# HliasGit/navier_stokes_solver

Measured on AMD Instinct MI355X. Metric: DoF*iters/s (FGMRES+aSIMPLE, Re=100; first K=5 outer iterations), higher is better.
Workload: dtype f64

## Files before the change

### include/nsk.h

```cpp
#ifndef NSK_H
#define NSK_H

#include <stdint.h>

#ifdef __cplusplus
extern "C" {
#endif

typedef struct nsk_handle_s *nsk_handle;

enum {
  NSK_BLK_F = 0,
  NSK_BLK_BT = 1,
  NSK_BLK_B = 2,
  NSK_BLK_MP = 3,
  NSK_BLK_BT_GHOST = 4,
  NSK_BLK_S = 5
};
enum { NSK_SPACE_U = 0, NSK_SPACE_P = 1 };
enum { NSK_SOLVER_GMRES = 0, NSK_SOLVER_FGMRES = 1, NSK_SOLVER_BICGSTAB = 2 };
enum { NSK_PREC_BLOCK_DIAGONAL = 0, NSK_PREC_BLOCK_TRIANGULAR = 1, NSK_PREC_ASIMPLE = 2 };
enum { NSK_VARIANT_STATIONARY = 0, NSK_VARIANT_UNSTEADY = 1 };
enum { NSK_TRI_VELOCITY = 0, NSK_TRI_PRESSURE = 1 };

enum {
  NSK_OPT_TRI_ORDERING = 0,
  NSK_OPT_SUBDOMAINS = 1,
  NSK_OPT_FUSE_BLOCK_ROW = 2,
  NSK_OPT_STREAM_KERNELS = 3,
  NSK_OPT_INNER_FUSED_GS = 4,
  NSK_OPT_OUTER_FUSED_GS = 5,
  NSK_OPT_CG_SINGLE_REDUCTION = 11,
  NSK_OPT_BSR_VELOCITY = 7,
  NSK_OPT_TRI_SYNC_FREE = 9,
  NSK_OPT_VELOCITY_AMG = 10,
  NSK_OPT_TRI_LINE_GROUPS = 12,
  NSK_OPT_MASS_ORDERING = 13,
  NSK_OPT_SCHUR_SIGN = 14,
  NSK_OPT_BLAS1_PAIRS = 15,
  NSK_OPT_FACTOR_PRECISION = 16,
  NSK_OPT_INNER_MATRIX_PRECISION = 17,
  NSK_OPT_INNER_BASIS_PRECISION = 18,
  NSK_OPT_INNER_MATRIX_FREE_F = 19
};

typedef struct {
  double setup_ms, solve_ms;
  int64_t outer_iters, inner_u_its, inner_p_its, prec_applies, spmv_calls, tri_applies, reductions, host_syncs;
  double spmv_bytes, tri_bytes, blas1_bytes;
  int32_t n_colors_u, n_levels_u, n_colors_p, n_levels_p;
  int64_t nnz_s;
  int64_t sync_free_fallbacks;
  int64_t cur_outer_iters;
  double cur_residual;
  int64_t overlapped_spmvs;
  int64_t ring_applies;
  int64_t columns_skipped;
} nsk_stats;

int nsk_get_unique_id(void *out128);

int nsk_local_group_id(int nranks, void *out128);

nsk_handle nsk_create(int rank, int nranks, int device_id, const void *rccl_unique_id);
void nsk_destroy(nsk_handle h);
const char *nsk_last_error(nsk_handle h);

int nsk_set_partition(nsk_handle h, int space, int64_t owned_begin, int64_t owned_end, int n_ghost,
                      const int32_t *ghost_gids);
int nsk_set_support_points(nsk_handle h, int space, const double *xy);
int nsk_set_halo_plan(nsk_handle h, int space, int n_neighbors, const int32_t *peer_rank, const int32_t *send_ptr,
                      const int32_t *send_idx, const int32_t *recv_ptr);

int nsk_set_block_csr(nsk_handle h, int blk, int n_rows, int n_cols, const int32_t *rowptr, const int32_t *col,
                      const double *val);
int nsk_update_values(nsk_handle h, int blk, const double *val);

int nsk_set_option(nsk_handle h, int opt, double value);

int nsk_setup_preconditioner(nsk_handle h, int type, int variant, double alpha);

int nsk_solve(nsk_handle h, int solver, double tol_abs, int max_iter, const double *rhs_u, const double *rhs_p,
              double *x_u, double *x_p, int *iters, double *final_res);

int nsk_upload_system(nsk_handle h, const double *rhs_u, const double *rhs_p, const double *x_u, const double *x_p);
int nsk_solve_resident(nsk_handle h, int solver, double tol_abs, int max_iter, int *iters, double *final_res);
int nsk_download_solution(nsk_handle h, double *x_u, double *x_p);

int nsk_spmv(nsk_handle h, int blk, const double *x_owned, double *y, int add);
int nsk_jacobian_vmult(nsk_handle h, const double *x_u, const double *x_p, double *y_u, double *y_p);
int nsk_dot(nsk_handle h, int n, const double *x, const double *y, double *dot_out, double *norm_x_out);
int nsk_vec_op(nsk_handle h, int op, int n, double a, double c, const double *x, double *y, const double *z,
               const double *d, double *scalar_out);
int nsk_tri_apply(nsk_handle h, int which, const double *b, double *x);
int nsk_amg_info(nsk_handle h, int shard, int level, int64_t *rows, int64_t *nnz, double *lambda_max);
int nsk_tri_get_perm(nsk_handle h, int which, int32_t *perm);
int nsk_tri_get_value_bytes(nsk_handle h, int which, int32_t *bytes);
int nsk_inner_value_bytes(nsk_handle h, int blk, int32_t *bytes);
int nsk_inner_basis_bytes(nsk_handle h, int32_t *bytes);
int nsk_inner_spmv(nsk_handle h, int blk, const double *x_owned, double *y);
int nsk_inner_matrix_free(nsk_handle h, int32_t *on);
int nsk_matfree_f(nsk_handle h, const double *x_owned, double *y);
int nsk_precond_vmult(nsk_handle h, const double *src_u, const double *src_p, double *dst_u, double *dst_p,
                      int calls);
int64_t nsk_block_nnz(nsk_handle h, int blk);
int nsk_get_block(nsk_handle h, int blk, int32_t *rowptr, int32_t *col, double *val);
int nsk_debug_spmv_form(int blk_ok, int stream_ok, int inner32, int use_stream, int use_bsr, int mode, int inner);

int nsk_assembly_set_cells(nsk_handle h, int64_t n_cells, const int32_t *cell_u_nodes, const int32_t *cell_p_dofs,
                           const uint8_t *cell_flags, const double *tables944, int32_t cell_of_dof0);
int nsk_assembly_set_dirichlet(nsk_handle h, const uint8_t *dirichlet_u, const double *bc_u );
int nsk_assembly_set_simplex(nsk_handle h, int64_t n_cells, const int32_t *cell_u_nodes, const int32_t *cell_p_dofs,
                             const double *grad_lambda, const double *area, int64_t n_blocks, const int32_t *blk_ptr,
                             const int32_t *blk_ent, const int64_t *blk_pos0, const int64_t *blk_pos1,
                             const int32_t *node_ptr, const int32_t *node_ent, const int32_t *vert_ptr,
                             const int32_t *vert_ent, const double *outlet_w, int64_t pos00);
int nsk_state_set(nsk_handle h, const double *u_owned, const double *p_owned);
int nsk_state_get(nsk_handle h, double *u_owned, double *p_owned);
int nsk_state_save(nsk_handle h);
int nsk_state_update(nsk_handle h, double alpha);
int nsk_state_save_old(nsk_handle h);
int nsk_assemble(nsk_handle h, int stokes, double nu, double inv_dt, double p_out, int inhomogeneous_bc,
                 double *residual_norm);
int nsk_forces_set_faces(nsk_handle h, int64_t n_faces, const int32_t *face_cell, const uint8_t *face_side,
                         const double *tables672);
int nsk_forces_set_edges(nsk_handle h, int64_t n_edges, const int32_t *edge_cell, const uint8_t *edge_local,
                         const double *edge_nl);
int nsk_forces(nsk_handle h, double nu, double *drag_lift, double *local_drag_lift );
int nsk_state_get_patches(nsk_handle h, int64_t n, const int32_t *cells, double *vel ,
                          double *prs );
int nsk_record_set_cells(nsk_handle h, int64_t n_cells, const int32_t *cells, int subdivisions,
                         const double *w_u , const double *w_p );
int nsk_state_get_record(nsk_handle h, int64_t n_points, double *vel3 , double *prs );
int nsk_scale_values(nsk_handle h, int blk, double factor);
int nsk_download_rhs(nsk_handle h, double *rhs_u, double *rhs_p);
int nsk_time_assemble(nsk_handle h, double nu, double inv_dt, int reps, double *avg_ms);

int nsk_get_stats(nsk_handle h, nsk_stats *out);
int nsk_get_history(nsk_handle h, double *out, int cap);
int nsk_cancel(nsk_handle h);
int nsk_abort_group(nsk_handle h);
int nsk_reset_stats(nsk_handle h);

int nsk_time_op(nsk_handle h, int op, int reps, double *avg_ms, double *bytes);

int nsk_profile_begin(nsk_handle h, int op, int max_samples);
int nsk_profile_read(nsk_handle h, int op, double *avg_ms, int *n_samples, double *bytes_per_launch,
                     int64_t *n_calls, double *bytes_format);
int nsk_profile_end(nsk_handle h);

#ifdef __cplusplus
}
#endif
#endif
```

### navier_stokes_solver_amd/csrc/nsk_core.cpp

```cpp
#include "nsk_core.hpp"

#include <rccl/rccl.h>

#include <algorithm>
#include <condition_variable>
#include <cstdlib>
#include <map>
#include <memory>
#include <mutex>

namespace nsk {

#define NSK_NCCL(call)                                                                     \
  do {                                                                                     \
    ncclResult_t r__ = (call);                                                             \
    if (r__ != ncclSuccess)                                                                \
      throw ::nsk::Error(-20, std::string(#call) + ": " + ncclGetErrorString(r__));        \
  } while (0)

struct LocalGroup {
  int n = 0;
  std::mutex m;
  std::condition_variable cv;
  int waiting = 0;
// ... 485 lines not shown
    if (ns >= 0 && comm.active()) {
      comm.allreduce_sum(slot(ns), 1, stream);
      scalar_sqrt(stream, slot(ns), slot(ns) + 1);
    }
    if (ns >= 0) ++st.reductions;
    st.blas1_bytes += 4.0 * n * mc + 16.0 * n;
    ++gs_launches;
  }
}
void Ctx::multi_add(int n, double *x, double *const *z, const double *y, int m) {
  const int cap = gs_one_launch == 1 ? kMgsMaxVecs : gs_one_launch == 2 ? 16 : 1;
  for (int i0 = 0; i0 < m; i0 += cap) {
    const int mc = std::min(cap, m - i0);
    VecPackAll Z{};
    CoefPack Y{};
    for (int k = 0; k < mc; ++k) { Z.v[k] = z[i0 + k]; Y.y[k] = y[i0 + k]; }
    if (gs_one_launch && vec_multi_add(stream, n, x, Z, Y, mc)) {
      st.blas1_bytes += 8.0 * n * (mc + 2);
      ++gs_launches;
    } else {
      for (int k = 0; k < mc; ++k, ++gs_launches) vec_axpy(stream, n, sref(y[i0 + k]), z[i0 + k], x);
      st.blas1_bytes += 24.0 * n * mc;
    }
  }
}

bool Ctx::mgs_applicable(int n, int nv) const {
  if (!fused_mgs || comm.active() || nv < 1 || nv > kMgsMaxVecs) return false;
  const int G = std::min(n_cu, kMgsThreads);
  return (long)n <= (long)G * kMgsThreads * 12;
}

void Ctx::warn(const std::string &msg) {
  fprintf(stderr, "[nsk] warning: %s\n", msg.c_str());
  if (warn_text) *warn_text = "warning: " + msg;
}

void Ctx::mgs_timed_out() {
  fused_mgs = false;
  ++mgs_fallbacks;
  if (mgs_err.p) NSK_HIP(hipMemsetAsync(mgs_err.p, 0, sizeof(int), stream));
  warn("one-launch Gram-Schmidt sweep: a wait ran out of spins (workgroups not co-resident: another process on the "
       "GPU?); this column is redone link by link and the sweep stays off for this handle (slower, same results)");
}

bool Ctx::mgs_sweep(int n, double *w, double *const *v, int nv, int so) {
  if (!mgs_applicable(n, nv)) return false;
  const int G = std::min(n_cu, kMgsThreads);
  const size_t tab = (size_t)(kMgsMaxVecs + 1) * G;
  if (mgs_grid != G) {
    mgs_tables.alloc(2 * tab);
    vec_fill_sentinel(stream, (int)(2 * tab), mgs_tables.p);
    mgs_err.alloc(1);
    NSK_HIP(hipMemsetAsync(mgs_err.p, 0, sizeof(int), stream));
    mgs_grid = G;
    mgs_parity = 0;
  }
  MgsArgs A{};
  A.n = n;
  A.nv = nv;
  for (int k = 0; k < nv; ++k) A.v[k] = v[k];
  A.aux = w;
  A.table = mgs_tables.p + (size_t)mgs_parity * tab;
  A.rearm = mgs_tables.p + (size_t)(1 - mgs_parity) * tab;
  A.out = slot(so);
  A.err = mgs_err.p;
  A.fault = mgs_fault ? 1 : 0;
  NSK_HIP(hipMemsetAsync(slot(so + nv + 2), 0, sizeof(double), stream));
  mgs_tier = nsk::mgs_sweep(stream, A, G);
  if (!mgs_tier) return false;
  mgs_parity = 1 - mgs_parity;
  st.reductions += nv + 1;
  st.blas1_bytes += 8.0 * n * (nv + 2);
  return true;
}

int Csr::spmv_launch(hipStream_t s, SpmvForm f, const double *xo, const double *xg, double *y, int mode, const double *z,
                     int c0, int c1) const {
  if (f == SpmvForm::csr_vector) return nsk::spmv(s, view(), lpr, xo, xg, y, mode, z);
  if (c1 == kToPlanEnd) c1 = is_blk(f) ? blk_nblk : nblk;
  if (c1 <= c0) return 0;
  const int *cb = off16.p ? colbase.p + c0 : nullptr;
  switch (f) {
    case SpmvForm::blk_f32: nsk::spmv_blk_stream(s, blk_view32(), blk_rowblk.p + c0, c1 - c0, xo, xg, y); return 0;
    case SpmvForm::blk: nsk::spmv_blk_stream(s, blk_view(), blk_R, blk_C, blk_rowblk.p + c0, c1 - c0, xo, xg, y); return 0;
    case SpmvForm::stream_f32: return nsk::spmv_stream(s, view32(), rowblk.p + c0, c1 - c0, even_rows, xo, xg, y, off16.p, cb);
    default: return nsk::spmv_stream(s, view(), rowblk.p + c0, c1 - c0, even_rows, xo, xg, y, mode, z, off16.p, cb);
  }
}

void Ctx::spmv(Csr &A, Space &colspace, const DVec &x, double *y, int mode, const double *z) {
  comm.halo_exchange(colspace, x, stream);
  A.spmv_launch(stream, A.spmv_form(true, false, mode), x.own, x.ghost, y, mode, z);
  ++st.spmv_calls;
  st.spmv_bytes += (double)A.spmv_bytes() + (mode ? 8.0 * A.n_rows : 0.0);
}

bool build_rowblocks(const int *ra, const int *rb, int n_rows, int max_nnz, const std::vector<int> *cuts,
                     std::vector<int> &rowblk, const unsigned char *glue) {
  rowblk.clear();
  rowblk.push_back(0);
  size_t ci = 0;
  int r0 = 0;
  auto nnz_of = [&](int a, int b) { return (ra[b] - ra[a]) + (rb ? rb[b] - rb[a] : 0); };
  while (r0 < n_rows) {
    while (cuts && ci < cuts->size() && (*cuts)[ci] <= r0) ++ci;
    const int limit = (cuts && ci < cuts->size()) ? std::min(n_rows, (*cuts)[ci]) : n_rows;
    int r1 = r0 + 1;
    if (nnz_of(r0, r1) > max_nnz) return false;
    while (r1 < limit && r1 - r0 < kStreamRows && nnz_of(r0, r1 + 1) <= max_nnz) ++r1;
    if (glue) {
      while (r1 < limit && r1 > r0 && glue[r1]) --r1;
      if (r1 == r0) {
        r1 = r0 + 1;
        while (r1 < limit && glue[r1]) ++r1;
        if (r1 - r0 > kStreamRows || nnz_of(r0, r1) > max_nnz) return false;
      }
    }
    rowblk.push_back(r1);
    r0 = r1;
  }
  return true;
}

void Csr::find_interior() {
  int_r0 = int_r1 = 0;
  if (n_cols == n_own_cols) { int_r1 = n_rows; return; }
  std::vector<char> ghost((size_t)n_rows, 0);
#pragma omp parallel for schedule(static)
  for (int i = 0; i < n_rows; ++i) {
    char g = 0;
    for (int k = h_rowptr[i]; k < h_rowptr[i + 1]; ++k) g |= h_col[k] >= n_own_cols;
    ghost[i] = g;
  }
  int best0 = 0, best1 = 0, start = 0;
  for (int i = 0; i <= n_rows; ++i) {
    if (i == n_rows || ghost[i]) {
      if (i - start > best1 - best0) { best0 = start; best1 = i; }
      start = i + 1;
    }
  }
  int_r0 = best0;
  int_r1 = best1;
}

static void interior_runs(const std::vector<int> &rb, int r0, int r1, int &b0, int &b1) {
  b0 = b1 = 0;
  const int nb = (int)rb.size() - 1;
  for (int b = 0; b < nb; ++b)
    if (rb[b] >= r0 && rb[b + 1] <= r1) {
      if (b1 == b0) b0 = b;
      b1 = b + 1;
    }
}

void Csr::build_stream_plan(hipStream_t s) {
  std::vector<int> rb;
  find_interior();
  std::vector<int> cuts;
  if (int_r0 > 0) cuts.push_back(int_r0);
  if (int_r1 < n_rows && int_r1 > int_r0) cuts.push_back(int_r1);
  stream_ok = n_rows > 0 && build_rowblocks(h_rowptr.data(), nullptr, n_rows, kStreamNnz, cuts.empty() ? nullptr : &cuts, rb);
  if (!stream_ok) { nblk = 0; return; }
  nblk = (int)rb.size() - 1;
  interior_runs(rb, int_r0, int_r1, int_b0, int_b1);
  even_rows = true;
  for (int i = 0; i <= n_rows; ++i)
    if (h_rowptr[i] & 1) { even_rows = false; break; }
  rowblk.upload(rb, s);
  off16.release();
  colbase.release();
  idx16_wide = false;
}

void Csr::build_index16(hipStream_t s, bool want) {
  off16.release();
  colbase.release();
  idx16_wide = false;
  if (!want || !stream_ok || nblk <= 0) return;
  if (nnz <= 0) {
    colbase.alloc((size_t)nblk);
    off16.alloc(8);
    NSK_HIP(hipMemsetAsync(colbase.p, 0, sizeof(int) * (size_t)nblk, s));
    NSK_HIP(hipMemsetAsync(off16.p, 0, 8 * sizeof(unsigned short), s));
    return;
  }
  if (!col.p) return;
  DBuf<int> wide;
  wide.alloc(1);
  colbase.alloc((size_t)nblk);
  NSK_HIP(hipMemsetAsync(wide.p, 0, sizeof(int), s));
  nsk::setup_run_col_base(s, nblk, nullptr, rowblk.p, rowptr.p, col.p, colbase.p, wide.p);
  int w = 0;
  NSK_HIP(hipMemcpyAsync(&w, wide.p, sizeof(int), hipMemcpyDeviceToHost, s));
  NSK_HIP(hipStreamSynchronize(s));
  if (w) {
    idx16_wide = true;
    colbase.release();
    return;
  }
  off16.alloc((size_t)nnz + 8);
  NSK_HIP(hipMemsetAsync(off16.p + nnz, 0, 8 * sizeof(unsigned short), s));
  nsk::setup_run_col_offsets(s, nblk, nullptr, rowblk.p, rowptr.p, col.p, colbase.p, off16.p);
}

void Csr::build_blocked(int R, int C, hipStream_t s) {
  blk_ok = false;
  if (n_rows <= 0 || n_rows % R || n_own_cols % C || n_cols % C) return;
  const int nr = n_rows / R;
  std::vector<int> rp(nr + 1, 0);
  bool ok = true;
#pragma omp parallel for schedule(static) reduction(&& : ok)
  for (int r = 0; r < nr; ++r) {
    const int a0 = h_rowptr[R * r], len = h_rowptr[R * r + 1] - a0;
    bool good = len % C == 0;
    for (int q = 1; good && q < R; ++q) good = h_rowptr[R * r + q + 1] - h_rowptr[R * r + q] == len;
    for (int k = 0; good && k < len; k += C) {
      const int c = h_col[a0 + k];
      good = c % C == 0;
      for (int q = 0; good && q < R; ++q)
        for (int t = 0; good && t < C; ++t) good = h_col[h_rowptr[R * r + q] + k + t] == c + t;
    }
    rp[r + 1] = len / C;
    ok = ok && good;
  }
  if (!ok) return;
  for (int r = 0; r < nr; ++r) rp[r + 1] += rp[r];
  blk_count = rp[nr];
  UVec<int> bcol((size_t)blk_count), bsrc((size_t)blk_count * R * C);
  std::vector<int> rb;
#pragma omp parallel for schedule(static)
  for (int r = 0; r < nr; ++r)
    for (int k = 0; k < rp[r + 1] - rp[r]; ++k) {
      const size_t b = (size_t)rp[r] + k;
      bcol[b] = h_col[h_rowptr[R * r] + C * k] / C;
      for (int q = 0; q < R; ++q)
        for (int t = 0; t < C; ++t) bsrc[(b * R + q) * C + t] = h_rowptr[R * r + q] + C * k + t;
    }
  find_interior();
  const int ib0 = (int_r0 + R - 1) / R, ib1 = int_r1 / R;
  std::vector<int> cuts;
  if (ib0 > 0 && ib0 < nr) cuts.push_back(ib0);
  if (ib1 < nr && ib1 > ib0) cuts.push_back(ib1);
  if (!build_rowblocks(rp.data(), nullptr, nr, kBlkMax, cuts.empty() ? nullptr : &cuts, rb)) return;
  interior_runs(rb, ib0, ib1, blk_int_b0, blk_int_b1);
  blk_R = R;
  blk_C = C;
  blk_rows = nr;
  blk_nblk = (int)rb.size() - 1;
  h_blk_rowptr = rp;
  blk_rowptr.upload(rp, s);
  blk_col.upload(bcol, s);
  blk_src.upload(bsrc, s);
  blk_rowblk.upload(rb, s);
  blk_val.alloc((size_t)blk_count * R * C);
  NSK_HIP(hipStreamSynchronize(s));
  blk_ok = true;
  refresh_blocked(s);
}

void Csr::refresh_blocked(hipStream_t s) {
  if (blk_ok) vec_gather(s, (int)(blk_count * blk_R * blk_C), blk_src.p, val.p, blk_val.p);
}

void Csr::refresh_f32(hipStream_t s, bool count_overflow) {
  if (!inner32) return;
  if (count_overflow) {
    if (!f32_overflow.p) f32_overflow.alloc(1);
    NSK_HIP(hipMemsetAsync(f32_overflow.p, 0, sizeof(unsigned), s));
  }
  unsigned *ovf = count_overflow ? f32_overflow.p : nullptr;
  if (inner32 == 1) {
    const size_t n = (size_t)blk_count * blk_R * blk_C;
    if (blk_val32.n != n) blk_val32.alloc(n);
    vec_gather(s, (int)n, blk_src.p, val.p, blk_val32.p);
    if (ovf) vec_to_float(s, (int)nnz, val.p, nullptr, ovf);
  } else {
    if (val32.n != (size_t)nnz) val32.alloc((size_t)nnz);
    vec_to_float(s, (int)nnz, val.p, val32.p, ovf);
  }
  val32_version = values_version;
}

double *VecPool::get(bool zero) {
  double *p;
  if (!free_list.empty()) {
    p = free_list.back();
    free_list.pop_back();
  } else {
    NSK_HIP(hipMalloc((void **)&p, sizeof(double) * (((size_t)n + ng + 15) / 16 * 16 + 16)));
    all.push_back(p);
    zero = true;
  }
  if (zero) NSK_HIP(hipMemsetAsync(p, 0, sizeof(double) * ((size_t)n + ng), ctx->stream));
  return p;
}

void VecPool::destroy() {
  for (double *p : all) (void)hipFree(p);
  all.clear();
  free_list.clear();
}

float *BasisPool32::get(int j, int n_) {
  if (n_ != n) { destroy(); n = n_; }
  if ((size_t)j >= v.size()) v.resize((size_t)j + 1, nullptr);
  if (!v[j]) NSK_HIP(hipMalloc((void **)&v[j], sizeof(float) * (((size_t)n + 3) / 4 * 4 + 4)));
  return v[j];
}

void BasisPool32::destroy() {
  for (float *p : v) if (p) (void)hipFree(p);
  v.clear();
  n = 0;
}

}
```

### navier_stokes_solver_amd/csrc/nsk_core.hpp

```cpp
#pragma once
#include <hip/hip_runtime.h>

#include <cstdint>
#include <cstdio>
#include <cstring>
#include <memory>
#include <stdexcept>
#include <string>
#include <vector>

#include "nsk_kernels.h"

struct ncclComm;

namespace nsk {

struct Error : std::runtime_error {
  int code;
  Error(int c, const std::string &m) : std::runtime_error(m), code(c) {}
};

#define NSK_HIP(call)                                                                              \
  do {                                                                                             \
    hipError_t e__ = (call);                                                                       \
// ... 18 lines not shown
template <class T>
struct DBuf {
  T *p = nullptr;
  size_t n = 0;
  DBuf() = default;
  DBuf(const DBuf &) = delete;
  DBuf &operator=(const DBuf &) = delete;
  DBuf(DBuf &&o) noexcept : p(o.p), n(o.n) { o.p = nullptr; o.n = 0; }
  DBuf &operator=(DBuf &&o) noexcept {
    if (this != &o) { release(); p = o.p; n = o.n; o.p = nullptr; o.n = 0; }
    return *this;
  }
  ~DBuf() { release(); }
  void release() {
    if (p) (void)hipFree(p);
    p = nullptr;
    n = 0;
  }
  void alloc(size_t count) {
    release();
    n = count;
    if (count) NSK_HIP(hipMalloc((void **)&p, count * sizeof(T)));
  }
  void upload(const T *h, size_t count, hipStream_t s) {
    if (count != n) alloc(count);
    if (count) NSK_HIP(hipMemcpyAsync(p, h, count * sizeof(T), hipMemcpyHostToDevice, s));
  }
  template <class A>
  void upload(const std::vector<T, A> &h, hipStream_t s) { upload(h.data(), h.size(), s); }
};

struct LocalXchg {
  DBuf<double> buf[2];
  hipEvent_t ready[2] = {nullptr, nullptr}, done[2] = {nullptr, nullptr};
  long seq = 0;
  std::vector<const LocalXchg *> peer;
  ~LocalXchg() {
    for (int k = 0; k < 2; ++k) {
      if (ready[k]) (void)hipEventDestroy(ready[k]);
      if (done[k]) (void)hipEventDestroy(done[k]);
    }
  }
};

struct Space {
  int n = 0;
  int ng = 0;
  int64_t gbegin = 0, gend = 0;
  std::vector<int> ghost_gid;
  std::vector<int> peers, send_ptr, recv_ptr;
  DBuf<int> d_send_idx;
  DBuf<double> d_send_buf;
  int n_send = 0;
  std::unique_ptr<LocalXchg> lx;
};

struct DVec {
  double *own = nullptr;
  double *ghost = nullptr;
  int n = 0;
};

enum class SpmvForm { csr_vector, stream, stream_f32, blk, blk_f32 };
inline bool is_f32(SpmvForm f) { return f == SpmvForm::stream_f32 || f == SpmvForm::blk_f32; }
inline bool is_blk(SpmvForm f) { return f == SpmvForm::blk || f == SpmvForm::blk_f32; }
constexpr SpmvForm spmv_form(bool blk_ok, bool stream_ok, int inner32, bool use_stream, bool use_bsr, int mode, bool inner) {
  if (inner && mode == 0 && inner32 == 1 && use_stream && use_bsr && blk_ok) return SpmvForm::blk_f32;
  if (inner && mode == 0 && inner32 == 2 && use_stream && stream_ok && !(blk_ok && use_bsr)) return SpmvForm::stream_f32;
  if (blk_ok && use_stream && use_bsr && mode == 0) return SpmvForm::blk;
  if (stream_ok && use_stream) return SpmvForm::stream;
  return SpmvForm::csr_vector;
}

struct Csr {
  int n_rows = 0, n_cols = 0, n_own_cols = 0;
  int64_t nnz = 0;
  std::vector<int> h_rowptr;
  UVec<int> h_col;
  DBuf<int> rowptr, col;
  DBuf<double> val;
  int lpr = 16;
  bool present = false;
  DBuf<int> rowblk;
  int nblk = 0;
  bool stream_ok = false, even_rows = false;
  void build_stream_plan(hipStream_t s);
  DBuf<unsigned short> off16;
  DBuf<int> colbase;
  bool idx16_wide = false;
  void build_index16(hipStream_t s, bool want);
  int int_r0 = 0, int_r1 = 0, int_b0 = 0, int_b1 = 0, blk_int_b0 = 0, blk_int_b1 = 0;
  void find_interior();
  bool blk_ok = false;
  int blk_R = 1, blk_C = 1, blk_rows = 0, blk_nblk = 0;
  int64_t blk_count = 0;
  std::vector<int> h_blk_rowptr;
  DBuf<int> blk_rowptr, blk_col, blk_src, blk_rowblk;
  DBuf<double> blk_val;
  void build_blocked(int R, int C, hipStream_t s);
  void refresh_blocked(hipStream_t s);
  BlkView blk_view() const { return BlkView{blk_rows, n_own_cols / blk_C, blk_rowptr.p, blk_col.p, blk_val.p}; }
  CsrView view() const { return CsrView{n_rows, n_own_cols, rowptr.p, col.p, val.p}; }
  int inner32 = 0;
  DBuf<float> blk_val32, val32;
  long values_version = 0, val32_version = -1;
  DBuf<unsigned> f32_overflow;
  void release_f32() { inner32 = 0; blk_val32.release(); val32.release(); f32_overflow.release(); val32_version = -1; }
  void refresh_f32(hipStream_t s, bool count_overflow);
  BlkView32 blk_view32() const { return BlkView32{blk_rows, n_own_cols / blk_C, blk_rowptr.p, blk_col.p, blk_val32.p}; }
  CsrView32 view32() const { return CsrView32{n_rows, n_own_cols, rowptr.p, col.p, val32.p}; }
  static constexpr int kToPlanEnd = -1;
  SpmvForm spmv_form(bool use_stream, bool use_bsr, int mode = 0, bool inner = false) const {
    return nsk::spmv_form(blk_ok, stream_ok, inner32, use_stream, use_bsr, mode, inner);
  }
  int spmv_launch(hipStream_t s, SpmvForm f, const double *x_own, const double *x_ghost, double *y, int mode = 0,
                  const double *z = nullptr, int c0 = 0, int c1 = kToPlanEnd) const;
  double format_bytes(SpmvForm f) const {
    const double vb = is_f32(f) ? 4.0 : 8.0;
    if (is_blk(f)) return (double)blk_count * (4.0 + vb * blk_R * blk_C) + 4.0 * (blk_rows + 1.0) + 8.0 * n_rows + 8.0 * n_cols;
    const bool index16 = off16.p && f != SpmvForm::csr_vector;
    return (double)spmv_bytes() - (8.0 - vb) * (double)nnz - (index16 ? 2.0 * (double)nnz - 4.0 * nblk : 0.0);
  }
  size_t spmv_bytes() const {
    return (size_t)12 * nnz + 4 * ((size_t)n_rows + 1) + 8 * (size_t)n_rows + 8 * (size_t)n_cols;
  }
};

bool build_rowblocks(const int *rowptr_a, const int *rowptr_b, int n_rows, int max_nnz, const std::vector<int> *cuts,
                     std::vector<int> &rowblk, const unsigned char *glue = nullptr);

inline int pick_lpr(int64_t nnz, int n_rows) {
  const double mean = n_rows > 0 ? (double)nnz / n_rows : 0.0;
  if (mean <= 6) return 4;
  if (mean <= 20) return 8;
  if (mean <= 80) return 16;
  if (mean <= 200) return 32;
  return 64;
}

struct LocalGroup;
struct Comm {
  int rank = 0, nranks = 1;
  ncclComm *comm = nullptr;
  LocalGroup *local = nullptr;
  const double *pub_buf = nullptr;
  const std::vector<int> *pub_peers = nullptr, *pub_send_ptr = nullptr;
  double *h_tmp = nullptr;
  bool on_stream = false;
  int device = 0;
  struct Pub {
    const LocalXchg *x[2] = {nullptr, nullptr};
    const std::vector<int> *peers[2] = {nullptr, nullptr}, *send_ptr[2] = {nullptr, nullptr};
    int parity[2] = {0, 0};
  } pub[2];
  long coll_seq = 0, ar_seq = 0;
  DBuf<double> ar_stage[2];
  hipEvent_t ar_ready[2] = {nullptr, nullptr}, ar_done[2] = {nullptr, nullptr};
  void local_exchange_on_stream(Space *const *sps, const DVec *xs, int count, hipStream_t s);
  bool active() const { return nranks > 1 || comm != nullptr; }
  void init(int rank, int nranks, const void *unique_id, int device_id = 0);
  void destroy();
  void abort_group();
  void allreduce_sum(double *d, int count, hipStream_t s);
  void halo_exchange(Space &sp, const DVec &x, hipStream_t s);
  void halo_exchange2(Space &sa, const DVec &xa, Space &sb, const DVec &xb, hipStream_t s);
};

int make_local_group(int nranks, void *out128, int on_stream = 0);
int abort_local_group(const void *unique_id);

struct Stats {
  double setup_ms = 0, solve_ms = 0;
  long outer_iters = 0, inner_u_its = 0, inner_p_its = 0, prec_applies = 0, spmv_calls = 0, tri_applies = 0,
       reductions = 0, host_syncs = 0, ring_applies = 0,
       columns_skipped = 0;
  double spmv_bytes = 0, tri_bytes = 0, blas1_bytes = 0;
};

struct Ctx {
  hipStream_t stream = nullptr;
  hipStream_t stream2 = nullptr;
  hipEvent_t ev_fork = nullptr, ev_join = nullptr;
  void ensure_stream2();
  int device = 0;
  int n_cu = 256;
  Comm comm;
  ReduceWs ws{};
  DBuf<double> ws_partials;
  DBuf<unsigned> ws_ticket;
  static constexpr int kSlots = 4096;
  DBuf<double> d_scal;
  double *h_scal = nullptr;
  int slot_top = 0;
  Stats st;

  void init(int device_id);
  void destroy();
  int alloc_slots(int k) {
    if (slot_top + k > kSlots) throw Error(-11, "out of device scalar slots");
    const int s = slot_top;
    slot_top += k;
    return s;
  }
  double *slot(int i) { return d_scal.p + i; }
  const double *read_slots(int first, int count);
  void sync() { NSK_HIP(hipStreamSynchronize(stream)); }

  void dot(int n, const double *x, const double *y, int slot_out);
  void norm2(int n, const double *x, int slot_out);
  void axpy_dot(int n, SRef a, const double *x, double *y, const double *w, int slot_out);
  void axpy_norm2(int n, SRef a, const double *x, double *y, int slot_out);
  void multi_dot(int n, const double *w, double *const *v, int m, int slot_out, bool defer = false);
// ... 80 lines not shown
```

### navier_stokes_solver_amd/csrc/nsk_debug.cpp

```cpp
#include <algorithm>
#include <cstring>

#include "nsk_handle.hpp"
#include "nsk_internal.h"

namespace {
std::vector<int> shifted(const int32_t *p, size_t n, int64_t base) {
  std::vector<int> v(n);
  for (size_t i = 0; i < n; ++i) {
    const int64_t q = (int64_t)p[i] + base;
    if (q < 0 || q > INT32_MAX) throw Error(-62, "position beyond int32");
    v[i] = (int)q;
  }
  return v;
}
DBuf<int> on_device(const int *h, size_t n) {
  DBuf<int> d;
  d.upload(h, n, nullptr);
  return d;
}
DBuf<double> on_device(const double *h, size_t n) {
  DBuf<double> d;
  d.upload(h, n, nullptr);
  return d;
// ... 256 lines not shown
    case NSK_DBG_KRY_MULTI_DOT_ALL_F32: {
      const bool rider = par[0] != 0.0;
      c.multi_dot_all_f32(n, d[0], f.data() + 1, m, rider, so);
      c.allreduce_slots(so, m + (rider ? 1 : 0));
      break;
    }
    case NSK_DBG_KRY_MULTI_AXPY_ALL_F32:
      set_slots(m);
      c.multi_axpy_all_f32(n, d[0], f.data() + 1, m, so, par[m] != 0.0 ? so + m : -1);
      break;
    case NSK_DBG_KRY_GS_COLUMN_F32: {
      const int mode = (int)par[0];
      if (mode < 1 || mode > 2) throw Error(-61, "nsk_debug_krylov: fp32 basis: Gram-Schmidt mode 1 or 2");
      if (!c.f32_basis_applies(mode)) throw Error(-61, "nsk_debug_krylov: fp32 basis: the pair forms only");
      arnoldi_column(c, n, d[0], (double *const *)nullptr, m, so, mode, [] {}, f.data() + 1);
      break;
    }
    case NSK_DBG_KRY_EQU:
      set_slots(1);
      vec_equ(st, n, sref(1.0, nullptr, c.slot(so)), d[0], d[1]);
      break;
    case NSK_DBG_KRY_EQU_F32:
      set_slots(1);
      vec_equ_f32(st, n, sref(1.0, nullptr, c.slot(so)), d[0], f[1], d[2]);
      break;
  }
  int bad_guards = 0;
  for (int k = 0; k < n_vec; ++k) {
    if (is_float(k)) {
      hf.resize((size_t)len[k]);
      bad_guards += fv[k].fetch(hf.data(), c);
      for (int64_t i = 0; i < len[k]; ++i) vec[k][i] = (double)hf[(size_t)i];
    } else {
      bad_guards += dv[k].fetch(vec[k], c);
    }
  }
  memcpy(slots64, c.read_slots(so, 64), sizeof(double) * 64);
  info8[0] = (int32_t)c.red_paths;
  info8[1] = path;
  info8[2] = std::min(c.n_cu, kMgsThreads);
  info8[3] = bad_guards;
  info8[4] = (int32_t)(c.gs_launches - gs_launches);
  for (int k = 5; k < 8; ++k) info8[k] = 0;
  return 0;
  NSK_CATCH(h)
}


int nsk_debug_spmv(nsk_handle h, int form, int lpr, int mode, int misalign, int c0, int c1, const nsk_dbg_spmv_mat *Am,
                   const nsk_dbg_spmv_mat *Bm, double *y, const double *z, const double *d, const double *dinv,
                   int32_t *rowblk_out, int rowblk_cap, int32_t *info) {
  NSK_TRY_DEV(h)
  Ctx &c = h->ctx;
  hipStream_t st = h->s();
  for (int k = 0; k < 16; ++k) info[k] = 0;
  info[0] = -1;
  if (form < NSK_DBG_SPMV_CSRV || form > NSK_DBG_SPMV_STREAM_I16_F32) throw Error(-65, "nsk_debug_spmv: unknown form");
  const bool two = form == NSK_DBG_SPMV_STREAM2 || form == NSK_DBG_SPMV_BLK_FUSED;
  const bool modes = form == NSK_DBG_SPMV_CSRV || form == NSK_DBG_SPMV_STREAM || form == NSK_DBG_SPMV_STREAM_I16;
  const bool epi = form == NSK_DBG_SPMV_BLK21_EPI;
  if (!Am || !y || two != (Bm != nullptr)) throw Error(-61, "nsk_debug_spmv: matrices");
  if (mode < 0 || mode > 2 || (mode != 0 && !modes) || (mode == 2 && !z)) throw Error(-61, "nsk_debug_spmv: mode");
  if (epi && !(d && dinv)) throw Error(-61, "nsk_debug_spmv: the epilogue needs d and dinv");
  if ((two || form == NSK_DBG_SPMV_CSRV) && c0 >= 0) throw Error(-61, "nsk_debug_spmv: this form runs whole plans only");
  int R = 1, C = 1;
  if (form == NSK_DBG_SPMV_BLK22 || form == NSK_DBG_SPMV_BLK22_F32 || form == NSK_DBG_SPMV_BLK_FUSED) R = C = 2;
  if (form == NSK_DBG_SPMV_BLK21 || epi) R = 2;
  if (form == NSK_DBG_SPMV_BLK12) C = 2;
  const bool blocked = form >= NSK_DBG_SPMV_BLK22 && form != NSK_DBG_SPMV_STREAM2 && form != NSK_DBG_SPMV_STREAM_I16 && form != NSK_DBG_SPMV_STREAM_I16_F32;
  if ((misalign & 4) && R == 2) throw Error(-61, "nsk_debug_spmv: the R = 2 forms store pairs, y is 16-byte aligned");
  if (two && Bm->n_rows != Am->n_rows) throw Error(-61, "nsk_debug_spmv: both matrices over the same rows");

  Csr A, B;
  dbg_fill_csr(A, *Am, st);
  if (two) dbg_fill_csr(B, *Bm, st);
  info[2] = A.lpr;
  info[3] = R;
  info[4] = C;
  info[5] = A.stream_ok;
  info[6] = A.stream_ok && A.even_rows;

  std::vector<int> rb;
  const std::vector<int> *ea = &A.h_rowptr, *eb = nullptr;
  DBuf<int> fused_rb;
  const int *d_rb = nullptr;
  int ib0 = 0, ib1 = 0, refused = 0;
  auto download = [&](const DBuf<int> &src, int nblk) {
    rb.resize((size_t)nblk + 1);
    NSK_HIP(hipMemcpyAsync(rb.data(), src.p, sizeof(int) * rb.size(), hipMemcpyDeviceToHost, st));
    c.sync();
    d_rb = src.p;
  };
  const bool i16 = form == NSK_DBG_SPMV_STREAM_I16 || form == NSK_DBG_SPMV_STREAM_I16_F32;
  if (form == NSK_DBG_SPMV_STREAM || form == NSK_DBG_SPMV_STREAM_F32 || i16) {
    if (!A.stream_ok) refused = 1;
    else { download(A.rowblk, A.nblk); ib0 = A.int_b0; ib1 = A.int_b1; }
    if (!refused && i16) {
      A.build_index16(st, true);
      if (!A.off16.p) refused = 5;
    }
  } else if (form == NSK_DBG_SPMV_STREAM2) {
    if (!A.even_rows) refused = 3;
    else if (!fused_row_plan(A, B, rb)) refused = 4;
    else { eb = &B.h_rowptr; fused_rb.upload(rb, st); d_rb = fused_rb.p; ib1 = (int)rb.size() - 1; }
  } else if (blocked) {
    A.build_blocked(R, C, st);
    if (two) B.build_blocked(2, 1, st);
    info[7] = A.blk_ok && (!two || B.blk_ok);
    if (!info[7] || (two && A.blk_rows != B.blk_rows)) refused = 2;
    else if (two) {
      if (!fused_blk_plan(A, B, rb)) refused = 4;
      else { ea = &A.h_blk_rowptr; eb = &B.h_blk_rowptr; fused_rb.upload(rb, st); d_rb = fused_rb.p; ib1 = (int)rb.size() - 1; }
    } else { download(A.blk_rowblk, A.blk_nblk); ea = &A.h_blk_rowptr; ib0 = A.blk_int_b0; ib1 = A.blk_int_b1; }
  }
  info[15] = refused;
  if (refused) return 1;
  const int nblk = (int)rb.size() - 1;
  if (form != NSK_DBG_SPMV_CSRV) {
    info[8] = nblk;
    info[9] = ib0;
    info[10] = ib1;
    for (int b = 0; b < nblk; ++b) {
      const int e = (*ea)[rb[b + 1]] - (*ea)[rb[b]] + (eb ? (*eb)[rb[b + 1]] - (*eb)[rb[b]] : 0);
      info[11] = std::max(info[11], rb[b + 1] - rb[b]);
      info[12] = std::max(info[12], e);
    }
    if (rowblk_out) std::copy(rb.begin(), rb.begin() + std::min<size_t>(rb.size(), (size_t)std::max(0, rowblk_cap)), rowblk_out);
    if (c0 < 0) { c0 = 0; c1 = nblk; }
    if (c0 > c1 || c1 > nblk) throw Error(-61, "nsk_debug_spmv: run range");
  }

  const int og = misalign & 1, ob = (misalign >> 1) & 1, oy = (misalign >> 2) & 1;
  DbgVec<double> xa, xag, xb, xbg, yv, zv, dv, div;
  xa.put(Am->x_own, (size_t)A.n_own_cols, kDbgFront, kDbgBack, st);
  xag.put(Am->x_ghost, (size_t)(A.n_cols - A.n_own_cols), kDbgFront + og, kDbgBack, st);
  if (two) {
    xb.put(Bm->x_own, (size_t)B.n_own_cols, kDbgFront + ob, kDbgBack, st);
    xbg.put(Bm->x_ghost, (size_t)(B.n_cols - B.n_own_cols), kDbgFront + og, kDbgBack, st);
  }
  yv.put(y, (size_t)A.n_rows, kDbgFront + oy, kDbgBack, st);
  if (z) zv.put(z, (size_t)A.n_rows, kDbgFront + oy, kDbgBack, st);
  if (epi) { dv.put(d, (size_t)A.n_rows, kDbgFront, kDbgBack, st); div.put(dinv, (size_t)A.n_rows, kDbgFront, kDbgBack, st); }

  const int n_run = c1 - c0;
  switch (form) {
    case NSK_DBG_SPMV_CSRV:
      if (lpr == 0) lpr = A.lpr;
      if (lpr != 2 && lpr != 4 && lpr != 8 && lpr != 16 && lpr != 32 && lpr != 64) throw Error(-61, "nsk_debug_spmv: lpr");
      info[2] = nsk::spmv(st, A.view(), lpr, xa.p, xag.p, yv.p, mode, zv.p);
      break;
    case NSK_DBG_SPMV_STREAM: case NSK_DBG_SPMV_STREAM_I16:
      info[1] = A.spmv_launch(st, SpmvForm::stream, xa.p, xag.p, yv.p, mode, zv.p, c0, c1);
      break;
    case NSK_DBG_SPMV_STREAM_F32: case NSK_DBG_SPMV_STREAM_I16_F32:
      A.inner32 = 2;
      A.refresh_f32(st, false);
      info[1] = A.spmv_launch(st, SpmvForm::stream_f32, xa.p, xag.p, yv.p, 0, nullptr, c0, c1);
      break;
    case NSK_DBG_SPMV_BLK22: case NSK_DBG_SPMV_BLK21: case NSK_DBG_SPMV_BLK12: case NSK_DBG_SPMV_BLK11:
      A.spmv_launch(st, SpmvForm::blk, xa.p, xag.p, yv.p, 0, nullptr, c0, c1);
      break;
    case NSK_DBG_SPMV_BLK22_F32:
      A.inner32 = 1;
      A.refresh_f32(st, false);
      A.spmv_launch(st, SpmvForm::blk_f32, xa.p, xag.p, yv.p, 0, nullptr, c0, c1);
      break;
    case NSK_DBG_SPMV_BLK21_EPI:
      nsk::spmv_blk_stream(st, A.blk_view(), 2, 1, d_rb + c0, n_run, xa.p, xag.p, yv.p, dv.p, div.p);
      break;
    case NSK_DBG_SPMV_STREAM2:
      info[1] = nsk::spmv2_stream(st, A.view(), xa.p, xag.p, B.view(), xb.p, xbg.p, d_rb, nblk, yv.p);
      break;
    case NSK_DBG_SPMV_BLK_FUSED:
      nsk::spmv_blk_fused22_21(st, A.blk_view(), xa.p, xag.p, B.blk_view(), xb.p, xbg.p, d_rb, nblk, yv.p);
      break;
  }
  NSK_HIP(hipGetLastError());
  info[0] = form;
  info[14] = form == NSK_DBG_SPMV_CSRV ? 0 : n_run;
  int bad = yv.fetch(y, c);
  for (DbgVec<double> *v : {&xa, &xag, &xb, &xbg, &zv, &dv, &div}) bad += v->fetch(nullptr, c);
  info[13] = bad;
  return 0;
  NSK_CATCH(h)
}

int nsk_debug_tri(nsk_handle h, const nsk_dbg_tri_args *a, int32_t *info) {
  NSK_TRY_DEV(h)
  Ctx &c = h->ctx;
  hipStream_t st = h->s();
  for (int k = 0; k < 40; ++k) info[k] = 0;
  if (!a || a->n < 1 || !a->rowptr || !a->col || !a->val || a->rowptr[0] != 0 || a->n_apply < 1 || !a->b || !a->x ||
      !a->perm_out || !a->factor_out)
    throw Error(-61, "nsk_debug_tri: arguments");
  if (a->kind < 0 || a->kind > 1 || a->ordering < ORDER_NATURAL || a->ordering > ORDER_MULTICOLOR || a->group < 1)
    throw Error(-61, "nsk_debug_tri: kind, ordering or group");
  const int n = a->n;
  for (int i = 0; i < n; ++i)
    if (a->rowptr[i + 1] < a->rowptr[i]) throw Error(-58, "nsk_debug_tri: rowptr not monotone");
  const int64_t nnz = a->rowptr[n];
  for (int i = 0; i < n; ++i)
    for (int k = a->rowptr[i]; k < a->rowptr[i + 1]; ++k)
      if (a->col[k] < 0 || a->col[k] >= n || (k > a->rowptr[i] && a->col[k - 1] >= a->col[k]))
        throw Error(-59, "nsk_debug_tri: column ids out of range or not sorted");
  std::vector<int> sub;
  if (a->n_sub > 1) {
    if (!a->sub_off || a->sub_off[0] != 0 || a->sub_off[a->n_sub] != n) throw Error(-61, "nsk_debug_tri: sub-domain offsets");
    for (int k = 0; k < a->n_sub; ++k)
      if (a->sub_off[k + 1] < a->sub_off[k]) throw Error(-61, "nsk_debug_tri: sub-domain offsets");
    sub.assign(a->sub_off, a->sub_off + a->n_sub + 1);
  }
  if (a->x_layout != 0 && !(a->want_block2 && a->sync_free)) {
    info[16] = 1;
    return 1;
  }

  Csr A;
  A.n_rows = A.n_cols = A.n_own_cols = n;
  A.nnz = nnz;
  A.h_rowptr.assign(a->rowptr, a->rowptr + n + 1);
  A.h_col.assign(a->col, a->col + nnz);
  A.rowptr.upload(a->rowptr, (size_t)n + 1, st);
  A.col.upload(a->col, (size_t)nnz, st);
  A.val.upload(a->val, (size_t)nnz, st);
  A.present = true;

  TriSolve T;
  T.use_stream = a->use_stream != 0;
  T.sync_free = a->sync_free != 0;
  T.tiny_bytes = a->tiny_bytes;
  T.host_analysis = a->host_analysis != 0;
  T.want_index16 = a->want_index16 != 0;
  T.want_f32 = a->want_f32 != 0;
  T.x_layout = a->x_layout != 0 ? 1 : 0;
  T.analyze(&c, A, a->kind, a->ordering, sub, a->want_block2 != 0, a->xy, a->group);
  T.y.alloc((size_t)n + 1 + kDbgBack);
  NSK_HIP(hipMemsetAsync(T.y.p, 0xFF, sizeof(double) * T.y.n, st));
  if (T.x_layout) {
    T.xc.alloc((size_t)n + 1 + kDbgBack);
    NSK_HIP(hipMemsetAsync(T.xc.p, 0xFF, sizeof(double) * T.xc.n, st));
  }
  T.numeric(A.val.p);
  NSK_HIP(hipGetLastError());

  std::vector<DbgVec<double>> bv((size_t)a->n_apply), xv((size_t)a->n_apply);
  for (int k = 0; k < a->n_apply; ++k) {
    bv[k].put(a->b + (size_t)k * n, (size_t)n, kDbgFront, kDbgBack, st);
    xv[k].put(a->x + (size_t)k * n, (size_t)n, kDbgFront, kDbgBack, st);
  }
  for (int k = 0; k < a->n_apply; ++k) T.apply(bv[k].p, xv[k].p);
  NSK_HIP(hipGetLastError());
  int bad = 0;
  for (int k = 0; k < a->n_apply; ++k) {
    bad += xv[k].fetch(a->x + (size_t)k * n, c);
    bad += bv[k].fetch(nullptr, c);
  }
  for (const DBuf<double> *iv : {&T.y, &T.xc}) {
// ... 22 lines not shown
    memcpy(&nanv, &nan_bits, 8);
    for (int64_t k = 0; k < nnz; ++k) a->factor_out[k] = nanv;
    for (size_t k = 0; k < fv.size(); ++k) {
      if (sp[k] < 0 || sp[k] >= nnz) throw Error(-62, "nsk_debug_tri: a source position outside the matrix");
      a->factor_out[sp[k]] = fv[k];
    }
  }

  const int path = T.last_path;
  const bool scalar_halves = path == TRI_PATH_SF_SCALAR || path == TRI_PATH_COLOUR_SCALAR;
  const bool halves = scalar_halves || path == TRI_PATH_SF_BLOCKED || path == TRI_PATH_COLOUR_BLOCKED;
  info[0] = path;
  info[1] = halves && T.f32 ? 32 : 64;
  info[2] = !scalar_halves ? 0 : T.Loff16.p ? 16 : 32;
  info[3] = !scalar_halves ? 0 : T.Uoff16.p ? 16 : 32;
  info[4] = T.gmax;
  info[5] = T.n_colors;
  info[6] = T.n_levels_L;
  info[7] = T.n_levels_U;
  if (T.stream_ready || T.block2_ready) {
    for (int half = 0; half < 2; ++half) {
      const DBuf<int4> &D = half ? T.Udesc : T.Ldesc;
      std::vector<int4> d(D.n);
      if (D.n) NSK_HIP(hipMemcpyAsync(d.data(), D.p, sizeof(int4) * D.n, hipMemcpyDeviceToHost, st));
      c.sync();
      info[8 + 2 * half] = (int)D.n;
      info[9 + 2 * half] = (half ? T.n_Usf : T.n_Lsf) - (int)D.n;
      for (const int4 &r : d) {
        info[12] = std::max(info[12], r.y - r.x);
        info[13] = std::max(info[13], r.w - r.z);
      }
    }
  }
  if (T.sf_err.p) {
    int e = 0;
    NSK_HIP(hipMemcpy(&e, T.sf_err.p, sizeof(int), hipMemcpyDeviceToHost));
    info[14] = e != 0;
  }
  info[15] = bad;
  info[17] = (a->want_block2 && !T.block2_ready ? 1 : 0) | (a->want_index16 && !(scalar_halves && T.Loff16.p) ? 2 : 0) |
             (a->want_f32 && info[1] != 32 ? 4 : 0) |
             (a->ordering == ORDER_NATURAL && n >= 4096 && !T.ring_ready ? 8 : 0);
  info[18] = T.lpr;
  for (const TriSolve::Step &s : T.schedL) ++info[s.serial ? 20 : 19];
  for (const TriSolve::Step &s : T.schedU) ++info[s.serial ? 29 : 28];
  info[21] = T.last_tiny;
  info[22] = T.ring_ready ? T.ringL.n_pass : 0;
  if (a->kind == 0)
    for (const TriSolve::Step &s : T.schedN) ++info[s.serial ? 24 : 23];
  info[25] = T.stream_ready;
  info[26] = T.block2_ready;
  info[27] = T.dev_analysis;
  info[30] = T.max_row_nnz;
  info[31] = (int32_t)T.nnz;
  info[32] = path == TRI_PATH_SF_BLOCKED && T.x_layout != 0;
  return 0;
  NSK_CATCH(h)
}

int nsk_debug_amg(nsk_handle h, const nsk_dbg_amg_args *a, int32_t *info) {
  NSK_TRY_DEV(h)
  return debug_amg(&h->ctx, a, info);
  NSK_CATCH(h)
}

int nsk_debug_index_width(nsk_handle h, int b, int32_t *out3) {
  NSK_TRY(h)
  if (b != NSK_BLK_S && b != NSK_BLK_MP) throw Error(-62, "nsk_debug_index_width: S or M_p");
  if (h->prec_type < 0) throw Error(-46, "call nsk_setup_preconditioner first");
  const Csr &A = h->blk[b];
  const TriSolve &T = b == NSK_BLK_S ? h->tS : h->tMp;
  out3[0] = !A.present || h->form_of(A) != SpmvForm::stream ? 0 : A.off16.p ? 16 : 32;
  const bool halves = T.stream_ready && T.halves_in_use();
  out3[1] = !halves ? 0 : T.Loff16.p ? 16 : 32;
  out3[2] = !halves ? 0 : T.Uoff16.p ? 16 : 32;
  return 0;
  NSK_CATCH(h)
}

int nsk_debug_spmv_form(int blk_ok, int stream_ok, int inner32, int use_stream, int use_bsr, int mode, int inner) {
  return (int)spmv_form(blk_ok != 0, stream_ok != 0, inner32, use_stream != 0, use_bsr != 0, mode, inner != 0);
}

int nsk_debug_pool_counts(nsk_handle h, int32_t *out6) {
  int k = 0;
  for (const VecPool *p : {&h->pool_u, &h->pool_p, &h->pool_b}) {
    out6[k++] = (int32_t)p->all.size();
    out6[k++] = (int32_t)p->free_list.size();
  }
  return 0;
}

int64_t nsk_debug_asm(nsk_handle h, int what, void *out, int64_t cap) {
  NSK_TRY_DEV(h)
  const auto &A = h->asmd;
  if (!A.ready || A.simplex || !A.mf_valid) throw Error(-66, "nsk_debug_asm: no Q3/Q2 assembly on the handle (call nsk_assemble)");
  const void *src = nullptr;
  size_t bytes = 0;
  switch (what) {
    case NSK_DBG_ASM_CQ: src = A.cq.p; bytes = sizeof(double) * (size_t)A.n_cells * kAsmCellDoubles; break;
    case NSK_DBG_ASM_D0: src = A.d0.p; bytes = sizeof(double); break;
    case NSK_DBG_ASM_NODE_CELLS: src = A.node_cells.p; bytes = sizeof(int) * A.node_cells.n; break;
    case NSK_DBG_ASM_NODE_OFF: src = A.node_off.p; bytes = A.node_off.n; break;
    case NSK_DBG_ASM_NODE_SELF: src = A.node_self.p; bytes = sizeof(int) * A.node_self.n; break;
    case NSK_DBG_ASM_PDOF_CELLS: src = A.pdof_cells.p; bytes = sizeof(int) * A.pdof_cells.n; break;
    default: throw Error(-65, "nsk_debug_asm: unknown item");
  }
  if (!out || cap < (int64_t)bytes) throw Error(-61, "nsk_debug_asm: out is too small");
  if (bytes) NSK_HIP(hipMemcpyAsync(out, src, bytes, hipMemcpyDeviceToHost, h->s()));
  h->ctx.sync();
  return (int64_t)bytes;
  NSK_CATCH(h)
}

}
```

### navier_stokes_solver_amd/csrc/nsk_handle.hpp

```cpp
#pragma once
#include <chrono>
#include <exception>
#include <string>
#include <vector>

#include "../../include/nsk.h"
#include "nsk_solver.hpp"
#include "nsk_amg.hpp"
#include "nsk_assembly.hpp"
#include "nsk_tri.hpp"

using namespace nsk;

inline double wall_ms() {
  return std::chrono::duration<double, std::milli>(std::chrono::steady_clock::now().time_since_epoch()).count();
}
inline bool verbose() {
  static const bool v = getenv("NSK_VERBOSE") && atoi(getenv("NSK_VERBOSE")) > 0;
  return v;
}
struct Phase {
  const char *name;
  double t0;
  explicit Phase(const char *n) : name(n), t0(wall_ms()) {}
// ... 18 lines not shown
    S.used = 0;
    S.e0.resize(cap);
    S.e1.resize(cap);
    for (int i = 0; i < cap; ++i) { (void)hipEventCreate(&S.e0[i]); (void)hipEventCreate(&S.e1[i]); }
  }
  Slot *want(int o) {
    for (int k = 0; k < n; ++k)
      if (slots[k].op == o) {
        ++slots[k].seen;
        return slots[k].used < slots[k].cap ? &slots[k] : nullptr;
      }
    return nullptr;
  }
  Slot *find(int o) {
    for (int k = 0; k < n; ++k)
      if (slots[k].op == o) return &slots[k];
    return nullptr;
  }
  void release() {
    for (int k = 0; k < n; ++k) {
      for (size_t i = 0; i < slots[k].e0.size(); ++i) { (void)hipEventDestroy(slots[k].e0[i]); (void)hipEventDestroy(slots[k].e1[i]); }
      slots[k] = Slot{};
    }
    n = 0;
  }
};

struct Sampled {
  EventSampler::Slot *smp;
  hipStream_t s;
  Sampled(EventSampler &es, int op, hipStream_t st) : smp(es.want(op)), s(st) {
    if (smp) (void)hipEventRecord(smp->e0[smp->used], s);
  }
  Sampled(const Sampled &) = delete;
  ~Sampled() {
    if (smp) (void)hipEventRecord(smp->e1[smp->used++], s);
  }
};
struct Event {
  hipEvent_t e = nullptr;
  Event() { NSK_HIP(hipEventCreate(&e)); }
  Event(const Event &) = delete;
  ~Event() { (void)hipEventDestroy(e); }
  operator hipEvent_t() const { return e; }
};

inline bool fused_blk_plan(const Csr &F, const Csr &Bt, std::vector<int> &rb) {
  return build_rowblocks(F.h_blk_rowptr.data(), Bt.h_blk_rowptr.data(), F.blk_rows, kBlkMax, nullptr, rb);
}
inline bool fused_row_plan(const Csr &F, const Csr &Bt, std::vector<int> &rb) {
  return build_rowblocks(F.h_rowptr.data(), Bt.h_rowptr.data(), F.n_rows, kStreamNnz, nullptr, rb);
}

struct nsk_handle_s {
  Ctx ctx;
  EventSampler sampler;
  std::string err;
  Space sp[2];
  Csr blk[6];
  VecPool pool_u, pool_p, pool_b;
  bool pools_ready = false;
  int tri_ordering = ORDER_MULTICOLOR, subdomains = 1, fuse_block_row = 1, use_stream = 1;
  int inner_fused_gs = 1;
  bool outer_fused_gs = false, cg_fused = false;
  int use_bsr = 1;
  int sync_free_fallbacks = 0;
  std::vector<double> support[2];
  int line_groups = 2, group_u = 2, group_p = 3;
  int mp_ordering = -1;
  int mass_ordering(int type, int variant_) const {
    if (mp_ordering >= 0) return mp_ordering;
    return (type == 0 && variant_ == 1) ? (int)ORDER_NATURAL : tri_ordering;
  }
  static constexpr int kGroupRowsU = 4000000, kGroupRowsP = 1000000;
  const double *xy(int space) const {
    if (!line_groups || support[space].size() != 2 * (size_t)sp[space].n) return nullptr;
    if (sync_free_mode < (space == 0 ? 2 : 1)) return nullptr;
    if (line_groups == 2 && sp[space].n > (space == 0 ? kGroupRowsU : kGroupRowsP)) return nullptr;
    return support[space].data();
  }
  int x_layout_mode = 2;
  int sync_free_mode = 2;
  int fault_inject = 0;
  DBuf<int> jrow_blk, jblk_blk;
  int jrow_nblk = 0, jblk_nblk = 0;
  bool jrow_ok = false, jblk_ok = false;

  int prec_type = -1, variant = 0;
  double alpha = 0.5;
  TriSolve tF, tMp, tS;
  Amg amgF;
  int velocity_amg = 1;
  int schur_sign = 1;
  int blas1_pairs = -1;
  int factor_precision = 64;
  int inner_matrix_precision = 64;
  int inner_basis_precision = 64;
  bool basis32_wanted = false;
  BasisPool32 basis32_u;
  int inner_basis_width() const {
    if (!inner_solve_on(NSK_BLK_F)) return 0;
    return basis32_wanted && ctx.f32_basis_applies(inner_fused_gs) ? 4 : 8;
  }
  void inner_fgmres_options(SolverFGMRES &sv) {
    sv.fused_gs = inner_fused_gs;
    sv.skip_unused = inner_skip();
    sv.basis32 = basis32_wanted ? &basis32_u : nullptr;
  }
  long mp_values_version = 0, mp_factored_version = -1;
  int mp_factored_kind = -1;
  bool amg_active = false;
  int timeop_between = -1;
  bool amg_pending = false;
  void amg_ready() {
    if (!amg_pending) return;
    amg_pending = false;
    const double t0 = wall_ms();
    try {
      amgF.setup(&ctx, blk[NSK_BLK_F], sub_offsets(0));
    } catch (...) {
      amgF.clear();
      amg_pending = true;
      throw;
    }
    setup_ms += wall_ms() - t0;
    lazy_setup_ms += wall_ms() - t0;
  }
  double lazy_setup_ms = 0;
  bool tF_ok = false, tMp_ok = false, tS_ok = false, s_symbolic = false;
  int tF_key = -1, tMp_key = -1, tS_key = -1;
  TriSolve *tP = nullptr;
  int s_max_row = 0;
  double *D = nullptr, *Dinv = nullptr, *tmp_p = nullptr, *delta_p = nullptr, *tmp_u = nullptr, *tmp_b = nullptr;
  double *rhs_b = nullptr, *x_b = nullptr, *x_keep = nullptr;
  volatile long progress_step = 0;
  volatile double progress_value = 0.0;
  volatile int cancel = 0;
  std::vector<double> history;
  long inner_u = 0, inner_p = 0, prec_applies = 0, outer_iters = 0;
  double setup_ms = 0, solve_ms = 0;
  bool skip_unused = true;
  SolverFGMRES::Pending pending;
  void drop_pending() {
    if (pending.v) pool_b.put(pending.v);
    if (pending.z) pool_b.put(pending.z);
    pending = SolverFGMRES::Pending{};
  }
  int inner_skip() const { return skip_unused ? SolverFGMRES::stateless : SolverFGMRES::reference; }

  struct AsmData {
    bool ready = false, dirichlet_set = false, have_bc = false, state_set = false;
    long n_cells = 0;
    int cell_of_dof0 = -1;
    DBuf<int> cell_u, cell_p, node_cells, node_self, pdof_cells;
    DBuf<unsigned char> cell_flags, node_off, dirichlet;
    DBuf<double> tables, cq, bc;
    double *sol_u = nullptr, *sol_p = nullptr, *eval_u = nullptr, *eval_p = nullptr;
    bool simplex = false;
    long sx_blocks = 0, sx_pos00 = 0;
    DBuf<int> sx_blk_ptr, sx_blk_ent, sx_node_ptr, sx_node_ent, sx_vert_ptr, sx_vert_ent;
    DBuf<long> sx_pos0, sx_pos1;
    DBuf<double> sx_grad, sx_area, sx_outlet;
    double *old_u = nullptr;
    bool have_old = false;
    double assemble_ms = 0;
    bool mf_valid = false;
    double mf_nu = 0, mf_inv_dt = 0;
// ... 56 lines not shown
    pool_u.init(&ctx, sp[0].n, sp[0].ng);
    pool_p.init(&ctx, sp[1].n, sp[1].ng);
    pool_b.init(&ctx, N(), sp[0].ng + sp[1].ng);
    rhs_b = pool_b.get(true);
    x_b = pool_b.get(true);
    pools_ready = true;
  }
  void halo(int space, const DVec &x) { ctx.comm.halo_exchange(sp[space], x, s()); }
  bool inner_solve_on(int b) const {
    if (prec_type < 0) return false;
    if (b == NSK_BLK_F) return prec_type != 2 || variant == 0;
    if (b == NSK_BLK_MP) return prec_type != 2;
    if (b == NSK_BLK_S) return prec_type == 2 && variant == 0;
    return false;
  }
  SpmvForm form_of(const Csr &A, int mode = 0, bool inner = false) const { return A.spmv_form(use_stream != 0, use_bsr != 0, mode, inner); }
  int inner_width(const Csr &A) const { return is_f32(form_of(A, 0, true)) ? 4 : 8; }
  void spmv_nohalo(Csr &A, const DVec &x, double *y, int mode = 0, const double *z = nullptr, bool inner = false) {
    {
      Sampled smp(sampler, (int)(&A - blk), s());
      A.spmv_launch(s(), form_of(A, mode, inner), x.own, x.ghost, y, mode, z);
    }
    ++ctx.st.spmv_calls;
    ctx.st.spmv_bytes += (double)A.spmv_bytes() + (mode == 1 ? 8.0 * A.n_rows : 0.0);
  }
  bool index16 = true;
  void index16_for(Csr &A, const char *name) {
    A.build_index16(s(), index16);
    if (verbose() && index16 && A.stream_ok && !A.off16.p)
      fprintf(stderr, "[nsk] %s: a run of the stream plan spans 65 536 columns or more — int32 column ids stay in use\n", name);
  }
  bool overlap_halo = true;
  long overlapped_spmvs = 0;
  void spmv_halo(Csr &A, int space, const DVec &x, double *y) {
    if (matfree_wanted && &A == &blk[NSK_BLK_F]) {
      const char *why = matfree_obstacle();
      if (!why) {
        halo(space, x);
        matfree_apply(x, y);
        return;
      }
      if (!matfree_warned) {
        matfree_warned = true;
        fprintf(stderr, "[nsk] warning: NSK_OPT_INNER_MATRIX_FREE_F = 1, but %s: the inner FGMRES multiplies by the assembled F\n", why);
      }
    }
    const SpmvForm form = form_of(A, 0, true);
    if (is_f32(form) && A.val32_version != A.values_version) A.refresh_f32(s(), false);
    const bool blocked = is_blk(form);
    const int b0 = blocked ? A.blk_int_b0 : A.int_b0, b1 = blocked ? A.blk_int_b1 : A.int_b1;
    const int nb = blocked ? A.blk_nblk : A.nblk;
    EventSampler::Slot *smp = sampler.find((int)(&A - blk));
    const bool sampling = smp && smp->used < smp->cap;
    if (!overlap_halo || ctx.comm.nranks <= 1 || form == SpmvForm::csr_vector || b1 <= b0 || sampling) {
      halo(space, x);
      spmv_nohalo(A, x, y, 0, nullptr, true);
      return;
    }
    if (smp) ++smp->seen;
    ++overlapped_spmvs;
    ctx.ensure_stream2();
    auto part = [&](hipStream_t st, int c0, int c1) { A.spmv_launch(st, form, x.own, x.ghost, y, 0, nullptr, c0, c1); };
    NSK_HIP(hipEventRecord(ctx.ev_fork, s()));
    NSK_HIP(hipStreamWaitEvent(ctx.stream2, ctx.ev_fork, 0));
    part(ctx.stream2, b0, b1);
    NSK_HIP(hipEventRecord(ctx.ev_join, ctx.stream2));
    halo(space, x);
    part(s(), 0, b0);
    part(s(), b1, nb);
    NSK_HIP(hipStreamWaitEvent(s(), ctx.ev_join, 0));
    ++ctx.st.spmv_calls;
    ctx.st.spmv_bytes += (double)A.spmv_bytes();
  }
  void jacobian_vmult(const DVec &xb, double *yb) {
    const DVec xu = ub(xb.own), xp = pb(xb.own);
    ctx.comm.halo_exchange2(sp[0], xu, sp[1], xp, s());
    Csr &F = blk[NSK_BLK_F], &Bt = blk[NSK_BLK_BT], &B = blk[NSK_BLK_B];
    const bool blocked = use_stream && use_bsr && F.blk_ok && Bt.blk_ok && F.blk_R == 2 && Bt.blk_R == 2 &&
                         F.blk_rows == Bt.blk_rows;
    if (fuse_block_row && blocked && !jblk_ok && jblk_nblk == 0) {
      std::vector<int> rb;
      if (fused_blk_plan(F, Bt, rb)) {
        jblk_nblk = (int)rb.size() - 1;
        jblk_blk.upload(rb, s());
        ctx.sync();
        jblk_ok = true;
      } else jblk_nblk = -1;
    }
    if (fuse_block_row && use_stream && !jrow_ok && jrow_nblk == 0 && F.even_rows) {
      std::vector<int> rb;
      if (fused_row_plan(F, Bt, rb)) {
        jrow_nblk = (int)rb.size() - 1;
        jrow_blk.upload(rb, s());
        ctx.sync();
        jrow_ok = true;
      } else jrow_nblk = -1;
    }
    const double fused_bytes = (double)F.spmv_bytes() + (double)Bt.spmv_bytes() - 8.0 * F.n_rows - 4.0 * (F.n_rows + 1);
    if (fuse_block_row && blocked && jblk_ok) {
      nsk::spmv_blk_fused22_21(s(), F.blk_view(), xu.own, xu.ghost, Bt.blk_view(), xp.own, xp.ghost, jblk_blk.p,
                               jblk_nblk, yb);
      ctx.st.spmv_calls += 2;
      ctx.st.spmv_bytes += fused_bytes;
    } else if (fuse_block_row && use_stream && jrow_ok) {
      nsk::spmv2_stream(s(), F.view(), xu.own, xu.ghost, Bt.view(), xp.own, xp.ghost, jrow_blk.p, jrow_nblk, yb);
      ctx.st.spmv_calls += 2;
      ctx.st.spmv_bytes += fused_bytes;
    } else {
      spmv_nohalo(F, xu, yb, 0);
      spmv_nohalo(Bt, xp, yb, 1);
    }
    spmv_nohalo(B, xu, yb + n_u(), 0);
  }
  void tri_apply_sampled(TriSolve &T, int op, const double *b, double *x) {
    Sampled smp(sampler, op, s());
    T.apply(b, x);
  }
  std::vector<int> sub_offsets(int space) const {
    std::vector<int> off;
    if (subdomains <= 1) return off;
    const int n = sp[space].n;
    off.resize(subdomains + 1);
    for (int k = 0; k <= subdomains; ++k) {
      long v = (long)n * k / subdomains;
      if (space == 0) v &= ~1L;
      off[k] = (int)v;
    }
    off[subdomains] = n;
    return off;
  }
  void check_sync_free() {
    int e = 0;
    for (TriSolve *T : {&tF, &tMp, &tS})
      if (T->sf_err.p) {
        int ei = 0;
        NSK_HIP(hipMemcpy(&ei, T->sf_err.p, sizeof(int), hipMemcpyDeviceToHost));
        if (ei) {
          NSK_HIP(hipMemsetAsync(T->sf_err.p, 0, sizeof(int), s()));
          T->sf_armed = false;
        }
        e |= ei;
      }
    if (ctx.comm.active() && sync_free_mode > 0) {
      const SlotLease sl(ctx, 1);
      vec_set(s(), 1, ctx.slot(sl), e ? 1.0 : 0.0);
      ctx.comm.allreduce_sum(ctx.slot(sl), 1, s());
      e = ctx.read_slots(sl, 1)[0] > 0.0;
    }
    if (e)
      throw Error(-70, "sync-free triangular solve: a producer/consumer wait ran out of spins (results invalid); "
                       "set NSK_OPT_TRI_SYNC_FREE to 0");
  }
  void push_tri_options() {
    tMp.sync_free = tS.sync_free = sync_free_mode >= 1;
    tF.sync_free = sync_free_mode == 2;
    tMp.sf_fault = tS.sf_fault = (fault_inject & 1) != 0;
    tF.sf_fault = (fault_inject & 2) != 0;
    tMp.want_index16 = tS.want_index16 = index16;
    tF.use_stream = tMp.use_stream = tS.use_stream = use_stream != 0;
  }
  void schur_symbolic();
  void setup(int type, int variant_, double alpha_);
  void prec_vmult(DVec &dst, const DVec &src);
  int solve_once(int solver, double tol, int max_iter, int *iters, double *final_res);
  int solve_resident(int solver, double tol, int max_iter, int *iters, double *final_res);
};
using H = nsk_handle_s;

#define NSK_TRY(h) try {
#define NSK_TRY_DEV(h) NSK_TRY(h) (void)hipSetDevice((h)->ctx.device);
#define NSK_CATCH(h)                                  \
  }                                                   \
  catch (const Error &e) {                            \
    (h)->err = e.what();                              \
    return e.code;                                    \
  }                                                   \
  catch (const std::exception &e) {                   \
    (h)->err = e.what();                              \
    return -1;                                        \
  }

#define NSK_CATCH_ABORT(h)                            \
  }                                                   \
  catch (const Error &e) {                            \
    (h)->err = e.what();                              \
    if (e.code != -25) (h)->ctx.comm.abort_group();   \
    return e.code;                                    \
  }                                                   \
// ... 6 lines not shown
```

### navier_stokes_solver_amd/csrc/nsk_internal.h

```cpp
#pragma once
#include <stdint.h>

enum {
  NSK_IOPT_TRI_X_LAYOUT = 6,
  NSK_IOPT_FAULT_INJECT = 100,
  NSK_IOPT_GROUP_U = 103,
  NSK_IOPT_GROUP_P = 104,
  NSK_IOPT_TINY_BYTES = 102,
  NSK_IOPT_OVERLAP_HALO = 107,
  NSK_IOPT_HOST_ANALYSIS = 108,
  NSK_IOPT_TIMEOP_BETWEEN = 109,
  NSK_IOPT_INDEX16 = 110,
  NSK_IOPT_GS_ONE_LAUNCH = 111,
  NSK_IOPT_FGMRES_SKIP_UNUSED = 112,
  NSK_IOPT_FUSED_MGS = 106
};

#ifdef __cplusplus
extern "C" {
#endif
int nsk_debug_tri_trace(struct nsk_handle_s *h, int which, int64_t *out16, int max_runs, int *grid);
int nsk_local_group_id_mode(int nranks, int on_stream, void *out128);
int nsk_abort_local_group(const void *uid128);
int nsk_debug_tri_ordering(int n, const int32_t *rowptr, const int32_t *col, int n_sub, const int32_t *sub_off,
                           int want_block2, const double *xy, int group, int32_t *perm_out, int32_t *info4,
                           uint8_t *chain_out);
int nsk_debug_ilu0_at_offset(int what, int n, const int32_t *rowptr, const int32_t *col, double *val_inout, int64_t base);
int nsk_debug_schur_at_offset(int n_p, int n_u, const int32_t *b_rp, const int32_t *b_col, const double *b_val,
                              const double *dinv, const int32_t *bt_rp, const int32_t *bt_col, const double *bt_val,
                              const int32_t *s_rp, const int32_t *s_col, double *s_val_out, int64_t base);
enum {
  NSK_DBG_KRY_DOT = 0, NSK_DBG_KRY_NORM2 = 1, NSK_DBG_KRY_AXPY_DOT = 2, NSK_DBG_KRY_AXPY_NORM2 = 3, NSK_DBG_KRY_CG_UPDATE = 4,
  NSK_DBG_KRY_MULTI_DOT = 5, NSK_DBG_KRY_MULTI_AXPY = 6, NSK_DBG_KRY_GS_COLUMN = 7, NSK_DBG_KRY_DOT3 = 8,
  NSK_DBG_KRY_CG_SCALARS = 9, NSK_DBG_KRY_CG_FUSED_UPDATE = 10, NSK_DBG_KRY_CHEBY = 11, NSK_DBG_KRY_DENSE_MV = 12,
  NSK_DBG_KRY_MULTI_DOT_ALL = 13, NSK_DBG_KRY_MULTI_AXPY_ALL = 14, NSK_DBG_KRY_MULTI_ADD = 15,
  NSK_DBG_KRY_MULTI_DOT_ALL_F32 = 16, NSK_DBG_KRY_MULTI_AXPY_ALL_F32 = 17, NSK_DBG_KRY_GS_COLUMN_F32 = 18,
  NSK_DBG_KRY_EQU = 19, NSK_DBG_KRY_EQU_F32 = 20
};
int nsk_debug_krylov(struct nsk_handle_s *h, int op, int n, int m, int offset, const double *par, int n_vec,
                     double *const *vec, const int64_t *len, double *slots64, int32_t *info8);
enum {
  NSK_DBG_SPMV_CSRV = 0, NSK_DBG_SPMV_STREAM = 1, NSK_DBG_SPMV_STREAM_F32 = 2, NSK_DBG_SPMV_BLK22 = 3,
  NSK_DBG_SPMV_BLK21 = 4, NSK_DBG_SPMV_BLK12 = 5, NSK_DBG_SPMV_BLK11 = 6, NSK_DBG_SPMV_BLK22_F32 = 7,
  NSK_DBG_SPMV_BLK21_EPI = 8, NSK_DBG_SPMV_STREAM2 = 9, NSK_DBG_SPMV_BLK_FUSED = 10, NSK_DBG_SPMV_STREAM_I16 = 11,
  NSK_DBG_SPMV_STREAM_I16_F32 = 12
};
struct nsk_dbg_spmv_mat {
  int32_t n_rows, n_cols, n_own_cols, pad_;
  const int32_t *rowptr, *col;
  const double *val, *x_own, *x_ghost;
};
int nsk_debug_spmv(struct nsk_handle_s *h, int form, int lpr, int mode, int misalign, int c0, int c1,
                   const struct nsk_dbg_spmv_mat *A, const struct nsk_dbg_spmv_mat *B, double *y, const double *z,
                   const double *d, const double *dinv, int32_t *rowblk_out, int rowblk_cap, int32_t *info16);
struct nsk_dbg_tri_args {
  int32_t n, kind, ordering, n_sub;
  const int32_t *rowptr, *col;
  const double *val;
  const int32_t *sub_off;
  const double *xy;
  int32_t group, want_block2, use_stream, sync_free;
  double tiny_bytes;
  int32_t host_analysis, want_index16, want_f32, x_layout;
  int32_t n_apply, pad_;
  const double *b;
  double *x;
  int32_t *perm_out;
  double *factor_out;
};
int nsk_debug_tri(struct nsk_handle_s *h, const struct nsk_dbg_tri_args *a, int32_t *info40);
enum {
  NSK_DBG_AMG_SCAN = 0, NSK_DBG_AMG_BLOCK = 1, NSK_DBG_AMG_DIAG = 2, NSK_DBG_AMG_STRENGTH = 3, NSK_DBG_AMG_MIS_PULL = 4,
  NSK_DBG_AMG_MIS_DECIDE = 5, NSK_DBG_AMG_MIS_MARK = 6, NSK_DBG_AMG_ROOTS = 7, NSK_DBG_AMG_JOIN = 8,
  NSK_DBG_AMG_AGG_WEIGHTS = 9, NSK_DBG_AMG_AGGREGATE = 10, NSK_DBG_AMG_PRODUCT = 11, NSK_DBG_AMG_PRODUCT_COUNT = 12,
  NSK_DBG_AMG_TRANSPOSE = 13, NSK_DBG_AMG_ROWS_SORT = 14, NSK_DBG_AMG_START_VECTOR = 15
};
struct nsk_dbg_amg_mat {
  int32_t n_rows, n_cols;
  const int32_t *rowptr, *col;
  const double *val;
};
struct nsk_dbg_amg_args {
  int32_t op, n, r0, r1, pass, stamp, roots_only, first, product, first_tier, nc, out_cap;
  int64_t flag_words;
  double threshold, c;
  struct nsk_dbg_amg_mat A, B;
  const int32_t *i_in;
  const uint64_t *key, *key2;
  const uint16_t *flag;
  const double *ad, *dinv, *pw;
  int32_t *i_out;
  uint64_t *k_out;
  uint16_t *flag_out;
  double *d_out, *d_out2;
  int32_t *out_rp, *out_col;
  double *out_val;
  int64_t *out64;
};
int nsk_debug_amg(struct nsk_handle_s *h, const struct nsk_dbg_amg_args *a, int32_t *info16);
int nsk_debug_index_width(struct nsk_handle_s *h, int b, int32_t *out3);
int nsk_debug_spmv_form(int blk_ok, int stream_ok, int inner32, int use_stream, int use_bsr, int mode, int inner);
int nsk_debug_pool_counts(struct nsk_handle_s *h, int32_t *out6);
enum { NSK_DBG_ASM_CQ = 0, NSK_DBG_ASM_D0 = 1, NSK_DBG_ASM_NODE_CELLS = 2, NSK_DBG_ASM_NODE_OFF = 3,
       NSK_DBG_ASM_NODE_SELF = 4, NSK_DBG_ASM_PDOF_CELLS = 5 };
int64_t nsk_debug_asm(struct nsk_handle_s *h, int what, void *out, int64_t cap);
#ifdef __cplusplus
}
#endif
```

### navier_stokes_solver_amd/csrc/nsk_kernels.h

```cpp
#pragma once
#include <hip/hip_runtime.h>
#include <stdint.h>

namespace nsk {

struct SRef {
  double c;
  const double *num;
  const double *den;
};
inline SRef sref(double c) { return SRef{c, nullptr, nullptr}; }
inline SRef sref(double c, const double *num) { return SRef{c, num, nullptr}; }
inline SRef sref(double c, const double *num, const double *den) { return SRef{c, num, den}; }

struct ReduceWs {
  double *partials;
  unsigned *ticket;
  int pairs;
};
constexpr int kMaxReduceBlocks = 512;
constexpr int kMaxReduceOut = 32;

template <class V>
struct CsrViewT {
  int n_rows;
  int n_own_cols;
  const int *rowptr;
  const int *col;
  const V *val;
};
using CsrView = CsrViewT<double>;
using CsrView32 = CsrViewT<float>;
int spmv(hipStream_t s, const CsrView &A, int lanes_per_row, const double *x_own, const double *x_ghost, double *y,
         int mode, const double *z);

constexpr int kStreamNnz = 2048;
constexpr int kStreamRows = 64;
int spmv_stream(hipStream_t s, const CsrView &A, const int *rowblk, int nblk, int even_rows, const double *x_own,
                const double *x_ghost, double *y, int mode, const double *z, const unsigned short *off16 = nullptr,
                const int *colbase = nullptr);
int spmv_stream(hipStream_t s, const CsrView32 &A, const int *rowblk, int nblk, int even_rows, const double *x_own,
                const double *x_ghost, double *y, const unsigned short *off16 = nullptr, const int *colbase = nullptr);
int spmv2_stream(hipStream_t s, const CsrView &A, const double *xa_own, const double *xa_ghost, const CsrView &B,
                 const double *xb_own, const double *xb_ghost, const int *rowblk, int nblk, double *y);

template <class V>
struct BlkViewT {
  int n_brows;
  int n_own_bcols;
  const int *rowptr;
  const int *col;
  const V *val;
};
using BlkView = BlkViewT<double>;
using BlkView32 = BlkViewT<float>;
constexpr int kBlkMax = 1024;
void spmv_blk_stream(hipStream_t s, const BlkView &A, int R, int C, const int *rowblk, int nblk, const double *x_own,
                     const double *x_ghost, double *y, const double *epi_d = nullptr, const double *epi_dinv = nullptr);
void spmv_blk_stream(hipStream_t s, const BlkView32 &A, const int *rowblk, int nblk, const double *x_own,
                     const double *x_ghost, double *y);
void spmv_blk_fused22_21(hipStream_t s, const BlkView &A, const double *xa_own, const double *xa_ghost,
                         const BlkView &B, const double *xb_own, const double *xb_ghost, const int *rowblk, int nblk,
                         double *y);

void vec_set(hipStream_t s, int n, double *y, double v);
void vec_copy(hipStream_t s, int n, const double *x, double *y);
void vec_equ(hipStream_t s, int n, SRef a, const double *x, double *y);
void vec_axpy(hipStream_t s, int n, SRef a, const double *x, double *y);
void vec_sadd(hipStream_t s, int n, SRef sc, SRef a, const double *x, double *y);
void vec_axpy2(hipStream_t s, int n, SRef a, const double *x, SRef b, const double *z, double *y);
void vec_scale(hipStream_t s, int n, SRef a, double *y);
void vec_mul(hipStream_t s, int n, const double *d, double *y);
void vec_submul(hipStream_t s, int n, const double *d, const double *x, double *y);
void vec_sub_then_mul(hipStream_t s, int n, const double *x, const double *d, double *y);
void vec_recip(hipStream_t s, int n, const double *x, double *y);
void vec_cheby_step(hipStream_t s, int n, double c1, double c2, const double *dinv, const double *r, double *w,
                    double *x, int set_x);
void dense_mv(hipStream_t s, int n, const double *M, const double *b, double *x);
constexpr int kRedScalar = 1, kRedPairs = 2;
int vec_dot(hipStream_t s, const ReduceWs &ws, int n, const double *x, const double *y, double *out, int want_sqrt);
int vec_axpy_dot(hipStream_t s, const ReduceWs &ws, int n, SRef a, const double *x, double *y, const double *w,
                 double *out, int want_sqrt);
int vec_cg_update(hipStream_t s, const ReduceWs &ws, int n, SRef a, const double *d, const double *h, double *x,
                  double *g, double *out);
struct VecPack {
  const double *v[8];
};
int vec_multi_dot(hipStream_t s, const ReduceWs &ws, int n, const double *w, const VecPack &P, int m, double *out);
void gs_pythagoras(hipStream_t s, double *h, int m);
int vec_multi_axpy(hipStream_t s, const ReduceWs &ws, int n, double *w, const VecPack &P, int m, const double *h,
                   double *norm_out);
constexpr int kMgsThreads = 1024, kMgsMaxVecs = 32;
struct VecPackAll {
  const double *v[kMgsMaxVecs];
};
int vec_multi_dot_all(hipStream_t s, const ReduceWs &ws, int n, const double *w, const VecPackAll &P, int m, double *out);
int vec_multi_axpy_all(hipStream_t s, const ReduceWs &ws, int n, double *w, const VecPackAll &P, int m, const double *h,
                       double *norm_out);
struct CoefPack {
  double y[kMgsMaxVecs];
};
int vec_multi_add(hipStream_t s, int n, double *x, const VecPackAll &Z, const CoefPack &Y, int m);
struct VecPack32 {
  const float *v[kMgsMaxVecs];
};
int vec_multi_dot_f32(hipStream_t s, const ReduceWs &ws, int n, const double *w, const VecPack32 &P, int m, int rider,
                      double *out);
int vec_multi_axpy_f32(hipStream_t s, const ReduceWs &ws, int n, double *w, const VecPack32 &P, int m, const double *h,
                       double *norm_out);
int red_grid_quads(int n);
void vec_equ_f32(hipStream_t s, int n, SRef a, const double *x, float *v, double *vw);
struct MgsArgs {
  int n, nv;
  const double *v[kMgsMaxVecs];
  double *aux, *table, *rearm, *out;
  int *err;
  int fault;
};
int mgs_sweep(hipStream_t s, const MgsArgs &A, int G);
int vec_dot3(hipStream_t s, const ReduceWs &ws, int n, const double *r, const double *u, const double *w, double *out);
void cg_fused_scalars(hipStream_t s, double *sc7, int first);
void vec_cg_fused_update(hipStream_t s, int n, const double *sc7, const double *u, const double *w, double *p, double *sv,
                         double *x, double *r);
void scalar_sqrt(hipStream_t s, const double *in, double *out);
void vec_gather(hipStream_t s, int n, const int *idx, const double *x, double *y);
void vec_gather(hipStream_t s, int n, const int *idx, const double *x, float *y);
void vec_to_float(hipStream_t s, int n, const double *x, float *y, unsigned *overflow);
void extract_diag(hipStream_t s, const CsrView &A, double *d, double *dinv);

struct TriView {
  int n;
  const int *rowptr;
  const int *diag;
  const int *col;
  const double *val;
  const int *perm;
};
void tri_lower_level(hipStream_t s, const TriView &T, int kind, int lpr, const int *rows, int nrows, const double *rhs,
                     double *y);
void tri_upper_level(hipStream_t s, const TriView &T, int kind, int lpr, const int *rows, int nrows, double *y,
                     double *out);
void tri_lower_serial(hipStream_t s, const TriView &T, int kind, const int *lvl_ptr, const int *rows, int l0, int l1,
                      const double *rhs, double *y);
void tri_upper_serial(hipStream_t s, const TriView &T, int kind, const int *lvl_ptr, const int *rows, int l0, int l1,
                      double *y, double *out);
// ... 111 lines not shown
```

### navier_stokes_solver_amd/csrc/nsk_kernels.hip

```cpp
#include "nsk_kernels.h"

#include <algorithm>
#include <type_traits>

namespace nsk {

namespace {

constexpr int BLK = 256;

__device__ __forceinline__ double sval(const SRef &s) {
  double v = s.c;
  if (s.num) v *= *s.num;
  if (s.den) v /= *s.den;
  return v;
}

template <int W>
__device__ __forceinline__ double subwave_sum(double v) {
#pragma unroll
  for (int off = W / 2; off > 0; off >>= 1) v += __shfl_down(v, off, W);
  return v;
}

inline int ew_grid(int n) {
  long b = ((long)n + BLK * 4 - 1) / (BLK * 4);
  if (b < 1) b = 1;
  if (b > 2048) b = 2048;
  return (int)b;
}
constexpr int RBLK = 1024;
inline int red_grid(int n) {
  long b = ((long)n + RBLK * 4 - 1) / (RBLK * 4);
  if (b < 1) b = 1;
  if (b > kMaxReduceBlocks) b = kMaxReduceBlocks;
  return (int)b;
}
inline int red_grid_pairs(int n, int cap) {
  long b = (((long)n + 1) / 2 + RBLK * 4 - 1) / (RBLK * 4);
  if (b < 1) b = 1;
  if (b > cap) b = cap;
  return (int)b;
}

template <int LPR, int MODE>
__global__ __launch_bounds__(BLK) void spmv_kernel(CsrView A, const double *__restrict__ xo,
                                                   const double *__restrict__ xg, double *__restrict__ y,
                                                   const double *__restrict__ z) {
  const long tid = (long)blockIdx.x * BLK + threadIdx.x;
  const int row = (int)(tid / LPR);
  const int lane = (int)(tid % LPR);
  double s = 0.0;
  if (row < A.n_rows) {
    const int re = A.rowptr[row + 1];
    for (int k = A.rowptr[row] + lane; k < re; k += LPR) {
      const int c = A.col[k];
      const double xv = c < A.n_own_cols ? xo[c] : xg[c - A.n_own_cols];
      s += A.val[k] * xv;
    }
  }
  s = subwave_sum<LPR>(s);
  if (lane == 0 && row < A.n_rows) {
    if (MODE == 0) y[row] = s;
    else if (MODE == 1) y[row] = (z ? z[row] : y[row]) + s;
    else y[row] = z[row] - s;
  }
}

constexpr int RG = 4;

__device__ __forceinline__ double2 widen2(double2 v) { return v; }
__device__ __forceinline__ double2 widen2(float2 v) { return make_double2((double)v.x, (double)v.y); }

template <class I>
struct IdxPair;
template <>
struct IdxPair<int> {
  typedef int v2 __attribute__((ext_vector_type(2)));
  typedef v2 unaligned __attribute__((aligned(4)));
  typedef v2 aligned2;
  int a, b;
  __device__ __forceinline__ IdxPair(v2 q, int) : a(q[0]), b(q[1]) {}
};
template <>
struct IdxPair<unsigned short> {
  typedef unsigned v2;
  typedef unsigned unaligned __attribute__((aligned(2)));
  typedef unsigned aligned2;
  int a, b;
  __device__ __forceinline__ IdxPair(unsigned q, int base) : a(base + (int)(q & 0xffffu)), b(base + (int)(q >> 16)) {}
};

template <class V, int VEC, class I = int>
__device__ __forceinline__ void stream_products(const I *__restrict__ col, const V *__restrict__ val, int k0,
                                                int k1, int n_own, const double *__restrict__ xo,
                                                const double *__restrict__ xg, double *prod, int base = 0) {
  if (VEC == 3) {
    constexpr int U = kStreamNnz / (2 * BLK);
    typedef V vv2 __attribute__((ext_vector_type(2)));
    typedef vv2 vd2u __attribute__((aligned(sizeof(V))));
    int c0[U], c1[U];
    double v0[U], v1[U], x0[U], x1[U];
#pragma unroll
    for (int u = 0; u < U; ++u) {
      const int k = k0 + 2 * ((int)threadIdx.x + u * BLK);
      if (k + 1 < k1) {
        const IdxPair<I> ci(*reinterpret_cast<const typename IdxPair<I>::unaligned *>(col + k), base);
        const vv2 vi = *reinterpret_cast<const vd2u *>(val + k);
        c0[u] = ci.a; c1[u] = ci.b; v0[u] = (double)vi[0]; v1[u] = (double)vi[1];
      } else {
        const bool ok = k < k1;
        c0[u] = ok ? base + (int)col[k] : 0; v0[u] = ok ? (double)val[k] : 0.0; c1[u] = 0; v1[u] = 0.0;
      }
    }
#pragma unroll
    for (int u = 0; u < U; ++u) {
      x0[u] = *(c0[u] < n_own ? xo + c0[u] : xg + (c0[u] - n_own));
      x1[u] = *(c1[u] < n_own ? xo + c1[u] : xg + (c1[u] - n_own));
    }
#pragma unroll
    for (int u = 0; u < U; ++u) {
      const int k = k0 + 2 * ((int)threadIdx.x + u * BLK);
      if (k < k1) prod[k - k0] = v0[u] * x0[u];
      if (k + 1 < k1) prod[k - k0 + 1] = v1[u] * x1[u];
    }
  } else if (VEC == 2) {
    constexpr int U = kStreamNnz / (2 * BLK);
    typedef typename std::conditional<std::is_same<V, double>::value, double2, float2>::type V2;
    int2 c[U];
    double2 v[U];
#pragma unroll
    for (int u = 0; u < U; ++u) {
      const int k = k0 + 2 * ((int)threadIdx.x + u * BLK);
      const bool ok = k < k1;
      if (ok) {
        const IdxPair<I> ci(*reinterpret_cast<const typename IdxPair<I>::aligned2 *>(col + k), base);
        c[u] = make_int2(ci.a, ci.b);
      } else c[u] = make_int2(0, 0);
      v[u] = ok ? widen2(*reinterpret_cast<const V2 *>(val + k)) : make_double2(0.0, 0.0);
    }
    double x0[U], x1[U];
#pragma unroll
    for (int u = 0; u < U; ++u) {
      x0[u] = *(c[u].x < n_own ? xo + c[u].x : xg + (c[u].x - n_own));
      x1[u] = *(c[u].y < n_own ? xo + c[u].y : xg + (c[u].y - n_own));
    }
#pragma unroll
    for (int u = 0; u < U; ++u) {
      const int k = k0 + 2 * ((int)threadIdx.x + u * BLK);
      if (k < k1) { prod[k - k0] = v[u].x * x0[u]; prod[k - k0 + 1] = v[u].y * x1[u]; }
    }
  } else {
    constexpr int U = kStreamNnz / BLK;
    int c[U];
    double v[U], xv[U];
#pragma unroll
    for (int u = 0; u < U; ++u) {
      const int k = k0 + (int)threadIdx.x + u * BLK;
      const bool ok = k < k1;
      c[u] = ok ? base + (int)col[k] : 0;
      v[u] = ok ? (double)val[k] : 0.0;
    }
#pragma unroll
    for (int u = 0; u < U; ++u) xv[u] = *(c[u] < n_own ? xo + c[u] : xg + (c[u] - n_own));
#pragma unroll
    for (int u = 0; u < U; ++u) {
      const int k = k0 + (int)threadIdx.x + u * BLK;
      if (k < k1) prod[k - k0] = v[u] * xv[u];
    }
  }
}

__device__ __forceinline__ double row_sum_lds(const double *prod, int b, int e, int lane) {
  double s = 0.0;
  int j = b + lane;
  for (; j + 3 * RG < e; j += 4 * RG) {
    const double a0 = prod[j], a1 = prod[j + RG], a2 = prod[j + 2 * RG], a3 = prod[j + 3 * RG];
    s += a0;
    s += a1;
    s += a2;
    s += a3;
  }
  for (; j < e; j += RG) s += prod[j];
  return subwave_sum<RG>(s);
}

template <class V, int VEC, int MODE, class I = int>
__global__ __launch_bounds__(BLK) void spmv_stream_kernel(CsrViewT<V> A, const int *__restrict__ rowblk,
                                                          const double *__restrict__ xo,
                                                          const double *__restrict__ xg, double *__restrict__ y,
                                                          const double *__restrict__ z,
                                                          const unsigned short *__restrict__ off16 = nullptr,
                                                          const int *__restrict__ colbase = nullptr) {
  __shared__ double prod[kStreamNnz];
  const int r0 = rowblk[blockIdx.x], r1 = rowblk[blockIdx.x + 1];
  constexpr bool I16 = std::is_same<I, unsigned short>::value;
  const int base = I16 ? colbase[blockIdx.x] : 0;
  const int k0 = A.rowptr[r0], k1 = A.rowptr[r1];
  const int r = r0 + (int)threadIdx.x / RG, lane = threadIdx.x % RG;
  const bool have = r < r1;
  int jb = 0, je = 0;
  double zv = 0.0;
  if (have) {
    jb = A.rowptr[r] - k0;
    je = A.rowptr[r + 1] - k0;
    if (MODE == 1) zv = z ? z[r] : y[r];
    if (MODE == 2) zv = z[r];
  }
  if constexpr (I16) stream_products<V, VEC, unsigned short>(off16, A.val, k0, k1, A.n_own_cols, xo, xg, prod, base);
  else stream_products<V, VEC>(A.col, A.val, k0, k1, A.n_own_cols, xo, xg, prod);
  __syncthreads();
  const double sum = row_sum_lds(prod, jb, je, lane);
  if (have && lane == 0) {
    if (MODE == 0) y[r] = sum;
    else if (MODE == 1) y[r] = zv + sum;
    else y[r] = zv - sum;
  }
}

template <int VECA>
__global__ __launch_bounds__(BLK) void spmv2_stream_kernel(CsrView A, const double *__restrict__ xao,
                                                           const double *__restrict__ xag, CsrView B,
                                                           const double *__restrict__ xbo,
                                                           const double *__restrict__ xbg,
                                                           const int *__restrict__ rowblk, double *__restrict__ y) {
  __shared__ double prod[kStreamNnz];
  const int r0 = rowblk[blockIdx.x], r1 = rowblk[blockIdx.x + 1];
  const int a0 = A.rowptr[r0], a1 = A.rowptr[r1], b0 = B.rowptr[r0], b1 = B.rowptr[r1];
  const int r = r0 + (int)threadIdx.x / RG, lane = threadIdx.x % RG;
  const bool have = r < r1;
  int ab = 0, ae = 0, bb = 0, be = 0;
  if (have) {
    ab = A.rowptr[r] - a0; ae = A.rowptr[r + 1] - a0;
    bb = B.rowptr[r] - b0; be = B.rowptr[r + 1] - b0;
  }
  stream_products<double, VECA>(A.col, A.val, a0, a1, A.n_own_cols, xao, xag, prod);
  double *prodB = prod + (a1 - a0);
  stream_products<double, 1>(B.col, B.val, b0, b1, B.n_own_cols, xbo, xbg, prodB);
  __syncthreads();
  double sum = 0.0;
  for (int j = ab + lane; j < ae; j += RG) sum += prod[j];
  for (int j = bb + lane; j < be; j += RG) sum += prodB[j];
  sum = subwave_sum<RG>(sum);
  if (have && lane == 0) y[r] = sum;
}

template <class V, int R, int C>
__device__ __forceinline__ void blk_products(const BlkViewT<V> &A, int k0, int k1, const double *__restrict__ xo,
                                             const double *__restrict__ xg, double *p0, double *p1) {
  constexpr int U = kBlkMax / BLK;
  if (k0 >= k1) return;
  int m[U];
  double2 a0[U], a1[U];
  double x0[U], x1[U];
#pragma unroll
  for (int u = 0; u < U; ++u) {
    const int k = k0 + (int)threadIdx.x + u * BLK;
    const bool ok = k < k1;
    m[u] = ok ? __builtin_nontemporal_load(A.col + k) : 0;
    const V *v = A.val + (size_t)(R * C) * (ok ? k : k0);
    if constexpr (std::is_same<V, float>::value) {
      static_assert(R == 2 && C == 2, "fp32 values: 2 x 2 blocks only");
      const float4 q = *reinterpret_cast<const float4 *>(v);
      a0[u] = make_double2((double)q.x, (double)q.y); a1[u] = make_double2((double)q.z, (double)q.w);
    } else {
      if (R * C == 4) { a0[u] = *reinterpret_cast<const double2 *>(v); a1[u] = *reinterpret_cast<const double2 *>(v + 2); }
      else if (R * C == 2) { a0[u] = *reinterpret_cast<const double2 *>(v); a1[u] = make_double2(0.0, 0.0); }
      else { a0[u] = make_double2(v[0], 0.0); a1[u] = make_double2(0.0, 0.0); }
    }
  }
#pragma unroll
  for (int u = 0; u < U; ++u) {
    x1[u] = 0.0;
    if (C == 2) {
      if (m[u] < A.n_own_bcols) {
        const double2 xv = *reinterpret_cast<const double2 *>(xo + 2 * (size_t)m[u]);
        x0[u] = xv.x; x1[u] = xv.y;
      } else {
        const size_t g = 2 * (size_t)(m[u] - A.n_own_bcols);
        x0[u] = xg[g]; x1[u] = xg[g + 1];
      }
    } else {
      x0[u] = *(m[u] < A.n_own_bcols ? xo + m[u] : xg + (m[u] - A.n_own_bcols));
    }
  }
#pragma unroll
  for (int u = 0; u < U; ++u) {
    const int k = k0 + (int)threadIdx.x + u * BLK;
    if (k < k1) {
      if (R == 2 && C == 2) { p0[k - k0] = a0[u].x * x0[u] + a0[u].y * x1[u]; p1[k - k0] = a1[u].x * x0[u] + a1[u].y * x1[u]; }
      else if (R == 2 && C == 1) { p0[k - k0] = a0[u].x * x0[u]; p1[k - k0] = a0[u].y * x0[u]; }
      else if (R == 1 && C == 2) p0[k - k0] = a0[u].x * x0[u] + a0[u].y * x1[u];
      else p0[k - k0] = a0[u].x * x0[u];
    }
  }
}

template <class V, int R, int C, int EPI>
__global__ __launch_bounds__(BLK) void spmv_blk_kernel(BlkViewT<V> A, const int *__restrict__ rowblk,
                                                       const double *__restrict__ xo, const double *__restrict__ xg,
                                                       double *__restrict__ y, const double *__restrict__ d,
                                                       const double *__restrict__ dinv) {
  __shared__ double p0[kBlkMax];
  __shared__ double p1[R == 2 ? kBlkMax : 1];
  const int r0 = rowblk[blockIdx.x], r1 = rowblk[blockIdx.x + 1];
  const int k0 = A.rowptr[r0], k1 = A.rowptr[r1];
  const int r = r0 + (int)threadIdx.x / RG, lane = threadIdx.x % RG;
  const bool have = r < r1;
  int jb = 0, je = 0;
  if (have) { jb = A.rowptr[r] - k0; je = A.rowptr[r + 1] - k0; }
  blk_products<V, R, C>(A, k0, k1, xo, xg, p0, p1);
  __syncthreads();
  double s0 = 0.0, s1 = 0.0;
  for (int j = jb + lane; j < je; j += RG) { s0 += p0[j]; if (R == 2) s1 += p1[j]; }
  s0 = subwave_sum<RG>(s0);
  if (R == 2) s1 = subwave_sum<RG>(s1);
  if (have && lane == 0) {
    if (EPI == 1 && R == 2) {
      const double2 yo = *reinterpret_cast<const double2 *>(y + 2 * (size_t)r);
      const double2 dd = *reinterpret_cast<const double2 *>(d + 2 * (size_t)r);
      const double2 di = *reinterpret_cast<const double2 *>(dinv + 2 * (size_t)r);
      s0 = __dmul_rn(__dsub_rn(__dmul_rn(yo.x, dd.x), s0), di.x);
      s1 = __dmul_rn(__dsub_rn(__dmul_rn(yo.y, dd.y), s1), di.y);
    }
    if (R == 2) *reinterpret_cast<double2 *>(y + 2 * (size_t)r) = make_double2(s0, s1);
    else y[r] = s0;
  }
}

__global__ __launch_bounds__(BLK) void spmv_blk_fused_kernel(BlkView A, const double *__restrict__ xao,
                                                             const double *__restrict__ xag, BlkView B,
                                                             const double *__restrict__ xbo,
                                                             const double *__restrict__ xbg,
                                                             const int *__restrict__ rowblk, double *__restrict__ y) {
  __shared__ double p0[kBlkMax];
  __shared__ double p1[kBlkMax];
  const int r0 = rowblk[blockIdx.x], r1 = rowblk[blockIdx.x + 1];
  const int a0 = A.rowptr[r0], a1 = A.rowptr[r1], b0 = B.rowptr[r0], b1 = B.rowptr[r1];
  const int r = r0 + (int)threadIdx.x / RG, lane = threadIdx.x % RG;
  const bool have = r < r1;
  int ab = 0, ae = 0, bb = 0, be = 0;
  if (have) {
    ab = A.rowptr[r] - a0; ae = A.rowptr[r + 1] - a0;
    bb = B.rowptr[r] - b0 + (a1 - a0); be = B.rowptr[r + 1] - b0 + (a1 - a0);
  }
  blk_products<double, 2, 2>(A, a0, a1, xao, xag, p0, p1);
  blk_products<double, 2, 1>(B, b0, b1, xbo, xbg, p0 + (a1 - a0), p1 + (a1 - a0));
  __syncthreads();
  double s0 = 0.0, s1 = 0.0;
  for (int j = ab + lane; j < ae; j += RG) { s0 += p0[j]; s1 += p1[j]; }
  for (int j = bb + lane; j < be; j += RG) { s0 += p0[j]; s1 += p1[j]; }
  s0 = subwave_sum<RG>(s0);
  s1 = subwave_sum<RG>(s1);
  if (have && lane == 0) *reinterpret_cast<double2 *>(y + 2 * (size_t)r) = make_double2(s0, s1);
}

template <class V, int LOWER, int KIND, int NNZ, int I16 = 0>
__global__ __launch_bounds__(BLK) void tri_stream_kernel(TriHalfT<V> M, int b0, int nb, const double *__restrict__ dinv,
                                                         const int *__restrict__ perm,
                                                         const double *__restrict__ rhs, double *__restrict__ w) {
  __shared__ double prod[NNZ];
  const int per = (int)gridDim.x >> 3;
  const int mapped = (int)(blockIdx.x & 7) * per + (int)(blockIdx.x >> 3);
  if (mapped >= nb) return;
  const int4 d = M.desc[b0 + mapped];
  const int r0 = d.x, r1 = d.y, k0 = d.z, k1 = d.w;
  const int base = I16 ? M.base[b0 + mapped] : 0;
  const int r = r0 + (int)threadIdx.x / RG, lane = threadIdx.x % RG;
  const bool have = r < r1;
  int jb = 0, je = 0, i = 0;
  double own = 0.0, dv = 1.0;
  if (have) {
    jb = M.rowptr[r] - k0;
    je = M.rowptr[r + 1] - k0;
    i = perm[r];
    own = LOWER ? rhs[i] : w[i];
    if (KIND == 1 || !LOWER) dv = dinv[r];
  }
  {
    constexpr int U = NNZ / BLK;
    int c[U];
    double v[U], g[U];
#pragma unroll
    for (int u = 0; u < U; ++u) {
      const int k = k0 + (int)threadIdx.x + u * BLK;
      const bool ok = k < k1;
      if (I16) c[u] = ok ? base + (int)__builtin_nontemporal_load(M.off16 + k) : 0;
      else c[u] = ok ? __builtin_nontemporal_load(M.col + k) : 0;
      v[u] = ok ? (double)__builtin_nontemporal_load(M.val + k) : 0.0;
    }
#pragma unroll
    for (int u = 0; u < U; ++u) g[u] = w[c[u]];
#pragma unroll
    for (int u = 0; u < U; ++u) {
      const int k = k0 + (int)threadIdx.x + u * BLK;
      if (k < k1) prod[k - k0] = v[u] * g[u];
    }
  }
  __syncthreads();
  const double sum = row_sum_lds(prod, jb, je, lane);
  if (have && lane == 0) {
    double v;
    if (LOWER) v = KIND == 0 ? (own - sum) : (own - sum) * dv;
    else v = KIND == 0 ? (own - sum) * dv : own - sum * dv;
    w[i] = v;
  }
}

template <class V>
struct Blk4;
template <>
struct Blk4<double> {
  double2 r0, r1;
  __device__ __forceinline__ void load(const double *v) {
    r0 = *reinterpret_cast<const double2 *>(v);
    r1 = *reinterpret_cast<const double2 *>(v + 2);
  }
  __device__ __forceinline__ double2 row0() const { return r0; }
  __device__ __forceinline__ double2 row1() const { return r1; }
};
template <>
struct Blk4<float> {
  float4 q;
  __device__ __forceinline__ void load(const float *v) { q = *reinterpret_cast<const float4 *>(v); }
  __device__ __forceinline__ double2 row0() const { return make_double2((double)q.x, (double)q.y); }
  __device__ __forceinline__ double2 row1() const { return make_double2((double)q.z, (double)q.w); }
};

template <class V, int LOWER, int KIND>
__global__ __launch_bounds__(BLK) void tri_blk_kernel(TriBlkT<V> M, int b0, int nb, const double *__restrict__ intra,
                                                      const int *__restrict__ permn, const double *__restrict__ rhs,
                                                      double *__restrict__ x) {
  __shared__ double p0[kBlkMax];
  __shared__ double p1[kBlkMax];
// ... 993 lines not shown

__global__ __launch_bounds__(BLK) void spgemm_kernel(CsrView B, const double *__restrict__ dio,
                                                     const double *__restrict__ dig, CsrView Bt, CsrView Btg,
                                                     const int *__restrict__ srp, const int *__restrict__ scol,
                                                     double *__restrict__ sval, int n_rows, int max_nnz) {
  extern __shared__ double lds[];
  const int wave = threadIdx.x >> 6, lane = threadIdx.x & 63;
  const int i = blockIdx.x * (BLK / 64) + wave;
  if (i >= n_rows) return;
  double *acc = lds + (size_t)wave * max_nnz;
  const int ss = srp[i], se = srp[i + 1];
  for (int k = lane; k < se - ss; k += 64) acc[k] = 0.0;
  __builtin_amdgcn_fence(__ATOMIC_SEQ_CST, "wavefront");
  __builtin_amdgcn_wave_barrier();
  for (int k = B.rowptr[i]; k < B.rowptr[i + 1]; ++k) {
    const int m = B.col[k];
    const bool own = m < B.n_own_cols;
    const double a = B.val[k] * (own ? dio[m] : dig[m - B.n_own_cols]);
    const CsrView &R = own ? Bt : Btg;
    const int mr = own ? m : m - B.n_own_cols;
    const int qe = R.rowptr[mr + 1];
    for (int q = R.rowptr[mr] + lane; q < qe; q += 64) {
      const int j = R.col[q];
      int lo = ss, hi = se;
      while (lo < hi) {
        const int mid = lo + ((hi - lo) >> 1);
        if (scol[mid] < j) lo = mid + 1; else hi = mid;
      }
      acc[lo - ss] += a * R.val[q];
    }
    __builtin_amdgcn_fence(__ATOMIC_SEQ_CST, "wavefront");
    __builtin_amdgcn_wave_barrier();
  }
  for (int k = lane; k < se - ss; k += 64) sval[ss + k] = acc[k];
}

template <int LPR, int MODE>
void launch_spmv(hipStream_t s, const CsrView &A, const double *xo, const double *xg, double *y, const double *z) {
  const long threads = (long)A.n_rows * LPR;
  const int grid = (int)((threads + BLK - 1) / BLK);
  if (grid > 0) hipLaunchKernelGGL((spmv_kernel<LPR, MODE>), dim3(grid), dim3(BLK), 0, s, A, xo, xg, y, z);
}
template <int LPR>
void launch_spmv_mode(hipStream_t s, const CsrView &A, const double *xo, const double *xg, double *y, int mode,
                      const double *z) {
  if (mode == 0) launch_spmv<LPR, 0>(s, A, xo, xg, y, z);
  else if (mode == 1) launch_spmv<LPR, 1>(s, A, xo, xg, y, z);
  else launch_spmv<LPR, 2>(s, A, xo, xg, y, z);
}

template <int KIND, bool LOWER>
void launch_tri_level(hipStream_t s, const TriView &T, int lpr, const int *rows, int nrows, const double *rhs,
                      double *y, double *out) {
  if (nrows <= 0) return;
#define NSK_TRI_CASE(L)                                                                                      \
  case L: {                                                                                                  \
    const int grid = (int)(((long)nrows * L + BLK - 1) / BLK);                                               \
    hipLaunchKernelGGL((tri_level_kernel<L, KIND, LOWER>), dim3(grid), dim3(BLK), 0, s, T, rows, nrows, rhs, y, out); \
  } break;
  switch (lpr) {
    NSK_TRI_CASE(4)
    NSK_TRI_CASE(8)
    NSK_TRI_CASE(16)
    NSK_TRI_CASE(32)
    default: NSK_TRI_CASE(64)
  }
#undef NSK_TRI_CASE
}

}

int spmv(hipStream_t s, const CsrView &A, int lpr, const double *xo, const double *xg, double *y, int mode,
         const double *z) {
  switch (lpr) {
    case 2: launch_spmv_mode<2>(s, A, xo, xg, y, mode, z); return 2;
    case 4: launch_spmv_mode<4>(s, A, xo, xg, y, mode, z); return 4;
    case 8: launch_spmv_mode<8>(s, A, xo, xg, y, mode, z); return 8;
    case 16: launch_spmv_mode<16>(s, A, xo, xg, y, mode, z); return 16;
    case 32: launch_spmv_mode<32>(s, A, xo, xg, y, mode, z); return 32;
    default: launch_spmv_mode<64>(s, A, xo, xg, y, mode, z); return 64;
  }
}

int spmv_stream(hipStream_t s, const CsrView &A, const int *rowblk, int nblk, int even_rows, const double *xo,
                const double *xg, double *y, int mode, const double *z, const unsigned short *off16, const int *colbase) {
  if (nblk <= 0) return 0;
#define NSK_SS(V, M)                                                                                                                   \
  do {                                                                                                                                 \
    if (off16) hipLaunchKernelGGL((spmv_stream_kernel<double, V, M, unsigned short>), dim3(nblk), dim3(BLK), 0, s, A, rowblk, xo, xg, y, z, off16, colbase); \
    else hipLaunchKernelGGL((spmv_stream_kernel<double, V, M, int>), dim3(nblk), dim3(BLK), 0, s, A, rowblk, xo, xg, y, z, off16, colbase); \
  } while (0)
  if (even_rows) {
    if (mode == 0) NSK_SS(2, 0); else if (mode == 1) NSK_SS(2, 1); else NSK_SS(2, 2);
    return 2;
  }
  if (mode == 0) NSK_SS(3, 0); else if (mode == 1) NSK_SS(3, 1); else NSK_SS(3, 2);
  return 3;
#undef NSK_SS
}

int spmv_stream(hipStream_t s, const CsrView32 &A, const int *rowblk, int nblk, int even_rows, const double *xo,
                const double *xg, double *y, const unsigned short *off16, const int *colbase) {
  if (nblk <= 0) return 0;
  const double *z = nullptr;
#define NSK_SS(V)                                                                                                                      \
  do {                                                                                                                                 \
    if (off16) hipLaunchKernelGGL((spmv_stream_kernel<float, V, 0, unsigned short>), dim3(nblk), dim3(BLK), 0, s, A, rowblk, xo, xg, y, z, off16, colbase); \
    else hipLaunchKernelGGL((spmv_stream_kernel<float, V, 0, int>), dim3(nblk), dim3(BLK), 0, s, A, rowblk, xo, xg, y, z, off16, colbase); \
  } while (0)
  if (even_rows) { NSK_SS(2); return 2; }
  NSK_SS(3);
  return 3;
#undef NSK_SS
}

int spmv2_stream(hipStream_t s, const CsrView &A, const double *xao, const double *xag, const CsrView &B,
                 const double *xbo, const double *xbg, const int *rowblk, int nblk, double *y) {
  if (nblk <= 0) return 0;
  hipLaunchKernelGGL((spmv2_stream_kernel<2>), dim3(nblk), dim3(BLK), 0, s, A, xao, xag, B, xbo, xbg, rowblk, y);
  return 2;
}

template <class V>
static void tri_blk_level_t(hipStream_t s, const TriBlkT<V> &M, int b0, int b1, int lower, int kind, const double *intra,
                            const int *permn, const double *rhs, double *x) {
  const int nb = b1 - b0;
  if (nb <= 0) return;
  const int grid = ((nb + 7) / 8) * 8;
#define NSK_TB(L, K) hipLaunchKernelGGL((tri_blk_kernel<V, L, K>), dim3(grid), dim3(BLK), 0, s, M, b0, nb, intra, permn, rhs, x)
  if (lower) { if (kind == 0) NSK_TB(1, 0); else NSK_TB(1, 1); }
  else { if (kind == 0) NSK_TB(0, 0); else NSK_TB(0, 1); }
#undef NSK_TB
}
void tri_blk_level(hipStream_t s, const TriBlk &M, int b0, int b1, int lower, int kind, const double *intra,
                   const int *permn, const double *rhs, double *x) {
  tri_blk_level_t(s, M, b0, b1, lower, kind, intra, permn, rhs, x);
}
void tri_blk_level(hipStream_t s, const TriBlk32 &M, int b0, int b1, int lower, int kind, const double *intra,
                   const int *permn, const double *rhs, double *x) {
  tri_blk_level_t(s, M, b0, b1, lower, kind, intra, permn, rhs, x);
}

void spmv_blk_stream(hipStream_t s, const BlkView &A, int R, int C, const int *rowblk, int nblk, const double *xo,
                     const double *xg, double *y, const double *epi_d, const double *epi_dinv) {
  if (nblk <= 0) return;
  if (epi_d) {
    hipLaunchKernelGGL((spmv_blk_kernel<double, 2, 1, 1>), dim3(nblk), dim3(BLK), 0, s, A, rowblk, xo, xg, y, epi_d, epi_dinv);
    return;
  }
#define NSK_BK(RR, CC) hipLaunchKernelGGL((spmv_blk_kernel<double, RR, CC, 0>), dim3(nblk), dim3(BLK), 0, s, A, rowblk, xo, xg, y, nullptr, nullptr)
  if (R == 2 && C == 2) NSK_BK(2, 2);
  else if (R == 2 && C == 1) NSK_BK(2, 1);
  else if (R == 1 && C == 2) NSK_BK(1, 2);
  else NSK_BK(1, 1);
#undef NSK_BK
}

void spmv_blk_stream(hipStream_t s, const BlkView32 &A, const int *rowblk, int nblk, const double *xo, const double *xg,
                     double *y) {
  if (nblk > 0)
    hipLaunchKernelGGL((spmv_blk_kernel<float, 2, 2, 0>), dim3(nblk), dim3(BLK), 0, s, A, rowblk, xo, xg, y, nullptr, nullptr);
}

void spmv_blk_fused22_21(hipStream_t s, const BlkView &A, const double *xao, const double *xag, const BlkView &B,
                         const double *xbo, const double *xbg, const int *rowblk, int nblk, double *y) {
  if (nblk > 0)
    hipLaunchKernelGGL(spmv_blk_fused_kernel, dim3(nblk), dim3(BLK), 0, s, A, xao, xag, B, xbo, xbg, rowblk, y);
}

template <class V>
static void tri_stream_level_t(hipStream_t s, const TriHalfT<V> &M, int b0, int b1, int lower, int kind, int run_nnz,
                               const double *dinv, const int *perm, const double *rhs, double *w) {
  const int nb = b1 - b0;
  if (nb <= 0) return;
  const int grid = ((nb + 7) / 8) * 8;
#define NSK_TS(L, K, N) hipLaunchKernelGGL((tri_stream_kernel<V, L, K, N>), dim3(grid), dim3(BLK), 0, s, M, b0, nb, dinv, perm, rhs, w)
#define NSK_TSN(L, K)                                            \
  do {                                                           \
    if (M.off16) hipLaunchKernelGGL((tri_stream_kernel<V, L, K, 2048, 1>), dim3(grid), dim3(BLK), 0, s, M, b0, nb, dinv, perm, rhs, w); \
    else if (run_nnz <= 512) NSK_TS(L, K, 512);                  \
    else if (run_nnz <= 1024) NSK_TS(L, K, 1024);                \
    else NSK_TS(L, K, 2048);                                     \
  } while (0)
  if (lower) { if (kind == 0) NSK_TSN(1, 0); else NSK_TSN(1, 1); }
  else { if (kind == 0) NSK_TSN(0, 0); else NSK_TSN(0, 1); }
#undef NSK_TSN
#undef NSK_TS
}
void tri_stream_level(hipStream_t s, const TriHalf &M, int b0, int b1, int lower, int kind, int run_nnz,
                      const double *dinv, const int *perm, const double *rhs, double *w) {
  tri_stream_level_t(s, M, b0, b1, lower, kind, run_nnz, dinv, perm, rhs, w);
}
void tri_stream_level(hipStream_t s, const TriHalf32 &M, int b0, int b1, int lower, int kind, int run_nnz,
                      const double *dinv, const int *perm, const double *rhs, double *w) {
  tri_stream_level_t(s, M, b0, b1, lower, kind, run_nnz, dinv, perm, rhs, w);
}

#define NSK_EW(n, ...)                                                                       \
  do {                                                                                       \
    if ((n) > 0) {                                                                           \
      auto f__ = __VA_ARGS__;                                                                \
      hipLaunchKernelGGL((ew_kernel<decltype(f__)>), dim3(ew_grid(n)), dim3(BLK), 0, s, n, f__); \
    }                                                                                        \
  } while (0)

void vec_set(hipStream_t s, int n, double *y, double v) { NSK_EW(n, [=] __device__(int i) { y[i] = v; }); }
void vec_copy(hipStream_t s, int n, const double *x, double *y) { NSK_EW(n, [=] __device__(int i) { y[i] = x[i]; }); }
void vec_equ(hipStream_t s, int n, SRef a, const double *x, double *y) {
  NSK_EW(n, [=] __device__(int i) { y[i] = sval(a) * x[i]; });
}
void vec_axpy(hipStream_t s, int n, SRef a, const double *x, double *y) {
  NSK_EW(n, [=] __device__(int i) { y[i] += sval(a) * x[i]; });
}
void vec_sadd(hipStream_t s, int n, SRef sc, SRef a, const double *x, double *y) {
  NSK_EW(n, [=] __device__(int i) { y[i] = sval(sc) * y[i] + sval(a) * x[i]; });
}
void vec_axpy2(hipStream_t s, int n, SRef a, const double *x, SRef b, const double *z, double *y) {
  NSK_EW(n, [=] __device__(int i) { y[i] += sval(a) * x[i] + sval(b) * z[i]; });
}
void vec_scale(hipStream_t s, int n, SRef a, double *y) { NSK_EW(n, [=] __device__(int i) { y[i] *= sval(a); }); }
void vec_mul(hipStream_t s, int n, const double *d, double *y) { NSK_EW(n, [=] __device__(int i) { y[i] *= d[i]; }); }
void vec_submul(hipStream_t s, int n, const double *d, const double *x, double *y) {
  NSK_EW(n, [=] __device__(int i) { y[i] -= d[i] * x[i]; });
}
void vec_sub_then_mul(hipStream_t s, int n, const double *x, const double *d, double *y) {
  NSK_EW(n, [=] __device__(int i) { y[i] = (y[i] - x[i]) * d[i]; });
}
void vec_recip(hipStream_t s, int n, const double *x, double *y) {
  NSK_EW(n, [=] __device__(int i) { y[i] = 1.0 / x[i]; });
}
void vec_cheby_step(hipStream_t s, int n, double c1, double c2, const double *dinv, const double *r, double *w,
                    double *x, int set_x) {
  NSK_EW(n, [=] __device__(int i) {
    const double wi = (c1 != 0.0 ? c1 * w[i] : 0.0) + c2 * dinv[i] * r[i];
    w[i] = wi;
    x[i] = set_x ? wi : x[i] + wi;
  });
}

__global__ __launch_bounds__(BLK) void dense_mv_kernel(int n, const double *__restrict__ M, const double *__restrict__ b,
                                                       double *__restrict__ x) {
  const int row = (int)(blockIdx.x * (BLK / 64) + threadIdx.x / 64), lane = threadIdx.x % 64;
  double sum = 0.0;
  if (row < n)
    for (int j = lane; j < n; j += 64) sum += M[(size_t)row * n + j] * b[j];
  sum = subwave_sum<64>(sum);
  if (row < n && lane == 0) x[row] = sum;
}
void dense_mv(hipStream_t s, int n, const double *M, const double *b, double *x) {
  if (n <= 0) return;
// ... 593 lines not shown
```

### navier_stokes_solver_amd/csrc/nsk_precond.cpp

```cpp
#include <algorithm>
#include <exception>
#include <thread>

#include <omp.h>
#include "nsk_handle.hpp"

void H::schur_symbolic() {
  Csr &B = blk[NSK_BLK_B], &Bt = blk[NSK_BLK_BT], &Btg = blk[NSK_BLK_BT_GHOST], &S = blk[NSK_BLK_S];
  if (!Bt.present) throw Error(-41, "aSIMPLE needs block (0,1)");
  if (sp[0].ng > 0 && !Btg.present) throw Error(-42, "aSIMPLE on several ranks needs NSK_BLK_BT_GHOST");
  const int np = B.n_rows, ncols = sp[1].n + sp[1].ng;
  bool on_device = !tS.host_analysis && sp[0].ng == 0 && sp[1].ng == 0 && B.n_cols == Bt.n_rows && np > 0;
  DBuf<int> rp_d, col_d;
  int64_t nnz_s = 0;
  if (on_device) {
    try {
      nnz_s = device_product_pattern(&ctx, B, Bt, rp_d, col_d);
    } catch (const Error &e) {
      if (verbose()) fprintf(stderr, "[nsk] Schur pattern on the device: %s — host loop instead\n", e.what());
      on_device = false;
    }
  }
  if (on_device) {
    S.n_rows = np;
// ... 239 lines not shown
  const DVec su = ub(src.own), spv = pb(src.own);
  const int nu = n_u(), np = n_p();
  MatVec A_F = [&](const DVec &x, double *y) { spmv_halo(F, 0, x, y); };
  PrecVmult P_F = [&](DVec &d, const DVec &r) {
    if (amg_active) { amg_ready(); amgF.apply(r.own, d.own); }
    else tri_apply_sampled(tF, 20, r.own, d.own);
  };
  PrecVmult P_P = [&](DVec &d, const DVec &r) { tri_apply_sampled(*tP, 21, r.own, d.own); };
  const SlotLease sl(ctx, 4);
  auto norm_of = [&](const double *v, int n) { ctx.norm2(n, v, sl); return ctx.read_slots(sl + 1, 1)[0]; };

  if (prec_type == 0 || prec_type == 1) {
    Csr &Mp = blk[NSK_BLK_MP];
    MatVec A_M = [&](const DVec &x, double *y) { spmv_halo(Mp, 1, x, y); };
    int max_u, max_p;
    double tol_u, tol_p;
    if (prec_type == 0) {
      if (variant == 0) { max_u = 100001; max_p = 100000; tol_u = 1e-1 * norm_of(su.own, nu); tol_p = 1e-1 * norm_of(spv.own, np); }
      else { max_u = max_p = 1000; tol_u = tol_p = 1e-1; }
    } else {
      if (variant == 0) { max_u = 10000001; max_p = 100000; tol_u = 1e-2 * norm_of(su.own, nu); tol_p = 1e-2 * norm_of(spv.own, np); }
      else { max_u = 2000001; max_p = 2000000; tol_u = 1e-4 * norm_of(su.own, nu); tol_p = 1e-5 * norm_of(spv.own, np); }
    }
    SolverControl cu(max_u, tol_u), cp(max_p, tol_p);
    try {
      SolverFGMRES sv(ctx, pool_u, cu);
      inner_fgmres_options(sv);
      sv.solve(A_F, du, su, P_F);
      inner_u += cu.last_step();
      if (prec_type == 0) {
        SolverCG sc(ctx, pool_p, cp);
        sc.fused = cg_fused;
        sc.solve(A_M, dp, spv, P_P);
      } else {
        halo(0, du);
        spmv_nohalo(B, du, tmp_p, 2, spv.own);
        DVec tp = pool_p.view(tmp_p);
        SolverCG sc(ctx, pool_p, cp);
        sc.fused = cg_fused;
        sc.solve(A_M, dp, tp, P_P);
      }
      inner_p += cp.last_step();
    } catch (NoConvergence &e) {
      throw NoConvergence(3, e.last_step, e.last_residual);
    }
    return;
  }
  if (variant == 0) {
    Csr &S = blk[NSK_BLK_S];
    MatVec A_S = [&](const DVec &x, double *y) { spmv_halo(S, 1, x, y); };
    try {
      SolverControl cF(100000, 1e-1 * norm_of(su.own, nu));
      SolverFGMRES sF(ctx, pool_u, cF);
      inner_fgmres_options(sF);
      sF.solve(A_F, du, su, P_F);
      inner_u += cF.last_step();
      halo(0, du);
      spmv_nohalo(B, du, tmp_p, 2, spv.own);
      SolverControl cS(100000, 1e-1 * norm_of(tmp_p, np));
      SolverCG sS(ctx, pool_p, cS);
      sS.fused = cg_fused;
      DVec dlt = pool_p.view(delta_p), tp = pool_p.view(tmp_p);
      sS.solve(A_S, dlt, tp, P_P);
      inner_p += cS.last_step();
    } catch (NoConvergence &e) {
      throw NoConvergence(3, e.last_step, e.last_residual);
    }
    vec_scale(s(), np, sref(alpha), delta_p);
    DVec dlt = pool_p.view(delta_p);
    halo(1, dlt);
    spmv_nohalo(Bt, dlt, tmp_u, 0);
    vec_submul(s(), nu, Dinv, tmp_u, du.own);
    vec_copy(s(), np, delta_p, dp.own);
    return;
  }
  tri_apply_sampled(tF, 20, su.own, du.own);
  halo(0, du);
  spmv_nohalo(B, du, tmp_p, 1, spv.own);
  tri_apply_sampled(*tP, 21, tmp_p, dp.own);
  vec_scale(s(), np, sref(1.0 / alpha), dp.own);
  halo(1, dp);
  Csr &BT = Bt;
  if (BT.blk_ok && use_stream && use_bsr && BT.blk_R == 2 && BT.blk_C == 1) {
    nsk::spmv_blk_stream(s(), BT.blk_view(), 2, 1, BT.blk_rowblk.p, BT.blk_nblk, dp.own, dp.ghost, du.own, D, Dinv);
    ++ctx.st.spmv_calls;
    ctx.st.spmv_bytes += (double)BT.spmv_bytes() + 24.0 * nu;
  } else {
    vec_mul(s(), nu, D, du.own);
    spmv_nohalo(Bt, dp, tmp_u, 0);
    vec_sub_then_mul(s(), nu, tmp_u, Dinv, du.own);
  }
}

int H::solve_once(int solver, double tol, int max_iter, int *iters, double *final_res) {
  SolverControl control(max_iter, tol);
  control.progress_step = &progress_step;
  control.progress_value = &progress_value;
  history.clear();
  control.history = &history;
  control.cancel = &cancel;
  MatVec A = [&](const DVec &x, double *y) { jacobian_vmult(x, y); };
  PrecVmult P = [&](DVec &d, const DVec &r) { prec_vmult(d, r); };
  DVec x = bb(x_b);
  const DVec b = bb(rhs_b);
  int rc = 0;
  const int slot_mark = ctx.slot_top;
  SolverFGMRES::Pending left_over;
  struct Keep {
    H &h; SolverFGMRES::Pending &p;
    ~Keep() { if (p.v) { h.drop_pending(); h.pending = p; } }
  } keep{*this, left_over};
  try {
    if (solver == 0) { SolverGMRES sv(ctx, pool_b, control); sv.solve(A, x, b, P); }
    else if (solver == 1) {
      SolverFGMRES sv(ctx, pool_b, control);
      sv.fused_gs = outer_fused_gs ? 1 : 0;
      if (skip_unused) {
        const bool asimple = prec_type == 2;
        sv.skip_unused = asimple && variant != 0 ? SolverFGMRES::stateless : SolverFGMRES::defer;
        if (asimple && variant == 0) sv.pending = &left_over;
      }
      sv.solve(A, x, b, P);
    }
    else { SolverBicgstab sv(ctx, pool_b, control); sv.solve(A, x, b, P); }
  } catch (NoConvergence &e) {
    rc = e.code;
  }
  ctx.slot_top = slot_mark;
  ctx.sync();
  check_sync_free();
  outer_iters += control.last_step();
  if (iters) *iters = control.last_step();
  if (final_res) *final_res = control.last_value();
  return rc;
}

int H::solve_resident(int solver, double tol, int max_iter, int *iters, double *final_res) {
  if (prec_type < 0) throw Error(-46, "call nsk_setup_preconditioner first");
  if (solver < 0 || solver > 2) throw Error(-47, "Invalid solver type. Use 0: GMRES, 1: FGMRES, 2: Bicgstab.");
  const double t0 = wall_ms();
  lazy_setup_ms = 0;
  cancel = 0;
  const bool guarded = sync_free_mode > 0;
  if (guarded) {
    if (!x_keep) x_keep = pool_b.get(false);
    vec_copy(s(), N(), x_b, x_keep);
  }
  int rc;
  try {
    rc = solve_once(solver, tol, max_iter, iters, final_res);
  } catch (const Error &e) {
    if (e.code != -70 || !guarded) throw;
    const long undo = outer_iters;
    sync_free_mode = 0;
    ++sync_free_fallbacks;
    ctx.warn("single-launch triangular solve: a producer/consumer wait ran out of spins (workgroups not resident in "
             "dispatch order: another process on the GPU?); the solve is redone from the caller's initial guess with one "
             "launch per colour — factors re-ordered WITHOUT line groups, which only the single-launch kernels know — and "
             "this handle keeps that slower path (NSK_OPT_TRI_SYNC_FREE = 0)");
    setup(prec_type, variant, alpha);
    vec_copy(s(), N(), x_keep, x_b);
    outer_iters = undo;
    rc = solve_once(solver, tol, max_iter, iters, final_res);
  }
  solve_ms = wall_ms() - t0 - lazy_setup_ms;
  return rc;
}
// ... 1 lines not shown
```

### navier_stokes_solver_amd/solver.py

```python
from __future__ import annotations

import ctypes as C
import os

import numpy as np

_HERE = os.path.dirname(os.path.abspath(__file__))
_LIB = None

BLK_F, BLK_BT, BLK_B, BLK_MP, BLK_BT_GHOST, BLK_S = range(6)
SPACE_U, SPACE_P = 0, 1
GMRES, FGMRES, BICGSTAB = 0, 1, 2
BLOCK_DIAGONAL, BLOCK_TRIANGULAR, ASIMPLE = 0, 1, 2
STATIONARY, UNSTEADY = 0, 1
TRI_VELOCITY, TRI_PRESSURE = 0, 1
OPT_TRI_ORDERING, OPT_SUBDOMAINS, OPT_FUSE_BLOCK_ROW, OPT_STREAM_KERNELS = 0, 1, 2, 3
OPT_INNER_FUSED_GS, OPT_OUTER_FUSED_GS, OPT_BSR_VELOCITY = 4, 5, 7
OPT_TRI_SYNC_FREE = 9
OPT_VELOCITY_AMG = 10
OPT_CG_SINGLE_REDUCTION = 11
IOPT_TRI_X_LAYOUT, IOPT_FAULT_INJECT, IOPT_TINY_BYTES = 6, 100, 102
OPT_TRI_LINE_GROUPS, IOPT_GROUP_U, IOPT_GROUP_P = 12, 103, 104
OPT_MASS_ORDERING = 13
OPT_BLAS1_PAIRS = 15
OPT_SCHUR_SIGN = 14
OPT_FACTOR_PRECISION = 16
OPT_INNER_MATRIX_PRECISION = 17
OPT_INNER_BASIS_PRECISION = 18
OPT_INNER_MATRIX_FREE_F = 19
TIMEOP_MATFREE_F = 56
TIMEOP_INNER_SPMV = 50
IOPT_FUSED_MGS, IOPT_OVERLAP_HALO = 106, 107
IOPT_TIMEOP_BETWEEN = 109
IOPT_INDEX16 = 110
IOPT_GS_ONE_LAUNCH = 111
IOPT_FGMRES_SKIP_UNUSED = 112
IOPT_HOST_ANALYSIS = 108
ORDER_NATURAL, ORDER_MULTICOLOR = 0, 1

EXPORTS = [
    "nsk_get_unique_id", "nsk_local_group_id", "nsk_create", "nsk_destroy", "nsk_last_error", "nsk_set_partition", "nsk_set_halo_plan",
    "nsk_set_support_points",
    "nsk_set_block_csr", "nsk_update_values", "nsk_set_option", "nsk_setup_preconditioner", "nsk_solve",
    "nsk_upload_system", "nsk_solve_resident", "nsk_download_solution", "nsk_spmv", "nsk_jacobian_vmult", "nsk_dot", "nsk_vec_op",
    "nsk_tri_apply", "nsk_amg_info", "nsk_tri_get_perm", "nsk_tri_get_value_bytes", "nsk_inner_value_bytes", "nsk_inner_basis_bytes", "nsk_inner_matrix_free", "nsk_matfree_f", "nsk_inner_spmv", "nsk_precond_vmult", "nsk_block_nnz", "nsk_get_block", "nsk_get_stats",
    "nsk_reset_stats", "nsk_get_history", "nsk_cancel", "nsk_abort_group", "nsk_assembly_set_cells", "nsk_assembly_set_simplex", "nsk_assembly_set_dirichlet", "nsk_state_set", "nsk_state_get",
    "nsk_state_save", "nsk_state_save_old", "nsk_state_update", "nsk_assemble", "nsk_scale_values", "nsk_download_rhs", "nsk_time_assemble", "nsk_time_op", "nsk_profile_begin", "nsk_profile_read", "nsk_profile_end",
    "nsk_debug_spmv_form",
    "nsk_forces_set_faces", "nsk_forces_set_edges", "nsk_forces", "nsk_state_get_patches",
    "nsk_record_set_cells", "nsk_state_get_record",
]


class Stats(C.Structure):
    _fields_ = [("setup_ms", C.c_double), ("solve_ms", C.c_double),
                ("outer_iters", C.c_int64), ("inner_u_its", C.c_int64), ("inner_p_its", C.c_int64),
                ("prec_applies", C.c_int64), ("spmv_calls", C.c_int64), ("tri_applies", C.c_int64),
                ("reductions", C.c_int64), ("host_syncs", C.c_int64),
                ("spmv_bytes", C.c_double), ("tri_bytes", C.c_double), ("blas1_bytes", C.c_double),
                ("n_colors_u", C.c_int32), ("n_levels_u", C.c_int32), ("n_colors_p", C.c_int32),
                ("n_levels_p", C.c_int32), ("nnz_s", C.c_int64), ("sync_free_fallbacks", C.c_int64),
                ("cur_outer_iters", C.c_int64), ("cur_residual", C.c_double), ("overlapped_spmvs", C.c_int64),
                ("ring_applies", C.c_int64), ("columns_skipped", C.c_int64)]


class NoConvergence(RuntimeError):

    def __init__(self, status, last_step, last_residual):
        super().__init__(f"solver did not converge (status {status}, step {last_step}, residual {last_residual:g})")
        self.status, self.last_step, self.last_residual = status, last_step, last_residual


def library_path() -> str:
    return os.environ.get("NSK_HIP_LIBRARY") or os.path.join(_HERE, "libnsk_hip.so")


def lib() -> C.CDLL:
    global _LIB
    if _LIB is None:
        path = library_path()
        if not os.path.exists(path):
            raise RuntimeError(f"{path} missing — the HIP extension is required (run __graft_entry__.build())")
        try:
            import torch
        except ImportError:
            pass
        L = C.CDLL(path, mode=C.RTLD_GLOBAL)
        vp, i32p, f64p = C.c_void_p, C.c_void_p, C.c_void_p
        L.nsk_get_unique_id.argtypes = [vp]
        L.nsk_local_group_id.argtypes = [C.c_int, vp]
        L.nsk_create.restype = vp
        L.nsk_create.argtypes = [C.c_int, C.c_int, C.c_int, vp]
        L.nsk_destroy.argtypes = [vp]
        L.nsk_last_error.restype = C.c_char_p
        L.nsk_last_error.argtypes = [vp]
        L.nsk_set_partition.argtypes = [vp, C.c_int, C.c_int64, C.c_int64, C.c_int, i32p]
        L.nsk_set_halo_plan.argtypes = [vp, C.c_int, C.c_int, i32p, i32p, i32p, i32p]
        L.nsk_set_support_points.argtypes = [vp, C.c_int, vp]
        L.nsk_set_block_csr.argtypes = [vp, C.c_int, C.c_int, C.c_int, i32p, i32p, f64p]
        L.nsk_update_values.argtypes = [vp, C.c_int, f64p]
        L.nsk_set_option.argtypes = [vp, C.c_int, C.c_double]
        L.nsk_setup_preconditioner.argtypes = [vp, C.c_int, C.c_int, C.c_double]
        L.nsk_solve.argtypes = [vp, C.c_int, C.c_double, C.c_int, f64p, f64p, f64p, f64p, C.POINTER(C.c_int),
                                C.POINTER(C.c_double)]
        L.nsk_upload_system.argtypes = [vp, f64p, f64p, f64p, f64p]
        L.nsk_solve_resident.argtypes = [vp, C.c_int, C.c_double, C.c_int, C.POINTER(C.c_int), C.POINTER(C.c_double)]
        L.nsk_download_solution.argtypes = [vp, f64p, f64p]
        L.nsk_spmv.argtypes = [vp, C.c_int, f64p, f64p, C.c_int]
        L.nsk_jacobian_vmult.argtypes = [vp, f64p, f64p, f64p, f64p]
        L.nsk_dot.argtypes = [vp, C.c_int, f64p, f64p, C.POINTER(C.c_double), C.POINTER(C.c_double)]
        L.nsk_vec_op.argtypes = [vp, C.c_int, C.c_int, C.c_double, C.c_double, f64p, f64p, f64p, f64p, C.POINTER(C.c_double)]
        L.nsk_assembly_set_cells.argtypes = [vp, C.c_int64, i32p, i32p, vp, f64p, C.c_int32]
        L.nsk_assembly_set_dirichlet.argtypes = [vp, vp, f64p]
        L.nsk_state_set.argtypes = [vp, f64p, f64p]
        L.nsk_state_get.argtypes = [vp, f64p, f64p]
        L.nsk_state_save.argtypes = [vp]
        L.nsk_state_save_old.argtypes = [vp]
        L.nsk_state_update.argtypes = [vp, C.c_double]
        L.nsk_assemble.argtypes = [vp, C.c_int, C.c_double, C.c_double, C.c_double, C.c_int, C.POINTER(C.c_double)]
        L.nsk_scale_values.argtypes = [vp, C.c_int, C.c_double]
        L.nsk_forces_set_faces.argtypes = [vp, C.c_int64, i32p, vp, f64p]
        L.nsk_forces_set_edges.argtypes = [vp, C.c_int64, i32p, vp, f64p]
        L.nsk_forces.argtypes = [vp, C.c_double, f64p, f64p]
        L.nsk_state_get_patches.argtypes = [vp, C.c_int64, i32p, f64p, f64p]
        L.nsk_record_set_cells.argtypes = [vp, C.c_int64, i32p, C.c_int, f64p, f64p]
        L.nsk_state_get_record.argtypes = [vp, C.c_int64, f64p, f64p]
        L.nsk_download_rhs.argtypes = [vp, f64p, f64p]
        L.nsk_time_assemble.argtypes = [vp, C.c_double, C.c_double, C.c_int, C.POINTER(C.c_double)]
        L.nsk_amg_info.argtypes = [vp, C.c_int, C.c_int, C.POINTER(C.c_int64), C.POINTER(C.c_int64),
                                   C.POINTER(C.c_double)]
        L.nsk_tri_apply.argtypes = [vp, C.c_int, f64p, f64p]
        L.nsk_tri_get_perm.argtypes = [vp, C.c_int, i32p]
        L.nsk_tri_get_value_bytes.argtypes = [vp, C.c_int, C.POINTER(C.c_int32)]
        L.nsk_inner_value_bytes.argtypes = [vp, C.c_int, C.POINTER(C.c_int32)]
        L.nsk_inner_basis_bytes.argtypes = [vp, C.POINTER(C.c_int32)]
        L.nsk_inner_matrix_free.argtypes = [vp, C.POINTER(C.c_int32)]
        L.nsk_matfree_f.argtypes = [vp, f64p, f64p]
        L.nsk_inner_spmv.argtypes = [vp, C.c_int, f64p, f64p]
        L.nsk_precond_vmult.argtypes = [vp, f64p, f64p, f64p, f64p, C.c_int]
        L.nsk_block_nnz.restype = C.c_int64
        L.nsk_block_nnz.argtypes = [vp, C.c_int]
        L.nsk_get_block.argtypes = [vp, C.c_int, i32p, i32p, f64p]
        L.nsk_get_stats.argtypes = [vp, C.POINTER(Stats)]
        L.nsk_reset_stats.argtypes = [vp]
        L.nsk_get_history.argtypes = [vp, f64p, C.c_int]
        L.nsk_cancel.argtypes = [vp]
        L.nsk_time_op.argtypes = [vp, C.c_int, C.c_int, C.POINTER(C.c_double), C.POINTER(C.c_double)]
        L.nsk_profile_begin.argtypes = [vp, C.c_int, C.c_int]
        L.nsk_profile_read.argtypes = [vp, C.c_int, C.POINTER(C.c_double), C.POINTER(C.c_int), C.POINTER(C.c_double),
                                       C.POINTER(C.c_int64), C.POINTER(C.c_double)]
        L.nsk_profile_end.argtypes = [vp]
        _LIB = L
    return _LIB


def _f64(a):
    return np.ascontiguousarray(a, dtype=np.float64)


def _i32(a):
    return np.ascontiguousarray(a, dtype=np.int32)


def get_unique_id() -> bytes:
    buf = C.create_string_buffer(128)
    rc = lib().nsk_get_unique_id(buf)
    if rc != 0:
        raise RuntimeError(f"nsk_get_unique_id failed: {rc}")
    return buf.raw


def tri_ordering_host(csr, xy=None, group=1, want_block2=False, sub_off=None):
    L = lib()
    n = int(csr.rows)
    rp, col = _i32(csr.rowptr), _i32(csr.col)
    perm = np.empty(n, np.int32)
    info = np.zeros(4, np.int32)
    chain = np.zeros(n, np.uint8)
    a = None if xy is None else np.ascontiguousarray(xy, dtype=np.float64)
    so = None if sub_off is None else _i32(sub_off)
    L.nsk_debug_tri_ordering.argtypes = [C.c_int, C.c_void_p, C.c_void_p, C.c_int, C.c_void_p, C.c_int, C.c_void_p, C.c_int,
                                         C.c_void_p, C.c_void_p, C.c_void_p]
    rc = L.nsk_debug_tri_ordering(n, rp.ctypes.data, col.ctypes.data, 0 if so is None else len(so) - 1,
                                  None if so is None else so.ctypes.data, int(want_block2), None if a is None else a.ctypes.data,
                                  int(group), perm.ctypes.data, info.ctypes.data, chain.ctypes.data)
    if rc != 0:
        raise RuntimeError("nsk_debug_tri_ordering failed")
    return perm, int(info[0]), int(info[1]), bool(info[2]), chain[:int(info[3])]


SPMV_FORMS = ("csr_vector", "stream", "stream_f32", "blk", "blk_f32")


def spmv_form(blk_ok, stream_ok, inner32, use_stream, use_bsr, mode, inner) -> str:
    L = lib()
    L.nsk_debug_spmv_form.argtypes = [C.c_int] * 7
    return SPMV_FORMS[L.nsk_debug_spmv_form(int(blk_ok), int(stream_ok), int(inner32), int(use_stream), int(use_bsr), int(mode),
                                            int(inner))]


def local_group_id(nranks: int, on_stream: bool = False) -> bytes:
    buf = C.create_string_buffer(128)
    L = lib()
    L.nsk_local_group_id_mode.argtypes = [C.c_int, C.c_int, C.c_void_p]
    if L.nsk_local_group_id_mode(nranks, 1 if on_stream else 0, buf) != 0:
        raise RuntimeError("nsk_local_group_id failed")
    return buf.raw


def abort_local_group(unique_id: bytes) -> None:
    L = lib()
    L.nsk_abort_local_group.argtypes = [C.c_void_p]
    L.nsk_abort_local_group(C.c_char_p(unique_id))


class LinearSolver:

    def __init__(self, rank: int = 0, nranks: int = 1, device: int = 0, unique_id: bytes | None = None):
        self.L = lib()
        self.rank, self.nranks = rank, nranks
        uid = C.create_string_buffer(unique_id, 128) if unique_id is not None else None
        self.h = self.L.nsk_create(rank, nranks, device, uid)
        if not self.h:
            raise RuntimeError("nsk_create failed (no usable GPU / RCCL?) — there is no CPU fallback")
        self.n_u = self.n_p = 0

    def close(self):
        if getattr(self, "h", None):
            self.L.nsk_destroy(self.h)
            self.h = None

    def __del__(self):
        try:
            self.close()
        except Exception:
            pass

    def last_error(self) -> str:
        return self.L.nsk_last_error(self.h).decode()

    def _ck(self, rc, allow=()):
        if rc < 0 or (rc > 0 and rc not in allow):
            raise RuntimeError(f"nsk error {rc}: {self.L.nsk_last_error(self.h).decode()}")
        return rc

    def set_partition(self, space, begin, end, ghost_gids):
        g = _i32(ghost_gids)
        self._ck(self.L.nsk_set_partition(self.h, space, int(begin), int(end), len(g), g.ctypes.data))

    def set_halo_plan(self, space, peers, send_ptr, send_idx, recv_ptr):
        p, sp_, si, rp = _i32(peers), _i32(send_ptr), _i32(send_idx), _i32(recv_ptr)
        self._ck(self.L.nsk_set_halo_plan(self.h, space, len(p), p.ctypes.data, sp_.ctypes.data, si.ctypes.data,
                                          rp.ctypes.data))

    def set_support_points(self, space, xy):
        if xy is None:
            self._ck(self.L.nsk_set_support_points(self.h, space, None))
            return
        a = np.ascontiguousarray(xy, dtype=np.float64)
        n = self.n_u if space == SPACE_U else self.n_p
        if a.shape != (n, 2):
            raise ValueError(f"support points of space {space}: expected shape ({n}, 2), got {a.shape}")
        self._ck(self.L.nsk_set_support_points(self.h, space, a.ctypes.data))

    def set_block(self, blk, csr):
        rp, col, val = _i32(csr.rowptr), _i32(csr.col), _f64(csr.val)
        self._ck(self.L.nsk_set_block_csr(self.h, blk, int(csr.rows), int(csr.cols), rp.ctypes.data, col.ctypes.data,
                                          val.ctypes.data))

    def update_values(self, blk, val):
        v = _f64(val)
        self._ck(self.L.nsk_update_values(self.h, blk, v.ctypes.data))

    def set_problem(self, pr, plan=None):
        info = pr.info
        self.n_u, self.n_p = pr.n_u, pr.n_p
        self.set_partition(SPACE_U, info["u_begin"], info["u_end"], pr.ghost_u)
        self.set_partition(SPACE_P, info["p_begin"], info["p_end"], pr.ghost_p)
        if plan is not None:
            for space in (SPACE_U, SPACE_P):
                pl = plan[space]
                self.set_halo_plan(space, pl["peers"], pl["send_ptr"], pl["send_idx"], pl["recv_ptr"])
        if getattr(pr, "support_u", None) is not None and getattr(pr, "support_p", None) is not None:
# ... 307 lines not shown
```

Before: 11.48 million.

## Precompute int4 run descriptors and stage stream SpMV loads branch-free

Replaces the per-block rowblk index array with precomputed int4 descriptors that carry both the row range and the nnz range of each stream block. The kernels no longer need dependent rowptr loads at block start. The stream product staging is restructured into a StreamStage helper with clamped, branch-free loads and a staged flag, and products are stored relative to the block start. This is meant to cut launch-prologue latency and divergence in the SpMV kernels, at the cost of extra descriptor memory and more complex kernel code.

Result: slower. 11.21 million (-2.3%).

```diff
diff --git a/include/nsk.h b/include/nsk.h
--- a/include/nsk.h
+++ b/include/nsk.h
@@ -106,6 +106,7 @@
 int64_t nsk_block_nnz(nsk_handle h, int blk);
 int nsk_get_block(nsk_handle h, int blk, int32_t *rowptr, int32_t *col, double *val);
 int nsk_debug_spmv_form(int blk_ok, int stream_ok, int inner32, int use_stream, int use_bsr, int mode, int inner);
+int nsk_debug_stream_slots(int pairs, int k0, int k1, int32_t *out4);
 
 int nsk_assembly_set_cells(nsk_handle h, int64_t n_cells, const int32_t *cell_u_nodes, const int32_t *cell_p_dofs,
                            const uint8_t *cell_flags, const double *tables944, int32_t cell_of_dof0);
diff --git a/navier_stokes_solver_amd/csrc/nsk_core.cpp b/navier_stokes_solver_amd/csrc/nsk_core.cpp
--- a/navier_stokes_solver_amd/csrc/nsk_core.cpp
+++ b/navier_stokes_solver_amd/csrc/nsk_core.cpp
@@ -591,10 +591,10 @@
   if (c1 <= c0) return 0;
   const int *cb = off16.p ? colbase.p + c0 : nullptr;
   switch (f) {
-    case SpmvForm::blk_f32: nsk::spmv_blk_stream(s, blk_view32(), blk_rowblk.p + c0, c1 - c0, xo, xg, y); return 0;
-    case SpmvForm::blk: nsk::spmv_blk_stream(s, blk_view(), blk_R, blk_C, blk_rowblk.p + c0, c1 - c0, xo, xg, y); return 0;
-    case SpmvForm::stream_f32: return nsk::spmv_stream(s, view32(), rowblk.p + c0, c1 - c0, even_rows, xo, xg, y, off16.p, cb);
-    default: return nsk::spmv_stream(s, view(), rowblk.p + c0, c1 - c0, even_rows, xo, xg, y, mode, z, off16.p, cb);
+    case SpmvForm::blk_f32: nsk::spmv_blk_stream(s, blk_view32(), blk_desc.p + c0, c1 - c0, xo, xg, y); return 0;
+    case SpmvForm::blk: nsk::spmv_blk_stream(s, blk_view(), blk_R, blk_C, blk_desc.p + c0, c1 - c0, xo, xg, y); return 0;
+    case SpmvForm::stream_f32: return nsk::spmv_stream(s, view32(), desc.p + c0, c1 - c0, even_rows, xo, xg, y, off16.p, cb);
+    default: return nsk::spmv_stream(s, view(), desc.p + c0, c1 - c0, even_rows, xo, xg, y, mode, z, off16.p, cb);
   }
 }
 
@@ -632,6 +632,16 @@
   return true;
 }
 
+std::vector<int4> run_descriptors(const std::vector<int> &rb, const int *ra, const int *rpb) {
+  const size_t nb = rb.empty() ? 0 : rb.size() - 1, per = rpb ? 2 : 1;
+  std::vector<int4> d(nb * per);
+  for (size_t b = 0; b < nb; ++b) {
+    d[per * b] = make_int4(rb[b], rb[b + 1], ra[rb[b]], ra[rb[b + 1]]);
+    if (rpb) d[2 * b + 1] = make_int4(rb[b], rb[b + 1], rpb[rb[b]], rpb[rb[b + 1]]);
+  }
+  return d;
+}
+
 void Csr::find_interior() {
   int_r0 = int_r1 = 0;
   if (n_cols == n_own_cols) { int_r1 = n_rows; return; }
@@ -670,13 +680,15 @@
   if (int_r0 > 0) cuts.push_back(int_r0);
   if (int_r1 < n_rows && int_r1 > int_r0) cuts.push_back(int_r1);
   stream_ok = n_rows > 0 && build_rowblocks(h_rowptr.data(), nullptr, n_rows, kStreamNnz, cuts.empty() ? nullptr : &cuts, rb);
-  if (!stream_ok) { nblk = 0; return; }
+  if (!stream_ok) { nblk = 0; desc.release(); return; }
   nblk = (int)rb.size() - 1;
   interior_runs(rb, int_r0, int_r1, int_b0, int_b1);
   even_rows = true;
   for (int i = 0; i <= n_rows; ++i)
     if (h_rowptr[i] & 1) { even_rows = false; break; }
   rowblk.upload(rb, s);
+  desc.upload(run_descriptors(rb, h_rowptr.data()), s);
+  NSK_HIP(hipStreamSynchronize(s));
   off16.release();
   colbase.release();
   idx16_wide = false;
@@ -762,6 +774,7 @@
   blk_col.upload(bcol, s);
   blk_src.upload(bsrc, s);
   blk_rowblk.upload(rb, s);
+  blk_desc.upload(run_descriptors(rb, rp.data()), s);
   blk_val.alloc((size_t)blk_count * R * C);
   NSK_HIP(hipStreamSynchronize(s));
   blk_ok = true;
diff --git a/navier_stokes_solver_amd/csrc/nsk_core.hpp b/navier_stokes_solver_amd/csrc/nsk_core.hpp
--- a/navier_stokes_solver_amd/csrc/nsk_core.hpp
+++ b/navier_stokes_solver_amd/csrc/nsk_core.hpp
@@ -124,6 +124,7 @@
   int lpr = 16;
   bool present = false;
   DBuf<int> rowblk;
+  DBuf<int4> desc;
   int nblk = 0;
   bool stream_ok = false, even_rows = false;
   void build_stream_plan(hipStream_t s);
@@ -138,6 +139,7 @@
   int64_t blk_count = 0;
   std::vector<int> h_blk_rowptr;
   DBuf<int> blk_rowptr, blk_col, blk_src, blk_rowblk;
+  DBuf<int4> blk_desc;
   DBuf<double> blk_val;
   void build_blocked(int R, int C, hipStream_t s);
   void refresh_blocked(hipStream_t s);
@@ -170,6 +172,8 @@
 
 bool build_rowblocks(const int *rowptr_a, const int *rowptr_b, int n_rows, int max_nnz, const std::vector<int> *cuts,
                      std::vector<int> &rowblk, const unsigned char *glue = nullptr);
+
+std::vector<int4> run_descriptors(const std::vector<int> &rowblk, const int *rowptr_a, const int *rowptr_b = nullptr);
 
 inline int pick_lpr(int64_t nnz, int n_rows) {
   const double mean = n_rows > 0 ? (double)nnz / n_rows : 0.0;
diff --git a/navier_stokes_solver_amd/csrc/nsk_debug.cpp b/navier_stokes_solver_amd/csrc/nsk_debug.cpp
--- a/navier_stokes_solver_amd/csrc/nsk_debug.cpp
+++ b/navier_stokes_solver_amd/csrc/nsk_debug.cpp
@@ -362,14 +362,13 @@
 
   std::vector<int> rb;
   const std::vector<int> *ea = &A.h_rowptr, *eb = nullptr;
-  DBuf<int> fused_rb;
-  const int *d_rb = nullptr;
+  DBuf<int4> fused_desc;
+  const int4 *d_desc = nullptr;
   int ib0 = 0, ib1 = 0, refused = 0;
   auto download = [&](const DBuf<int> &src, int nblk) {
     rb.resize((size_t)nblk + 1);
     NSK_HIP(hipMemcpyAsync(rb.data(), src.p, sizeof(int) * rb.size(), hipMemcpyDeviceToHost, st));
     c.sync();
-    d_rb = src.p;
   };
   const bool i16 = form == NSK_DBG_SPMV_STREAM_I16 || form == NSK_DBG_SPMV_STREAM_I16_F32;
   if (form == NSK_DBG_SPMV_STREAM || form == NSK_DBG_SPMV_STREAM_F32 || i16) {
@@ -382,7 +381,7 @@
   } else if (form == NSK_DBG_SPMV_STREAM2) {
     if (!A.even_rows) refused = 3;
     else if (!fused_row_plan(A, B, rb)) refused = 4;
-    else { eb = &B.h_rowptr; fused_rb.upload(rb, st); d_rb = fused_rb.p; ib1 = (int)rb.size() - 1; }
+    else { eb = &B.h_rowptr; fused_desc.upload(run_descriptors(rb, A.h_rowptr.data(), B.h_rowptr.data()), st); d_desc = fused_desc.p; ib1 = (int)rb.size() - 1; }
   } else if (blocked) {
     A.build_blocked(R, C, st);
     if (two) B.build_blocked(2, 1, st);
@@ -390,8 +389,12 @@
     if (!info[7] || (two && A.blk_rows != B.blk_rows)) refused = 2;
     else if (two) {
       if (!fused_blk_plan(A, B, rb)) refused = 4;
-      else { ea = &A.h_blk_rowptr; eb = &B.h_blk_rowptr; fused_rb.upload(rb, st); d_rb = fused_rb.p; ib1 = (int)rb.size() - 1; }
-    } else { download(A.blk_rowblk, A.blk_nblk); ea = &A.h_blk_rowptr; ib0 = A.blk_int_b0; ib1 = A.blk_int_b1; }
+      else {
+        ea = &A.h_blk_rowptr; eb = &B.h_blk_rowptr;
+        fused_desc.upload(run_descriptors(rb, A.h_blk_rowptr.data(), B.h_blk_rowptr.data()), st);
+        d_desc = fused_desc.p; ib1 = (int)rb.size() - 1;
+      }
+    } else { download(A.blk_rowblk, A.blk_nblk); d_desc = A.blk_desc.p; ea = &A.h_blk_rowptr; ib0 = A.blk_int_b0; ib1 = A.blk_int_b1; }
   }
   info[15] = refused;
   if (refused) return 1;
@@ -446,13 +449,13 @@
       A.spmv_launch(st, SpmvForm::blk_f32, xa.p, xag.p, yv.p, 0, nullptr, c0, c1);
       break;
     case NSK_DBG_SPMV_BLK21_EPI:
-      nsk::spmv_blk_stream(st, A.blk_view(), 2, 1, d_rb + c0, n_run, xa.p, xag.p, yv.p, dv.p, div.p);
+      nsk::spmv_blk_stream(st, A.blk_view(), 2, 1, d_desc + c0, n_run, xa.p, xag.p, yv.p, dv.p, div.p);
       break;
     case NSK_DBG_SPMV_STREAM2:
-      info[1] = nsk::spmv2_stream(st, A.view(), xa.p, xag.p, B.view(), xb.p, xbg.p, d_rb, nblk, yv.p);
+      info[1] = nsk::spmv2_stream(st, A.view(), xa.p, xag.p, B.view(), xb.p, xbg.p, d_desc, nblk, yv.p);
       break;
     case NSK_DBG_SPMV_BLK_FUSED:
-      nsk::spmv_blk_fused22_21(st, A.blk_view(), xa.p, xag.p, B.blk_view(), xb.p, xbg.p, d_rb, nblk, yv.p);
+      nsk::spmv_blk_fused22_21(st, A.blk_view(), xa.p, xag.p, B.blk_view(), xb.p, xbg.p, d_desc, nblk, yv.p);
       break;
   }
   NSK_HIP(hipGetLastError());
@@ -641,6 +644,21 @@
   return (int)spmv_form(blk_ok != 0, stream_ok != 0, inner32, use_stream != 0, use_bsr != 0, mode, inner != 0);
 }
 
+int nsk_debug_stream_slots(int pairs, int k0, int k1, int32_t *out4) {
+  if (!nsk::stream_staged(pairs != 0, k0, k1)) return 0;
+  const int n = pairs ? nsk::kStreamNnz / 2 : nsk::kStreamNnz;
+  for (int p = 0; p < n; ++p) {
+    if (pairs) {
+      const nsk::StreamPair s = nsk::stream_pair(k0, k1, p);
+      out4[4 * p] = s.ka; out4[4 * p + 1] = s.odd_last; out4[4 * p + 2] = s.st0; out4[4 * p + 3] = s.st1;
+    } else {
+      const nsk::StreamSingle s = nsk::stream_single(k0, k1, p);
+      out4[4 * p] = s.ka; out4[4 * p + 1] = 0; out4[4 * p + 2] = s.st; out4[4 * p + 3] = 0;
+    }
+  }
+  return n;
+}
+
 int nsk_debug_pool_counts(nsk_handle h, int32_t *out6) {
   int k = 0;
   for (const VecPool *p : {&h->pool_u, &h->pool_p, &h->pool_b}) {
diff --git a/navier_stokes_solver_amd/csrc/nsk_handle.hpp b/navier_stokes_solver_amd/csrc/nsk_handle.hpp
--- a/navier_stokes_solver_amd/csrc/nsk_handle.hpp
+++ b/navier_stokes_solver_amd/csrc/nsk_handle.hpp
@@ -124,7 +124,7 @@
   int x_layout_mode = 2;
   int sync_free_mode = 2;
   int fault_inject = 0;
-  DBuf<int> jrow_blk, jblk_blk;
+  DBuf<int4> jrow_desc, jblk_desc;
   int jrow_nblk = 0, jblk_nblk = 0;
   bool jrow_ok = false, jblk_ok = false;
 
@@ -347,7 +347,7 @@
       std::vector<int> rb;
       if (fused_blk_plan(F, Bt, rb)) {
         jblk_nblk = (int)rb.size() - 1;
-        jblk_blk.upload(rb, s());
+        jblk_desc.upload(run_descriptors(rb, F.h_blk_rowptr.data(), Bt.h_blk_rowptr.data()), s());
         ctx.sync();
         jblk_ok = true;
       } else jblk_nblk = -1;
@@ -356,19 +356,19 @@
       std::vector<int> rb;
       if (fused_row_plan(F, Bt, rb)) {
         jrow_nblk = (int)rb.size() - 1;
-        jrow_blk.upload(rb, s());
+        jrow_desc.upload(run_descriptors(rb, F.h_rowptr.data(), Bt.h_rowptr.data()), s());
         ctx.sync();
         jrow_ok = true;
       } else jrow_nblk = -1;
     }
     const double fused_bytes = (double)F.spmv_bytes() + (double)Bt.spmv_bytes() - 8.0 * F.n_rows - 4.0 * (F.n_rows + 1);
     if (fuse_block_row && blocked && jblk_ok) {
-      nsk::spmv_blk_fused22_21(s(), F.blk_view(), xu.own, xu.ghost, Bt.blk_view(), xp.own, xp.ghost, jblk_blk.p,
+      nsk::spmv_blk_fused22_21(s(), F.blk_view(), xu.own, xu.ghost, Bt.blk_view(), xp.own, xp.ghost, jblk_desc.p,
                                jblk_nblk, yb);
       ctx.st.spmv_calls += 2;
       ctx.st.spmv_bytes += fused_bytes;
     } else if (fuse_block_row && use_stream && jrow_ok) {
-      nsk::spmv2_stream(s(), F.view(), xu.own, xu.ghost, Bt.view(), xp.own, xp.ghost, jrow_blk.p, jrow_nblk, yb);
+      nsk::spmv2_stream(s(), F.view(), xu.own, xu.ghost, Bt.view(), xp.own, xp.ghost, jrow_desc.p, jrow_nblk, yb);
       ctx.st.spmv_calls += 2;
       ctx.st.spmv_bytes += fused_bytes;
     } else {
diff --git a/navier_stokes_solver_amd/csrc/nsk_internal.h b/navier_stokes_solver_amd/csrc/nsk_internal.h
--- a/navier_stokes_solver_amd/csrc/nsk_internal.h
+++ b/navier_stokes_solver_amd/csrc/nsk_internal.h
@@ -100,6 +100,7 @@
 int nsk_debug_amg(struct nsk_handle_s *h, const struct nsk_dbg_amg_args *a, int32_t *info16);
 int nsk_debug_index_width(struct nsk_handle_s *h, int b, int32_t *out3);
 int nsk_debug_spmv_form(int blk_ok, int stream_ok, int inner32, int use_stream, int use_bsr, int mode, int inner);
+int nsk_debug_stream_slots(int pairs, int k0, int k1, int32_t *out4);
 int nsk_debug_pool_counts(struct nsk_handle_s *h, int32_t *out6);
 enum { NSK_DBG_ASM_CQ = 0, NSK_DBG_ASM_D0 = 1, NSK_DBG_ASM_NODE_CELLS = 2, NSK_DBG_ASM_NODE_OFF = 3,
        NSK_DBG_ASM_NODE_SELF = 4, NSK_DBG_ASM_PDOF_CELLS = 5 };
diff --git a/navier_stokes_solver_amd/csrc/nsk_kernels.h b/navier_stokes_solver_amd/csrc/nsk_kernels.h
--- a/navier_stokes_solver_amd/csrc/nsk_kernels.h
+++ b/navier_stokes_solver_amd/csrc/nsk_kernels.h
@@ -36,13 +36,31 @@
 
 constexpr int kStreamNnz = 2048;
 constexpr int kStreamRows = 64;
-int spmv_stream(hipStream_t s, const CsrView &A, const int *rowblk, int nblk, int even_rows, const double *x_own,
+struct StreamPair {
+  int ka;
+  bool odd_last, st0, st1;
+};
+__host__ __device__ inline StreamPair stream_pair(int k0, int k1, int p) {
+  const int k = k0 + 2 * p;
+  return StreamPair{k < k1 - 2 ? k : k1 - 2, k == k1 - 1, k < k1, k + 1 < k1};
+}
+struct StreamSingle {
+  int ka;
+  bool st;
+};
+__host__ __device__ inline StreamSingle stream_single(int k0, int k1, int p) {
+  const int k = k0 + p;
+  return StreamSingle{k < k1 - 1 ? k : k1 - 1, k < k1};
+}
+__host__ __device__ inline bool stream_staged(bool pairs, int k0, int k1) { return k1 - k0 >= (pairs ? 2 : 1); }
+
+int spmv_stream(hipStream_t s, const CsrView &A, const int4 *desc, int nblk, int even_rows, const double *x_own,
                 const double *x_ghost, double *y, int mode, const double *z, const unsigned short *off16 = nullptr,
                 const int *colbase = nullptr);
-int spmv_stream(hipStream_t s, const CsrView32 &A, const int *rowblk, int nblk, int even_rows, const double *x_own,
+int spmv_stream(hipStream_t s, const CsrView32 &A, const int4 *desc, int nblk, int even_rows, const double *x_own,
                 const double *x_ghost, double *y, const unsigned short *off16 = nullptr, const int *colbase = nullptr);
 int spmv2_stream(hipStream_t s, const CsrView &A, const double *xa_own, const double *xa_ghost, const CsrView &B,
-                 const double *xb_own, const double *xb_ghost, const int *rowblk, int nblk, double *y);
+                 const double *xb_own, const double *xb_ghost, const int4 *desc2, int nblk, double *y);
 
 template <class V>
 struct BlkViewT {
@@ -55,12 +73,12 @@
 using BlkView = BlkViewT<double>;
 using BlkView32 = BlkViewT<float>;
 constexpr int kBlkMax = 1024;
-void spmv_blk_stream(hipStream_t s, const BlkView &A, int R, int C, const int *rowblk, int nblk, const double *x_own,
+void spmv_blk_stream(hipStream_t s, const BlkView &A, int R, int C, const int4 *desc, int nblk, const double *x_own,
                      const double *x_ghost, double *y, const double *epi_d = nullptr, const double *epi_dinv = nullptr);
-void spmv_blk_stream(hipStream_t s, const BlkView32 &A, const int *rowblk, int nblk, const double *x_own,
+void spmv_blk_stream(hipStream_t s, const BlkView32 &A, const int4 *desc, int nblk, const double *x_own,
                      const double *x_ghost, double *y);
 void spmv_blk_fused22_21(hipStream_t s, const BlkView &A, const double *xa_own, const double *xa_ghost,
-                         const BlkView &B, const double *xb_own, const double *xb_ghost, const int *rowblk, int nblk,
+                         const BlkView &B, const double *xb_own, const double *xb_ghost, const int4 *desc2, int nblk,
                          double *y);
 
 void vec_set(hipStream_t s, int n, double *y, double v);
diff --git a/navier_stokes_solver_amd/csrc/nsk_kernels.hip b/navier_stokes_solver_amd/csrc/nsk_kernels.hip
--- a/navier_stokes_solver_amd/csrc/nsk_kernels.hip
+++ b/navier_stokes_solver_amd/csrc/nsk_kernels.hip
@@ -68,9 +68,6 @@
 }
 
 constexpr int RG = 4;
-
-__device__ __forceinline__ double2 widen2(double2 v) { return v; }
-__device__ __forceinline__ double2 widen2(float2 v) { return make_double2((double)v.x, (double)v.y); }
 
 template <class I>
 struct IdxPair;
@@ -92,84 +89,84 @@
 };
 
 template <class V, int VEC, class I = int>
-__device__ __forceinline__ void stream_products(const I *__restrict__ col, const V *__restrict__ val, int k0,
-                                                int k1, int n_own, const double *__restrict__ xo,
-                                                const double *__restrict__ xg, double *prod, int base = 0) {
-  if (VEC == 3) {
-    constexpr int U = kStreamNnz / (2 * BLK);
-    typedef V vv2 __attribute__((ext_vector_type(2)));
-    typedef vv2 vd2u __attribute__((aligned(sizeof(V))));
-    int c0[U], c1[U];
-    double v0[U], v1[U], x0[U], x1[U];
+struct StreamStage {
+  static constexpr bool kPairs = VEC != 1;
+  static constexpr int U = kPairs ? kStreamNnz / (2 * BLK) : kStreamNnz / BLK;
+  typedef V vv2 __attribute__((ext_vector_type(2)));
+  typedef vv2 vv2u __attribute__((aligned(sizeof(V))));
+  typedef typename std::conditional<VEC == 3, typename IdxPair<I>::unaligned, typename IdxPair<I>::aligned2>::type QLoad;
+  typedef typename std::conditional<VEC == 3, vv2u, vv2>::type WLoad;
+  const I *__restrict__ col;
+  const V *__restrict__ val;
+  int k0, k1, base;
+  bool staged;
+  typename IdxPair<I>::v2 q[kPairs ? U : 1];
+  vv2 w[kPairs ? U : 1];
+  I c[kPairs ? 1 : U];
+  V v[kPairs ? 1 : U];
+  double x0[U], x1[kPairs ? U : 1];
+  double e0[kPairs ? U : 1], e1[kPairs ? U : 1];
+
+  __device__ __forceinline__ void init(const I *__restrict__ col_, const V *__restrict__ val_, int k0_, int k1_, int base_ = 0) {
+    col = col_; val = val_; k0 = k0_; k1 = k1_; base = base_;
+    staged = stream_staged(kPairs, k0, k1);
+  }
+  __device__ __forceinline__ void load() {
 #pragma unroll
     for (int u = 0; u < U; ++u) {
-      const int k = k0 + 2 * ((int)threadIdx.x + u * BLK);
-      if (k + 1 < k1) {
-        const IdxPair<I> ci(*reinterpret_cast<const typename IdxPair<I>::unaligned *>(col + k), base);
-        const vv2 vi = *reinterpret_cast<const vd2u *>(val + k);
-        c0[u] = ci.a; c1[u] = ci.b; v0[u] = (double)vi[0]; v1[u] = (double)vi[1];
+      if constexpr (kPairs) {
+        const int ka = stream_pair(k0, k1, (int)threadIdx.x + u * BLK).ka;
+        q[u] = *reinterpret_cast<const QLoad *>(col + ka);
+        w[u] = *reinterpret_cast<const WLoad *>(val + ka);
       } else {
-        const bool ok = k < k1;
-        c0[u] = ok ? base + (int)col[k] : 0; v0[u] = ok ? (double)val[k] : 0.0; c1[u] = 0; v1[u] = 0.0;
-      }
-    }
+        const int ka = stream_single(k0, k1, (int)threadIdx.x + u * BLK).ka;
+        c[u] = col[ka];
+        v[u] = val[ka];
+      }
+    }
+  }
+  __device__ __forceinline__ void gather(int n_own, const double *__restrict__ xo, const double *__restrict__ xg) {
 #pragma unroll
     for (int u = 0; u < U; ++u) {
-      x0[u] = *(c0[u] < n_own ? xo + c0[u] : xg + (c0[u] - n_own));
-      x1[u] = *(c1[u] < n_own ? xo + c1[u] : xg + (c1[u] - n_own));
-    }
+      if constexpr (kPairs) {
+        const StreamPair s = stream_pair(k0, k1, (int)threadIdx.x + u * BLK);
+        const IdxPair<I> ci(q[u], base);
+        const int ca = VEC == 3 && s.odd_last ? ci.b : ci.a, cb = ci.b;
+        e0[u] = VEC == 3 && s.odd_last ? (double)w[u][1] : (double)w[u][0];
+        e1[u] = (double)w[u][1];
+        x0[u] = *(ca < n_own ? xo + ca : xg + (ca - n_own));
+        x1[u] = *(cb < n_own ? xo + cb : xg + (cb - n_own));
+      } else {
+        const int ca = base + (int)c[u];
+        x0[u] = *(ca < n_own ? xo + ca : xg + (ca - n_own));
+      }
+    }
+  }
+  __device__ __forceinline__ void lone(int n_own, const double *__restrict__ xo, const double *__restrict__ xg, double *prod) const {
+    if (kPairs && k1 - k0 == 1 && threadIdx.x == 0) {
+      const int ca = base + (int)col[k0];
+      prod[0] = (double)val[k0] * *(ca < n_own ? xo + ca : xg + (ca - n_own));
+    }
+  }
+  __device__ __forceinline__ void alone(int n_own, const double *__restrict__ xo, const double *__restrict__ xg, double *prod) {
+    if (staged) { load(); gather(n_own, xo, xg); store(prod); }
+    else lone(n_own, xo, xg, prod);
+  }
+  __device__ __forceinline__ void store(double *prod) const {
 #pragma unroll
     for (int u = 0; u < U; ++u) {
-      const int k = k0 + 2 * ((int)threadIdx.x + u * BLK);
-      if (k < k1) prod[k - k0] = v0[u] * x0[u];
-      if (k + 1 < k1) prod[k - k0 + 1] = v1[u] * x1[u];
-    }
-  } else if (VEC == 2) {
-    constexpr int U = kStreamNnz / (2 * BLK);
-    typedef typename std::conditional<std::is_same<V, double>::value, double2, float2>::type V2;
-    int2 c[U];
-    double2 v[U];
-#pragma unroll
-    for (int u = 0; u < U; ++u) {
-      const int k = k0 + 2 * ((int)threadIdx.x + u * BLK);
-      const bool ok = k < k1;
-      if (ok) {
-        const IdxPair<I> ci(*reinterpret_cast<const typename IdxPair<I>::aligned2 *>(col + k), base);
-        c[u] = make_int2(ci.a, ci.b);
-      } else c[u] = make_int2(0, 0);
-      v[u] = ok ? widen2(*reinterpret_cast<const V2 *>(val + k)) : make_double2(0.0, 0.0);
-    }
-    double x0[U], x1[U];
-#pragma unroll
-    for (int u = 0; u < U; ++u) {
-      x0[u] = *(c[u].x < n_own ? xo + c[u].x : xg + (c[u].x - n_own));
-      x1[u] = *(c[u].y < n_own ? xo + c[u].y : xg + (c[u].y - n_own));
-    }
-#pragma unroll
-    for (int u = 0; u < U; ++u) {
-      const int k = k0 + 2 * ((int)threadIdx.x + u * BLK);
-      if (k < k1) { prod[k - k0] = v[u].x * x0[u]; prod[k - k0 + 1] = v[u].y * x1[u]; }
-    }
-  } else {
-    constexpr int U = kStreamNnz / BLK;
-    int c[U];
-    double v[U], xv[U];
-#pragma unroll
-    for (int u = 0; u < U; ++u) {
-      const int k = k0 + (int)threadIdx.x + u * BLK;
-      const bool ok = k < k1;
-      c[u] = ok ? base + (int)col[k] : 0;
-      v[u] = ok ? (double)val[k] : 0.0;
-    }
-#pragma unroll
-    for (int u = 0; u < U; ++u) xv[u] = *(c[u] < n_own ? xo + c[u] : xg + (c[u] - n_own));
-#pragma unroll
-    for (int u = 0; u < U; ++u) {
-      const int k = k0 + (int)threadIdx.x + u * BLK;
-      if (k < k1) prod[k - k0] = v[u] * xv[u];
-    }
-  }
-}
+      if constexpr (kPairs) {
+        const StreamPair s = stream_pair(k0, k1, (int)threadIdx.x + u * BLK);
+        const int j = 2 * ((int)threadIdx.x + u * BLK);
+        if (s.st0) prod[j] = e0[u] * x0[u];
+        if (s.st1) prod[j + 1] = e1[u] * x1[u];
+      } else {
+        const int j = (int)threadIdx.x + u * BLK;
+        if (stream_single(k0, k1, j).st) prod[j] = (double)v[u] * x0[u];
+      }
+    }
+  }
+};
 
 __device__ __forceinline__ double row_sum_lds(const double *prod, int b, int e, int lane) {
   double s = 0.0;
@@ -186,31 +183,44 @@
 }
 
 template <class V, int VEC, int MODE, class I = int>
-__global__ __launch_bounds__(BLK) void spmv_stream_kernel(CsrViewT<V> A, const int *__restrict__ rowblk,
+__global__ __launch_bounds__(BLK) void spmv_stream_kernel(CsrViewT<V> A, const int4 *__restrict__ desc,
                                                           const double *__restrict__ xo,
                                                           const double *__restrict__ xg, double *__restrict__ y,
                                                           const double *__restrict__ z,
-                                                          const unsigned short *__restrict__ off16 = nullptr,
-                                                          const int *__restrict__ colbase = nullptr) {
+                                                          const unsigned short *__restrict__ off16,
+                                                          const int *__restrict__ colbase) {
   __shared__ double prod[kStreamNnz];
-  const int r0 = rowblk[blockIdx.x], r1 = rowblk[blockIdx.x + 1];
   constexpr bool I16 = std::is_same<I, unsigned short>::value;
+  const int4 d = desc[blockIdx.x];
   const int base = I16 ? colbase[blockIdx.x] : 0;
-  const int k0 = A.rowptr[r0], k1 = A.rowptr[r1];
+  const int r0 = d.x, r1 = d.y, k0 = d.z, k1 = d.w;
   const int r = r0 + (int)threadIdx.x / RG, lane = threadIdx.x % RG;
   const bool have = r < r1;
+  const I *col;
+  if constexpr (I16) col = off16; else col = A.col;
+  StreamStage<V, VEC, I> st;
+  st.init(col, A.val, k0, k1, base);
   int jb = 0, je = 0;
   double zv = 0.0;
-  if (have) {
-    jb = A.rowptr[r] - k0;
-    je = A.rowptr[r + 1] - k0;
-    if (MODE == 1) zv = z ? z[r] : y[r];
-    if (MODE == 2) zv = z[r];
-  }
-  if constexpr (I16) stream_products<V, VEC, unsigned short>(off16, A.val, k0, k1, A.n_own_cols, xo, xg, prod, base);
-  else stream_products<V, VEC>(A.col, A.val, k0, k1, A.n_own_cols, xo, xg, prod);
+  auto bounds = [&]() {
+    if (have) {
+      jb = A.rowptr[r];
+      je = A.rowptr[r + 1];
+      if (MODE == 1) zv = z ? z[r] : y[r];
+      if (MODE == 2) zv = z[r];
+    }
+  };
+  if (st.staged) {
+    st.load();
+    bounds();
+    st.gather(A.n_own_cols, xo, xg);
+    st.store(prod);
+  } else {
+    bounds();
+    st.lone(A.n_own_cols, xo, xg, prod);
+  }
   __syncthreads();
-  const double sum = row_sum_lds(prod, jb, je, lane);
+  const double sum = row_sum_lds(prod, have ? jb - k0 : 0, have ? je - k0 : 0, lane);
   if (have && lane == 0) {
     if (MODE == 0) y[r] = sum;
     else if (MODE == 1) y[r] = zv + sum;
@@ -223,96 +233,134 @@
                                                            const double *__restrict__ xag, CsrView B,
                                                            const double *__restrict__ xbo,
                                                            const double *__restrict__ xbg,
-                                                           const int *__restrict__ rowblk, double *__restrict__ y) {
+                                                           const int4 *__restrict__ desc, double *__restrict__ y) {
   __shared__ double prod[kStreamNnz];
-  const int r0 = rowblk[blockIdx.x], r1 = rowblk[blockIdx.x + 1];
-  const int a0 = A.rowptr[r0], a1 = A.rowptr[r1], b0 = B.rowptr[r0], b1 = B.rowptr[r1];
+  const int4 da = desc[2 * blockIdx.x], db = desc[2 * blockIdx.x + 1];
+  const int r0 = da.x, r1 = da.y, a0 = da.z, a1 = da.w, b0 = db.z, b1 = db.w;
   const int r = r0 + (int)threadIdx.x / RG, lane = threadIdx.x % RG;
   const bool have = r < r1;
+  double *prodB = prod + (a1 - a0);
+  StreamStage<double, VECA> sa;
+  StreamStage<double, 1> sb;
+  sa.init(A.col, A.val, a0, a1);
+  sb.init(B.col, B.val, b0, b1);
   int ab = 0, ae = 0, bb = 0, be = 0;
-  if (have) {
-    ab = A.rowptr[r] - a0; ae = A.rowptr[r + 1] - a0;
-    bb = B.rowptr[r] - b0; be = B.rowptr[r + 1] - b0;
-  }
-  stream_products<double, VECA>(A.col, A.val, a0, a1, A.n_own_cols, xao, xag, prod);
-  double *prodB = prod + (a1 - a0);
-  stream_products<double, 1>(B.col, B.val, b0, b1, B.n_own_cols, xbo, xbg, prodB);
+  auto bounds = [&]() {
+    if (have) {
+      ab = A.rowptr[r]; ae = A.rowptr[r + 1];
+      bb = B.rowptr[r]; be = B.rowptr[r + 1];
+    }
+  };
+  if (sa.staged) {
+    sa.load();
+    bounds();
+    sa.gather(A.n_own_cols, xao, xag);
+    sa.store(prod);
+  } else {
+    bounds();
+    sa.lone(A.n_own_cols, xao, xag, prod);
+  }
+  sb.alone(B.n_own_cols, xbo, xbg, prodB);
   __syncthreads();
   double sum = 0.0;
-  for (int j = ab + lane; j < ae; j += RG) sum += prod[j];
-  for (int j = bb + lane; j < be; j += RG) sum += prodB[j];
+  if (have) {
+    for (int j = ab - a0 + lane; j < ae - a0; j += RG) sum += prod[j];
+    for (int j = bb - b0 + lane; j < be - b0; j += RG) sum += prodB[j];
+  }
   sum = subwave_sum<RG>(sum);
   if (have && lane == 0) y[r] = sum;
 }
 
 template <class V, int R, int C>
-__device__ __forceinline__ void blk_products(const BlkViewT<V> &A, int k0, int k1, const double *__restrict__ xo,
-                                             const double *__restrict__ xg, double *p0, double *p1) {
-  constexpr int U = kBlkMax / BLK;
-  if (k0 >= k1) return;
+struct BlkStage {
+  static constexpr int U = kBlkMax / BLK;
+  static constexpr bool kF32 = std::is_same<V, float>::value;
+  static_assert(!kF32 || (R == 2 && C == 2), "fp32 values: 2 x 2 blocks only");
+  const BlkViewT<V> &A;
+  int k0, k1;
+  bool staged;
   int m[U];
-  double2 a0[U], a1[U];
+  typename std::conditional<kF32, float4, double2>::type w0[U];
+  double2 w1[!kF32 && R * C == 4 ? U : 1];
   double x0[U], x1[U];
-#pragma unroll
-  for (int u = 0; u < U; ++u) {
-    const int k = k0 + (int)threadIdx.x + u * BLK;
-    const bool ok = k < k1;
-    m[u] = ok ? __builtin_nontemporal_load(A.col + k) : 0;
-    const V *v = A.val + (size_t)(R * C) * (ok ? k : k0);
-    if constexpr (std::is_same<V, float>::value) {
-      static_assert(R == 2 && C == 2, "fp32 values: 2 x 2 blocks only");
-      const float4 q = *reinterpret_cast<const float4 *>(v);
-      a0[u] = make_double2((double)q.x, (double)q.y); a1[u] = make_double2((double)q.z, (double)q.w);
-    } else {
-      if (R * C == 4) { a0[u] = *reinterpret_cast<const double2 *>(v); a1[u] = *reinterpret_cast<const double2 *>(v + 2); }
-      else if (R * C == 2) { a0[u] = *reinterpret_cast<const double2 *>(v); a1[u] = make_double2(0.0, 0.0); }
-      else { a0[u] = make_double2(v[0], 0.0); a1[u] = make_double2(0.0, 0.0); }
-    }
-  }
-#pragma unroll
-  for (int u = 0; u < U; ++u) {
-    x1[u] = 0.0;
-    if (C == 2) {
-      if (m[u] < A.n_own_bcols) {
-        const double2 xv = *reinterpret_cast<const double2 *>(xo + 2 * (size_t)m[u]);
-        x0[u] = xv.x; x1[u] = xv.y;
+  __device__ __forceinline__ BlkStage(const BlkViewT<V> &A_, int k0_, int k1_) : A(A_), k0(k0_), k1(k1_), staged(k0_ < k1_) {}
+  __device__ __forceinline__ void load() {
+#pragma unroll
+    for (int u = 0; u < U; ++u) {
+      const int k = k0 + (int)threadIdx.x + u * BLK, kk = k < k1 ? k : k0;
+      m[u] = __builtin_nontemporal_load(A.col + kk);
+      const V *v = A.val + (size_t)(R * C) * kk;
+      if constexpr (kF32) w0[u] = *reinterpret_cast<const float4 *>(v);
+      else if constexpr (R * C == 4) { w0[u] = *reinterpret_cast<const double2 *>(v); w1[u] = *reinterpret_cast<const double2 *>(v + 2); }
+      else if constexpr (R * C == 2) w0[u] = *reinterpret_cast<const double2 *>(v);
+      else w0[u] = make_double2(v[0], 0.0);
+    }
+  }
+  __device__ __forceinline__ void gather(const double *__restrict__ xo, const double *__restrict__ xg) {
+#pragma unroll
+    for (int u = 0; u < U; ++u) {
+      x1[u] = 0.0;
+      if (C == 2) {
+        if (m[u] < A.n_own_bcols) {
+          const double2 xv = *reinterpret_cast<const double2 *>(xo + 2 * (size_t)m[u]);
+          x0[u] = xv.x; x1[u] = xv.y;
+        } else {
+          const size_t g = 2 * (size_t)(m[u] - A.n_own_bcols);
+          x0[u] = xg[g]; x1[u] = xg[g + 1];
+        }
       } else {
-        const size_t g = 2 * (size_t)(m[u] - A.n_own_bcols);
-        x0[u] = xg[g]; x1[u] = xg[g + 1];
-      }
-    } else {
-      x0[u] = *(m[u] < A.n_own_bcols ? xo + m[u] : xg + (m[u] - A.n_own_bcols));
-    }
-  }
-#pragma unroll
-  for (int u = 0; u < U; ++u) {
-    const int k = k0 + (int)threadIdx.x + u * BLK;
-    if (k < k1) {
-      if (R == 2 && C == 2) { p0[k - k0] = a0[u].x * x0[u] + a0[u].y * x1[u]; p1[k - k0] = a1[u].x * x0[u] + a1[u].y * x1[u]; }
-      else if (R == 2 && C == 1) { p0[k - k0] = a0[u].x * x0[u]; p1[k - k0] = a0[u].y * x0[u]; }
-      else if (R == 1 && C == 2) p0[k - k0] = a0[u].x * x0[u] + a0[u].y * x1[u];
-      else p0[k - k0] = a0[u].x * x0[u];
-    }
-  }
-}
+        x0[u] = *(m[u] < A.n_own_bcols ? xo + m[u] : xg + (m[u] - A.n_own_bcols));
+      }
+    }
+  }
+  __device__ __forceinline__ void store(double *p0, double *p1) const {
+#pragma unroll
+    for (int u = 0; u < U; ++u) {
+      const int k = k0 + (int)threadIdx.x + u * BLK;
+      double2 a0, a1 = make_double2(0.0, 0.0);
+      if constexpr (kF32) { a0 = make_double2((double)w0[u].x, (double)w0[u].y); a1 = make_double2((double)w0[u].z, (double)w0[u].w); }
+      else { a0 = w0[u]; if constexpr (R * C == 4) a1 = w1[u]; }
+      auto dot2 = [](double2 a, double x, double y) { return __fma_rn(a.x, x, __dmul_rn(a.y, y)); };
+      if (k < k1) {
+        if (R == 2 && C == 2) { p0[k - k0] = dot2(a0, x0[u], x1[u]); p1[k - k0] = dot2(a1, x0[u], x1[u]); }
+        else if (R == 2 && C == 1) { p0[k - k0] = a0.x * x0[u]; p1[k - k0] = a0.y * x0[u]; }
+        else if (R == 1 && C == 2) p0[k - k0] = dot2(a0, x0[u], x1[u]);
+        else p0[k - k0] = a0.x * x0[u];
+      }
+    }
+  }
+  __device__ __forceinline__ void alone(const double *__restrict__ xo, const double *__restrict__ xg, double *p0, double *p1) {
+    if (staged) { load(); gather(xo, xg); store(p0, p1); }
+  }
+};
 
 template <class V, int R, int C, int EPI>
-__global__ __launch_bounds__(BLK) void spmv_blk_kernel(BlkViewT<V> A, const int *__restrict__ rowblk,
+__global__ __launch_bounds__(BLK) void spmv_blk_kernel(BlkViewT<V> A, const int4 *__restrict__ desc,
                                                        const double *__restrict__ xo, const double *__restrict__ xg,
                                                        double *__restrict__ y, const double *__restrict__ d,
                                                        const double *__restrict__ dinv) {
   __shared__ double p0[kBlkMax];
   __shared__ double p1[R == 2 ? kBlkMax : 1];
-  const int r0 = rowblk[blockIdx.x], r1 = rowblk[blockIdx.x + 1];
-  const int k0 = A.rowptr[r0], k1 = A.rowptr[r1];
+  asm volatile("" ::"s"(A.col), "s"(A.val), "s"(A.rowptr));
+  const int4 ds = desc[blockIdx.x];
+  const int r0 = ds.x, r1 = ds.y, k0 = ds.z, k1 = ds.w;
   const int r = r0 + (int)threadIdx.x / RG, lane = threadIdx.x % RG;
   const bool have = r < r1;
+  BlkStage<V, R, C> st(A, k0, k1);
   int jb = 0, je = 0;
-  if (have) { jb = A.rowptr[r] - k0; je = A.rowptr[r + 1] - k0; }
-  blk_products<V, R, C>(A, k0, k1, xo, xg, p0, p1);
+  auto bounds = [&]() {
+    if (have) { jb = A.rowptr[r]; je = A.rowptr[r + 1]; }
+  };
+  if (st.staged) {
+    st.load();
+    bounds();
+    st.gather(xo, xg);
+    st.store(p0, p1);
+  } else jb = je = k0;
   __syncthreads();
   double s0 = 0.0, s1 = 0.0;
-  for (int j = jb + lane; j < je; j += RG) { s0 += p0[j]; if (R == 2) s1 += p1[j]; }
+  if (have)
+    for (int j = jb - k0 + lane; j < je - k0; j += RG) { s0 += p0[j]; if (R == 2) s1 += p1[j]; }
   s0 = subwave_sum<RG>(s0);
   if (R == 2) s1 = subwave_sum<RG>(s1);
   if (have && lane == 0) {
@@ -332,24 +380,35 @@
                                                              const double *__restrict__ xag, BlkView B,
                                                              const double *__restrict__ xbo,
                                                              const double *__restrict__ xbg,
-                                                             const int *__restrict__ rowblk, double *__restrict__ y) {
+                                                             const int4 *__restrict__ desc, double *__restrict__ y) {
   __shared__ double p0[kBlkMax];
   __shared__ double p1[kBlkMax];
-  const int r0 = rowblk[blockIdx.x], r1 = rowblk[blockIdx.x + 1];
-  const int a0 = A.rowptr[r0], a1 = A.rowptr[r1], b0 = B.rowptr[r0], b1 = B.rowptr[r1];
+  const int4 da = desc[2 * blockIdx.x], db = desc[2 * blockIdx.x + 1];
+  const int r0 = da.x, r1 = da.y, a0 = da.z, a1 = da.w, b0 = db.z, b1 = db.w;
   const int r = r0 + (int)threadIdx.x / RG, lane = threadIdx.x % RG;
   const bool have = r < r1;
+  BlkStage<double, 2, 2> sa(A, a0, a1);
+  BlkStage<double, 2, 1> sb(B, b0, b1);
   int ab = 0, ae = 0, bb = 0, be = 0;
-  if (have) {
-    ab = A.rowptr[r] - a0; ae = A.rowptr[r + 1] - a0;
-    bb = B.rowptr[r] - b0 + (a1 - a0); be = B.rowptr[r + 1] - b0 + (a1 - a0);
-  }
-  blk_products<double, 2, 2>(A, a0, a1, xao, xag, p0, p1);
-  blk_products<double, 2, 1>(B, b0, b1, xbo, xbg, p0 + (a1 - a0), p1 + (a1 - a0));
+  auto bounds = [&]() {
+    if (have) {
+      ab = A.rowptr[r]; ae = A.rowptr[r + 1];
+      bb = B.rowptr[r]; be = B.rowptr[r + 1];
+    }
+  };
+  if (sa.staged) {
+    sa.load();
+    bounds();
+    sa.gather(xao, xag);
+    sa.store(p0, p1);
+  } else bounds();
+  sb.alone(xbo, xbg, p0 + (a1 - a0), p1 + (a1 - a0));
   __syncthreads();
   double s0 = 0.0, s1 = 0.0;
-  for (int j = ab + lane; j < ae; j += RG) { s0 += p0[j]; s1 += p1[j]; }
-  for (int j = bb + lane; j < be; j += RG) { s0 += p0[j]; s1 += p1[j]; }
+  if (have) {
+    for (int j = ab - a0 + lane; j < ae - a0; j += RG) { s0 += p0[j]; s1 += p1[j]; }
+    for (int j = bb - b0 + (a1 - a0) + lane; j < be - b0 + (a1 - a0); j += RG) { s0 += p0[j]; s1 += p1[j]; }
+  }
   s0 = subwave_sum<RG>(s0);
   s1 = subwave_sum<RG>(s1);
   if (have && lane == 0) *reinterpret_cast<double2 *>(y + 2 * (size_t)r) = make_double2(s0, s1);
@@ -1509,13 +1568,13 @@
   }
 }
 
-int spmv_stream(hipStream_t s, const CsrView &A, const int *rowblk, int nblk, int even_rows, const double *xo,
+int spmv_stream(hipStream_t s, const CsrView &A, const int4 *desc, int nblk, int even_rows, const double *xo,
                 const double *xg, double *y, int mode, const double *z, const unsigned short *off16, const int *colbase) {
   if (nblk <= 0) return 0;
 #define NSK_SS(V, M)                                                                                                                   \
   do {                                                                                                                                 \
-    if (off16) hipLaunchKernelGGL((spmv_stream_kernel<double, V, M, unsigned short>), dim3(nblk), dim3(BLK), 0, s, A, rowblk, xo, xg, y, z, off16, colbase); \
-    else hipLaunchKernelGGL((spmv_stream_kernel<double, V, M, int>), dim3(nblk), dim3(BLK), 0, s, A, rowblk, xo, xg, y, z, off16, colbase); \
+    if (off16) hipLaunchKernelGGL((spmv_stream_kernel<double, V, M, unsigned short>), dim3(nblk), dim3(BLK), 0, s, A, desc, xo, xg, y, z, off16, colbase); \
+    else hipLaunchKernelGGL((spmv_stream_kernel<double, V, M, int>), dim3(nblk), dim3(BLK), 0, s, A, desc, xo, xg, y, z, off16, colbase); \
   } while (0)
   if (even_rows) {
     if (mode == 0) NSK_SS(2, 0); else if (mode == 1) NSK_SS(2, 1); else NSK_SS(2, 2);
@@ -1526,14 +1585,14 @@
 #undef NSK_SS
 }
 
-int spmv_stream(hipStream_t s, const CsrView32 &A, const int *rowblk, int nblk, int even_rows, const double *xo,
+int spmv_stream(hipStream_t s, const CsrView32 &A, const int4 *desc, int nblk, int even_rows, const double *xo,
                 const double *xg, double *y, const unsigned short *off16, const int *colbase) {
   if (nblk <= 0) return 0;
   const double *z = nullptr;
 #define NSK_SS(V)                                                                                                                      \
   do {                                                                                                                                 \
-    if (off16) hipLaunchKernelGGL((spmv_stream_kernel<float, V, 0, unsigned short>), dim3(nblk), dim3(BLK), 0, s, A, rowblk, xo, xg, y, z, off16, colbase); \
-    else hipLaunchKernelGGL((spmv_stream_kernel<float, V, 0, int>), dim3(nblk), dim3(BLK), 0, s, A, rowblk, xo, xg, y, z, off16, colbase); \
+    if (off16) hipLaunchKernelGGL((spmv_stream_kernel<float, V, 0, unsigned short>), dim3(nblk), dim3(BLK), 0, s, A, desc, xo, xg, y, z, off16, colbase); \
+    else hipLaunchKernelGGL((spmv_stream_kernel<float, V, 0, int>), dim3(nblk), dim3(BLK), 0, s, A, desc, xo, xg, y, z, off16, colbase); \
   } while (0)
   if (even_rows) { NSK_SS(2); return 2; }
   NSK_SS(3);
@@ -1542,9 +1601,9 @@
 }
 
 int spmv2_stream(hipStream_t s, const CsrView &A, const double *xao, const double *xag, const CsrView &B,
-                 const double *xbo, const double *xbg, const int *rowblk, int nblk, double *y) {
+                 const double *xbo, const double *xbg, const int4 *desc, int nblk, double *y) {
   if (nblk <= 0) return 0;
-  hipLaunchKernelGGL((spmv2_stream_kernel<2>), dim3(nblk), dim3(BLK), 0, s, A, xao, xag, B, xbo, xbg, rowblk, y);
+  hipLaunchKernelGGL((spmv2_stream_kernel<2>), dim3(nblk), dim3(BLK), 0, s, A, xao, xag, B, xbo, xbg, desc, y);
   return 2;
 }
 
@@ -1568,14 +1627,14 @@
   tri_blk_level_t(s, M, b0, b1, lower, kind, intra, permn, rhs, x);
 }
 
-void spmv_blk_stream(hipStream_t s, const BlkView &A, int R, int C, const int *rowblk, int nblk, const double *xo,
+void spmv_blk_stream(hipStream_t s, const BlkView &A, int R, int C, const int4 *desc, int nblk, const double *xo,
                      const double *xg, double *y, const double *epi_d, const double *epi_dinv) {
   if (nblk <= 0) return;
   if (epi_d) {
-    hipLaunchKernelGGL((spmv_blk_kernel<double, 2, 1, 1>), dim3(nblk), dim3(BLK), 0, s, A, rowblk, xo, xg, y, epi_d, epi_dinv);
+    hipLaunchKernelGGL((spmv_blk_kernel<double, 2, 1, 1>), dim3(nblk), dim3(BLK), 0, s, A, desc, xo, xg, y, epi_d, epi_dinv);
     return;
   }
-#define NSK_BK(RR, CC) hipLaunchKernelGGL((spmv_blk_kernel<double, RR, CC, 0>), dim3(nblk), dim3(BLK), 0, s, A, rowblk, xo, xg, y, nullptr, nullptr)
+#define NSK_BK(RR, CC) hipLaunchKernelGGL((spmv_blk_kernel<double, RR, CC, 0>), dim3(nblk), dim3(BLK), 0, s, A, desc, xo, xg, y, nullptr, nullptr)
   if (R == 2 && C == 2) NSK_BK(2, 2);
   else if (R == 2 && C == 1) NSK_BK(2, 1);
   else if (R == 1 && C == 2) NSK_BK(1, 2);
@@ -1583,16 +1642,16 @@
 #undef NSK_BK
 }
 
-void spmv_blk_stream(hipStream_t s, const BlkView32 &A, const int *rowblk, int nblk, const double *xo, const double *xg,
+void spmv_blk_stream(hipStream_t s, const BlkView32 &A, const int4 *desc, int nblk, const double *xo, const double *xg,
                      double *y) {
   if (nblk > 0)
-    hipLaunchKernelGGL((spmv_blk_kernel<float, 2, 2, 0>), dim3(nblk), dim3(BLK), 0, s, A, rowblk, xo, xg, y, nullptr, nullptr);
+    hipLaunchKernelGGL((spmv_blk_kernel<float, 2, 2, 0>), dim3(nblk), dim3(BLK), 0, s, A, desc, xo, xg, y, nullptr, nullptr);
 }
 
 void spmv_blk_fused22_21(hipStream_t s, const BlkView &A, const double *xao, const double *xag, const BlkView &B,
-                         const double *xbo, const double *xbg, const int *rowblk, int nblk, double *y) {
+                         const double *xbo, const double *xbg, const int4 *desc, int nblk, double *y) {
   if (nblk > 0)
-    hipLaunchKernelGGL(spmv_blk_fused_kernel, dim3(nblk), dim3(BLK), 0, s, A, xao, xag, B, xbo, xbg, rowblk, y);
+    hipLaunchKernelGGL(spmv_blk_fused_kernel, dim3(nblk), dim3(BLK), 0, s, A, xao, xag, B, xbo, xbg, desc, y);
 }
 
 template <class V>
diff --git a/navier_stokes_solver_amd/csrc/nsk_precond.cpp b/navier_stokes_solver_amd/csrc/nsk_precond.cpp
--- a/navier_stokes_solver_amd/csrc/nsk_precond.cpp
+++ b/navier_stokes_solver_amd/csrc/nsk_precond.cpp
@@ -345,7 +345,7 @@
   halo(1, dp);
   Csr &BT = Bt;
   if (BT.blk_ok && use_stream && use_bsr && BT.blk_R == 2 && BT.blk_C == 1) {
-    nsk::spmv_blk_stream(s(), BT.blk_view(), 2, 1, BT.blk_rowblk.p, BT.blk_nblk, dp.own, dp.ghost, du.own, D, Dinv);
+    nsk::spmv_blk_stream(s(), BT.blk_view(), 2, 1, BT.blk_desc.p, BT.blk_nblk, dp.own, dp.ghost, du.own, D, Dinv);
     ++ctx.st.spmv_calls;
     ctx.st.spmv_bytes += (double)BT.spmv_bytes() + 24.0 * nu;
   } else {
diff --git a/navier_stokes_solver_amd/solver.py b/navier_stokes_solver_amd/solver.py
--- a/navier_stokes_solver_amd/solver.py
+++ b/navier_stokes_solver_amd/solver.py
@@ -46,7 +46,7 @@
     "nsk_tri_apply", "nsk_amg_info", "nsk_tri_get_perm", "nsk_tri_get_value_bytes", "nsk_inner_value_bytes", "nsk_inner_basis_bytes", "nsk_inner_matrix_free", "nsk_matfree_f", "nsk_inner_spmv", "nsk_precond_vmult", "nsk_block_nnz", "nsk_get_block", "nsk_get_stats",
     "nsk_reset_stats", "nsk_get_history", "nsk_cancel", "nsk_abort_group", "nsk_assembly_set_cells", "nsk_assembly_set_simplex", "nsk_assembly_set_dirichlet", "nsk_state_set", "nsk_state_get",
     "nsk_state_save", "nsk_state_save_old", "nsk_state_update", "nsk_assemble", "nsk_scale_values", "nsk_download_rhs", "nsk_time_assemble", "nsk_time_op", "nsk_profile_begin", "nsk_profile_read", "nsk_profile_end",
-    "nsk_debug_spmv_form",
+    "nsk_debug_spmv_form", "nsk_debug_stream_slots",
     "nsk_forces_set_faces", "nsk_forces_set_edges", "nsk_forces", "nsk_state_get_patches",
     "nsk_record_set_cells", "nsk_state_get_record",
 ]
@@ -199,6 +199,14 @@
                                             int(inner))]
 
 
+def stream_slots(pairs: bool, k0: int, k1: int):
+    L = lib()
+    L.nsk_debug_stream_slots.argtypes = [C.c_int, C.c_int, C.c_int, C.c_void_p]
+    out = np.zeros((2048, 4), dtype=np.int32)
+    n = L.nsk_debug_stream_slots(int(bool(pairs)), int(k0), int(k1), out.ctypes.data)
+    return out[:n] if n else None
+
+
 def local_group_id(nranks: int, on_stream: bool = False) -> bytes:
     buf = C.create_string_buffer(128)
     L = lib()
```
